# gabrielspmoreira/chameleon_recsys

Hardware: AMD Instinct MI355X
Metric: NAR training sessions/sec (higher is better)
Workload: dtype f32

## Files before the change

### chameleon_recsys_amd/_lib.py

```python
import ctypes
import os
from ctypes import c_double, c_float, c_int, c_int32, c_int64, c_long, c_size_t, c_uint32, c_void_p

_HERE = os.path.dirname(os.path.abspath(__file__))
LIB_PATH = os.path.join(_HERE, "libchameleon_nar.so")

P = c_void_p

_SIGNATURES = {
    "cham_neg_sample_workspace_bytes": (c_size_t, [c_int, c_int, c_int]),
    "cham_neg_sample": (c_int, [P, c_int, c_int, P, c_int, c_uint32, c_uint32, c_int, c_int, c_int, c_int, P, P, P, P, P,
                                P, c_size_t, P]),
    "cham_ctx_assemble": (c_int, [P, P, c_int, P, c_int, P, P, P, P, P, P]),
    "cham_set_log_bases": (c_int, [c_float, c_float]),
    "cham_step_ints": (c_int, [P, P, P, P, c_int64, c_int, c_int, P, c_int, P, P, P, P, P, P]),
    "cham_item_dynamic_raw": (c_int, [P, P, c_int, P, P, P, P, P]),
    "cham_norm_stats_from_recent": (c_int, [P, c_int, c_int64, P, P, P, P, P]),
    "cham_norm_stats_from_buffer": (c_int, [P, c_int, c_int64, P, P, P, P, P]),
    "cham_norm_stats_from_rows": (c_int, [P, P, P, c_int, P, P]),
    "cham_row_weights": (c_int, [P, c_int, P, c_size_t, c_int, P, P, P, P]),
    "cham_item_assemble": (c_int, [P, c_int, c_int, c_int, P, c_int, P, c_int, P, P, P, P, c_int, P, P, P, P, P, P]),
    "cham_item_assemble_lds": (c_int, [P, c_int, c_int, c_int, P, c_int, P, c_int, P, P, P, P, c_int, P, c_int, P, c_int, P, P, P, P, P, P]),
    "cham_feature_bwd": (c_int, [P, P, c_int, c_int, P, P, P]),
    "cham_feature_bwd_workspace_bytes": (c_size_t, [c_int]),
    "cham_feature_bwd_ws": (c_int, [P, P, c_int, c_int, P, P, P, c_size_t, P]),
    "cham_emb_grad_scan": (c_int, [P, c_int, c_int, c_int, c_int, P, P, P, c_int, P, P]),
    "cham_group_rows_workspace_bytes": (c_size_t, [c_int]),
    "cham_group_rows_segments_len": (c_size_t, [c_int]),
    "cham_group_rows": (c_int, [P, c_int, c_int, P, P, P, c_size_t, P]),
    "cham_emb_grad_grouped": (c_int, [P, c_int, c_int, c_int, c_int, P, P, P, P, P, P]),
    "cham_dropout": (c_int, [P, P, c_long, c_int, c_int, c_float, c_uint32, c_uint32, c_int, c_int, c_int, P, c_int, c_int, c_int, c_int, P]),
    "cham_dense_rows": (c_int, [P, c_int, P, c_int, c_int, c_int, c_int, P, P, P]),
    "cham_gemm_f32": (c_int, [P, c_int, c_int, P, c_int, c_int, P, c_int, c_int, c_int, c_int, P, c_int, P, c_int, c_int,
                              P, c_int, c_int, c_int, P, c_size_t, c_int, P]),
    "cham_gemm_bf16": (c_int, [P, c_int, c_int, P, c_int, c_int, P, c_int, c_int, c_int, c_int, P, c_int, P, c_int, c_int,
                               P, c_int, c_int, c_int, P, c_size_t, c_int, P]),
    "cham_gemm_f32x3": (c_int, [P, c_int, c_int, P, c_int, c_int, P, c_int, c_int, c_int, c_int, P, c_int, P, c_int, c_int,
                                P, c_int, c_int, c_int, P, c_size_t, c_int, P]),
    "cham_gemm_f32x2h": (c_int, [P, c_int, c_int, P, c_int, c_int, P, c_int, c_int, c_int, c_int, P, c_int,
                                 P, c_int, c_int, c_int, P, c_size_t, c_int, P, P, P]),
    "cham_gemm_f32x3_set_variant": (None, [c_int]),
    "cham_gemm_f32x3_launch_counts": (None, [P, c_int]),
    "cham_gemm_p3": (c_int, [P, c_int64, c_int, P, c_int64, c_int, c_int, P, c_int, c_int, c_int, c_int, P, c_int, P, c_int, c_int, c_int,
                             P, c_size_t, c_int, P]),
    "cham_gemm_b16_dma": (c_int, [P, c_int, P, c_int, c_int, P, c_int, c_int, c_int, c_int, P, c_int, P, c_int, c_int, c_int, P, c_size_t, c_int, P]),
    "cham_gemm_p3_launch_counts": (None, [P, c_int]),
    "cham_gemm_b16_dma_set_nt_wide": (c_int, [c_int]),
    "cham_split3": (c_int, [P, c_int, c_int, c_int, P, c_int64, c_int, P, c_int64, c_int, P]),
    "cham_combine_fwd_p3": (c_int, [P, P, c_int, c_int, c_int, c_int, P, P, c_int64, P]),
    "cham_mulpred_bwd_p3": (c_int, [P, P, P, c_int, c_int, c_int, P, P, c_int64, P, P]),
    "cham_dm_mulpred_p3": (c_int, [P, c_int, c_int, P, c_int64, P, P, c_int, c_int, c_int, P, c_int64, P, P, P]),
    "cham_h2_scale_absmax": (c_int, [P, c_size_t, P, c_size_t, P, P]),
    "cham_h2_scale_rownorm": (c_int, [P, c_long, c_int, c_int, P, P, P]),
    "cham_h2_scale_rownorm2": (c_int, [P, c_long, c_int, c_int, P, P, P, P]),
    "cham_split2h": (c_int, [P, c_int, c_int, c_int, P, c_int64, c_int, P, c_int64, c_int, P, c_int, P]),
    "cham_gemm_h2": (c_int, [P, c_int64, c_int, P, P, c_int64, c_int, P, c_int, P, c_int, c_int, c_int, c_int, P, c_int, P, c_int, c_int, c_int,
                             P, c_size_t, c_int, P]),
    "cham_h2b_block_elements": (c_int, []),
    "cham_gemm_h2b": (c_int, [P, c_int64, c_int, P, P, c_int64, c_int, P, c_int, P, c_int, c_int, c_int, c_int, P, c_int, P, c_int, c_int, c_int,
                              P, c_size_t, c_int, c_int, c_int, c_int, P]),
    "cham_combine_fwd_h2b": (c_int, [P, P, c_int, c_int, c_int, c_int, P, P, c_int64, P, c_int, P]),
    "cham_dm_mulpred_h2_blk": (c_int, [P, c_int, c_int, P, c_int64, P, P, P, P, c_int, c_int, c_int, P, c_int64, P, P, P, P]),
    "cham_gemm_h2_launch_counts": (None, [P, c_int]),
    "cham_gemm_h2_set_nt_wide": (c_int, [c_int]),
    "cham_combine_fwd_h2": (c_int, [P, P, c_int, c_int, c_int, c_int, P, P, c_int64, P, P]),
    "cham_mulpred_bwd_h2": (c_int, [P, P, P, c_int, c_int, c_int, P, P, c_int64, P, P, P]),
    "cham_dm_mulpred_h2": (c_int, [P, c_int, c_int, P, c_int64, P, P, c_int, c_int, c_int, P, c_int64, P, P, P, P]),
    "cham_dm_mulpred_h2h": (c_int, [P, c_int, c_int, P, c_int64, P, P, P, P, c_int, c_int, c_int, P, c_int64, P, P, P, P]),
    "cham_dm_mulpred_b16": (c_int, [P, c_int, c_int, P, P, P, c_int, c_int, c_int, P, P, P, P]),
    "cham_gemm_b16": (c_int, [P, c_int, c_int, P, c_int, c_int, P, c_int, c_int, c_int, c_int, c_int, P, c_int, P, c_int, c_int, c_int,
                              P, c_size_t, c_int, P]),
    "cham_gemm_b16_set_variant": (None, [c_int]),
    "cham_gemm_b16_launch_counts": (None, [P, c_int]),
    "cham_gemm_set_variant": (None, [c_int]),
    "cham_gemm_launch_counts": (None, [P, c_int]),
    "cham_combine_fwd": (c_int, [P, P, c_int, c_int, c_int, c_int, P, P, c_long, c_long, P]),
    "cham_combine_bwd_workspace_bytes": (c_size_t, [c_int, c_int, c_int, c_int]),
    "cham_combine_bwd": (c_int, [P, c_int, c_int, c_int, c_int, P, P, P, P, c_size_t, P]),
    "cham_combine_bwd_gs": (c_int, [P, c_int, c_int, c_int, c_int, P, P, P, P, c_size_t, P, c_size_t, P]),
    "cham_gemm_h2_groupsum_bytes": (c_size_t, [c_int, c_int, c_int]),
    "cham_gemm_h2_dgrad_gs": (c_int, [P, c_int64, c_int, P, P, c_int64, c_int, P, P, c_int, c_int, c_int, c_int, P, c_int, c_int, c_int, c_int, P,
                                      c_size_t, P]),
    "cham_combine_fwd_b16": (c_int, [P, P, c_int, c_int, c_int, c_int, P, P, P]),
    "cham_combine_bwd_b16": (c_int, [P, P, c_int, c_int, c_int, c_int, P, P, P, P, c_size_t, P]),
    "cham_mulpred_bwd_b16": (c_int, [P, P, P, c_int, c_int, c_int, P, P]),
    "cham_mul_rows_b16": (c_int, [P, P, c_int, c_int, c_int, P, P]),
    "cham_score_softmax_fwd_b16": (c_int, [P, c_int, P, P, c_int, c_int, c_float, P, P, P, P, c_float, P, P, P, P]),
    "cham_score_softmax_bwd_b16": (c_int, [P, c_int, P, P, P, c_int, c_int, c_float, c_float, P, P, c_float, P, P, P, P, P]),
    "cham_colsum_b16": (c_int, [P, c_int, c_int, c_int, P, P, c_int, P, c_size_t, P]),
    "cham_cast_b16": (c_int, [P, c_int, c_int, P, P, P]),
    "cham_upcast_b16": (c_int, [P, c_size_t, P, P]),
    "cham_rnn_fwd": (c_int, [c_int, P, P, P, c_int, c_int, c_int, P, P, P, P, P, P, P]),
    "cham_rnn_bwd": (c_int, [c_int, P, P, P, c_int, c_int, c_int, P, P, P, P, P, P]),
    "cham_rnn_coop_workspace_bytes": (c_size_t, [c_int, c_int]),
    "cham_ugrnn_fwd_coop": (c_int, [P, P, P, c_int, c_int, c_int, P, P, P, P, P, c_size_t, P]),
    "cham_ugrnn_bwd_coop": (c_int, [P, P, P, c_int, c_int, c_int, P, P, P, P, P, c_size_t, P]),
    "cham_rnn_coop_timeouts": (c_int, [P, c_int, c_int, P]),
    "cham_ugrnn_point_fwd": (c_int, [P, P, P, c_int, c_int, c_int, c_int, P, P, P, P, P, P]),
    "cham_ugrnn_point_bwd": (c_int, [P, P, P, c_int, c_int, c_int, c_int, P, P, P, P, P, P, P]),
    "cham_transpose_f32": (c_int, [P, c_int, c_int, P, P]),
    "cham_rows_gather": (c_int, [P, P, c_long, c_int, P, P]),
    "cham_rows_scatter": (c_int, [P, P, c_long, c_int, P, P]),
    "cham_mulpred_bwd": (c_int, [P, P, P, c_int, c_int, c_int, P, P]),
    "cham_score_softmax_fwd": (c_int, [P, c_int, P, P, c_int, c_int, c_float, P, P, P, P, c_float, P, P, P, P]),
    "cham_score_softmax_bwd": (c_int, [P, c_int, P, P, P, c_int, c_int, c_float, c_float, P, P, c_float, P, P, P, P, P]),
    "cham_rank_items": (c_int, [P, P, P, P, c_int, c_int, P, P, P, P]),
    "cham_state_workspace_bytes": (c_size_t, [c_int, c_int]),
    "cham_state_update": (c_int, [P, P, c_int, c_int, c_double, P, P, c_int, P, P, P, c_int, c_int, P, P, c_size_t, P]),
    "cham_sumsq_partial": (c_int, [P, c_size_t, P, P]),
    "cham_loss_finalize": (c_int, [P, c_int, c_float, P, c_float, P, P]),
    "cham_adam_tf": (c_int, [P, P, P, P, c_size_t, c_size_t, c_float, c_float, c_float, c_float, c_float, P]),
    "cham_step_scalars_bytes": (c_int, []),
    "cham_step_scalars_set": (c_int, [P, c_uint32, c_uint32, c_int64, c_float, c_float, c_int, P]),
    "cham_neg_sample_dev": (c_int, [P, c_int, c_int, P, c_int, c_uint32, P, c_int, c_int, c_int, c_int, c_int, P, P, P, P, P, P, c_size_t, P]),
    "cham_step_ints_dev": (c_int, [P, P, P, P, P, c_int, c_int, P, c_int, P, P, P, P, P, P]),
    "cham_norm_stats_from_buffer_dev": (c_int, [P, c_int, P, P, P, P, P, P]),
    "cham_score_softmax_bwd_dev": (c_int, [P, c_int, P, P, P, c_int, c_int, c_float, P, P, P, c_float, P, P, P, P, P]),
    "cham_score_softmax_bwd_b16_dev": (c_int, [P, c_int, P, P, P, c_int, c_int, c_float, P, P, P, c_float, P, P, P, P, P]),
    "cham_loss_finalize_dev": (c_int, [P, c_int, P, P, c_float, P, P]),
    "cham_adam_tf_dev": (c_int, [P, P, P, P, c_size_t, c_size_t, c_float, P, c_float, c_float, c_float, P]),
    "cham_accumulate": (c_int, [P, P, c_size_t, c_int, P]),
    "cham_loss_accumulate": (c_int, [P, P, c_int, P]),
    "cham_colsum_workspace_bytes": (c_size_t, [c_int, c_int]),
    "cham_colsum": (c_int, [P, c_int, c_int, c_int, P, P, c_int, P, c_size_t, P]),
}

EXPORTED_SYMBOLS = tuple(_SIGNATURES.keys())


class ChameleonLibError(RuntimeError):
    pass


_lib = None


def load():
    global _lib
    if _lib is not None:
        return _lib
    if not os.path.exists(LIB_PATH):
        raise ChameleonLibError(
            "HIP extension %s is missing - run `python -c 'import __graft_entry__ as g; g.build()'` "
            "(hipcc --offload-arch=gfx950).  There is no CPU fallback." % LIB_PATH)
    lib = ctypes.CDLL(LIB_PATH)
    for name, (res, args) in _SIGNATURES.items():
        fn = getattr(lib, name)
        fn.restype = res
        fn.argtypes = args
    lib.cham_gemm_h2_set_nt_wide(1 if os.environ.get("CHAM_H2_NT_WIDE", "1") == "1" else 0)
    lib.cham_gemm_b16_dma_set_nt_wide(1 if os.environ.get("CHAM_B16_NT_WIDE", "1") == "1" else 0)
    _lib = lib
    return lib


def check(rc, what):
    if rc != 0:
        raise ChameleonLibError("%s failed with code %d" % (what, rc))


def ptr(t):
    return None if t is None else t.data_ptr()
```

### chameleon_recsys_amd/build.py

```python
import hashlib
import os
import subprocess
import sys

HERE = os.path.dirname(os.path.abspath(__file__))
CSRC = os.path.join(HERE, "csrc")
LIB = os.path.join(HERE, "libchameleon_nar.so")
SOURCES = ["gemm.hip", "gemm_x3.hip", "gemm_p3.hip", "gemm_h2.hip", "dm_fused.hip", "gemm_b16.hip", "sampler.hip", "features.hip", "scorer.hip", "rnn.hip", "rnn_coop.hip", "optim.hip", "state.hip"]
FLAGS = ["--offload-arch=gfx950", "-O3", "-std=c++17", "-fPIC", "-Wall", "-Wno-unused-function"]
FLAGS += os.environ.get("CHAM_BUILD_DEFINES", "").split()


HOST_LIB = os.path.join(HERE, "libchameleon_tfrecord.so")
HOST_SOURCES = [os.path.join(CSRC, "host", "tfrecord.cpp")]
HOST_FLAGS = ["-O2", "-std=c++17", "-fPIC", "-shared", "-Wall", "-pthread"]


def _stamp(files=None, flags=FLAGS):
    h = hashlib.sha256()
    if files is None:
        files = [os.path.join(CSRC, f) for f in sorted(os.listdir(CSRC)) if os.path.isfile(os.path.join(CSRC, f))]
    for f in files:
        with open(f, "rb") as fh:
            h.update(os.path.basename(f).encode()); h.update(fh.read())
    h.update(" ".join(flags).encode())
    return h.hexdigest()


HOST_LIB_SANITIZED = os.path.join(HERE, "libchameleon_tfrecord_san.so")
SANITIZE_FLAGS = ["-O1", "-g", "-fno-omit-frame-pointer", "-fsanitize=address,undefined", "-fno-sanitize-recover=undefined"]


def build_host(force=False, verbose=True, sanitize=False):
    lib = HOST_LIB_SANITIZED if sanitize else HOST_LIB
    flags = [f for f in HOST_FLAGS if f != "-O2"] + SANITIZE_FLAGS if sanitize else HOST_FLAGS
    stamp_file = lib + ".stamp"
    stamp = _stamp(HOST_SOURCES, flags)
    if not force and os.path.exists(lib) and os.path.exists(stamp_file) and open(stamp_file).read() == stamp:
        return lib
    cmd = [os.environ.get("CXX", "g++")] + flags + HOST_SOURCES + ["-o", lib, "-lz"]
    if verbose:
        print(" ".join(cmd), flush=True)
    subprocess.check_call(cmd)
    with open(stamp_file, "w") as fh:
        fh.write(stamp)
    return lib


def sanitizer_runtime():
    try:
        out = subprocess.check_output([os.environ.get("CXX", "g++"), "-print-file-name=libasan.so"]).decode().strip()
    except (OSError, subprocess.CalledProcessError):
        return None
    return os.path.realpath(out) if os.path.sep in out and os.path.exists(out) else None


def _src_stamp(src):
    h = hashlib.sha256()
    for f in [os.path.join(CSRC, src)] + sorted(os.path.join(CSRC, x) for x in os.listdir(CSRC) if x.endswith(".h")):
        with open(f, "rb") as fh:
            h.update(os.path.basename(f).encode()); h.update(fh.read())
    h.update(" ".join(FLAGS).encode())
    return h.hexdigest()


def build(force=False, verbose=True):
    stamp_file = LIB + ".stamp"
    stamp = _stamp()
    if not force and os.path.exists(LIB) and os.path.exists(stamp_file) and open(stamp_file).read() == stamp:
        return LIB
    hipcc = os.environ.get("HIPCC", "/opt/rocm/bin/hipcc")
    objs = []
    procs = []
    os.makedirs(os.path.join(HERE, "build"), exist_ok=True)
    for s in SOURCES:
        o = os.path.join(HERE, "build", s.replace(".hip", ".o"))
        objs.append(o)
        st, sf = _src_stamp(s), o + ".stamp"
        if not force and os.path.exists(o) and os.path.exists(sf) and open(sf).read() == st:
            continue
        cmd = [hipcc] + FLAGS + ["-c", os.path.join(CSRC, s), "-o", o]
        if verbose:
            print(" ".join(cmd), flush=True)
        procs.append((s, sf, st, subprocess.Popen(cmd, stdout=subprocess.PIPE, stderr=subprocess.STDOUT)))
    for s, sf, st, p in procs:
        out, _ = p.communicate()
        if p.returncode != 0:
            sys.stderr.write(out.decode())
            raise RuntimeError("hipcc failed on %s" % s)
        if verbose and out.strip():
            print(out.decode())
        with open(sf, "w") as fh:
            fh.write(st)
    cmd = [hipcc, "--offload-arch=gfx950", "-shared", "-fPIC", "-o", LIB] + objs
    if verbose:
        print(" ".join(cmd), flush=True)
    subprocess.check_call(cmd)
    with open(stamp_file, "w") as fh:
        fh.write(stamp)
    return LIB


if __name__ == "__main__":
    build(force="--force" in sys.argv)
    build_host(force="--force" in sys.argv)
```

### chameleon_recsys_amd/csrc/gemm_h2.hip

```cpp
#include "gemm_shared.h"

typedef _Float16 half8 __attribute__((ext_vector_type(8)));
typedef short h2_s16x4 __attribute__((ext_vector_type(4)));

struct H2Params {
    const _Float16* A; const _Float16* B;
    long long a_ps, b_ps;
    int lda, ldb;
    const float* sa; const float* sb;
    float* C; int ldc;
    int M, N, K;
    const float* bias;
    const unsigned short* dref; int ldr;
    int kchunk, splits; float* partial;
    int nbm, nbn, xcd_split, accumulate;
    int a_tiles, b_tiles, r_blk;
    float* gsum; int ggrp, gsk;
};

#define H2_SLAB 8192
#define H2_STAGE (4 * H2_SLAB)
#define H2_RING 4

__device__ __forceinline__ u32x4 h2_rsrc(const void* base, unsigned bytes) {
    const unsigned long long a = (unsigned long long)base;
    u32x4 r;
    r.x = (unsigned)a; r.y = (unsigned)(a >> 32) & 0xFFFFu; r.z = bytes; r.w = 0x00020000u;
    return r;
}

__device__ __forceinline__ void h2_dma_stage(unsigned lds0, unsigned va, unsigned vb, const u32x4& ra0, const u32x4& ra1, const u32x4& rb0,
                                             const u32x4& rb1) {
    unsigned keep;
    const unsigned l1 = lds0 + H2_SLAB, l2 = lds0 + 2 * H2_SLAB, l3 = lds0 + 3 * H2_SLAB;
    asm volatile(
        "s_nop 4\n\t"
        "s_mov_b32 %0, m0\n\t"
        "s_mov_b32 m0, %1\n\ts_nop 0\n\tbuffer_load_dwordx4 %5, %7, 0 offen lds\n\t"
        "s_mov_b32 m0, %2\n\ts_nop 0\n\tbuffer_load_dwordx4 %5, %8, 0 offen lds\n\t"
        "s_mov_b32 m0, %3\n\ts_nop 0\n\tbuffer_load_dwordx4 %6, %9, 0 offen lds\n\t"
        "s_mov_b32 m0, %4\n\ts_nop 0\n\tbuffer_load_dwordx4 %6, %10, 0 offen lds\n\t"
        "s_mov_b32 m0, %0"
        : "=&s"(keep)
        : "s"(lds0), "s"(l1), "s"(l2), "s"(l3), "v"(va), "v"(vb), "s"(ra0), "s"(ra1), "s"(rb0), "s"(rb1)
        : "memory");
}

template <bool TN>
__device__ __forceinline__ half8 h2_frag(const unsigned char* __restrict__ s, unsigned hi_off = 4 * 512) {
    if constexpr (!TN) {
        return *reinterpret_cast<const half8*>(s);
    } else {
        typedef __attribute__((address_space(3))) h2_s16x4 lds_s4;
        const h2_s16x4 lo = __builtin_amdgcn_ds_read_tr16_b64_v4i16((lds_s4*)(s));
        const h2_s16x4 hi = __builtin_amdgcn_ds_read_tr16_b64_v4i16((lds_s4*)(s + hi_off));
        typedef short s16x8 __attribute__((ext_vector_type(8)));
        s16x8 v;
        v[0] = lo[0]; v[1] = lo[1]; v[2] = lo[2]; v[3] = lo[3]; v[4] = hi[0]; v[5] = hi[1]; v[6] = hi[2]; v[7] = hi[3];
        return __builtin_bit_cast(half8, v);
    }
}

__device__ __forceinline__ void h2_barrier() {
    __builtin_amdgcn_fence(__ATOMIC_RELEASE, "workgroup", "local");
    __builtin_amdgcn_s_waitcnt(0xc07f);
    __builtin_amdgcn_s_barrier();
    __builtin_amdgcn_fence(__ATOMIC_ACQUIRE, "workgroup", "local");
    __builtin_amdgcn_sched_barrier(0);
}

template <int EPI, int TM, int TNN>
__device__ __forceinline__ void h2_epilogue(const H2Params& p, floatx16 (&acc)[TM][TNN], int m0, int n0, int wm0, int wn0, int split, int lane) {
    int lane_e = lane;
    asm volatile("" : "+v"(lane_e));
    const int kl = lane_e >> 5, fl = lane_e & 31;
    const float ia = p.sa[1], ib = p.sb[1];
#pragma unroll
    for (int i = 0; i < TM; ++i)
#pragma unroll
        for (int j = 0; j < TNN; ++j)
#pragma unroll
            for (int e = 0; e < 16; ++e) acc[i][j][e] = (acc[i][j][e] * ia) * ib;
    if constexpr (EPI == 3) {
        const int limM = p.M - m0, limN = p.N - n0;
        const __amdgpu_buffer_rsrc_t cw = make_window(p.C + (size_t)m0 * p.ldc + n0);
        const bool rb = p.r_blk != 0;
        const __amdgpu_buffer_rsrc_t dw = make_window(rb ? p.dref + ((size_t)(m0 >> 8) * (size_t)(p.ldr >> 5) + (size_t)(n0 >> 5)) * H2B_BLOCK
                                                         : p.dref + (size_t)m0 * p.ldr + n0);
        const int rstride = rb ? 64 : p.ldr * 2;
        const bool gs = p.gsum != nullptr;
        const int G = gs ? p.ggrp : 1, rbase = m0 + wm0;
        float* gw = gs ? p.gsum + (size_t)(rbase >> 7) * (size_t)p.gsk * (size_t)p.N + n0 + wn0 + fl : nullptr;
        float cur[TNN], hik[TNN];
#pragma unroll
        for (int j = 0; j < TNN; ++j) { cur[j] = 0.f; hik[j] = 0.f; }
        int kk = 0;
        auto emit = [&]() {
#pragma unroll
            for (int j = 0; j < TNN; ++j) {
                const float x = cur[j] + __shfl_xor(cur[j], 32, 64);
                if (kl == 0 && wn0 + j * 32 + fl < limN) gw[(size_t)kk * p.N + j * 32] = x;
            }
            ++kk;
        };
        int bnd = 64;
        auto block_begin = [&](int i) {
            if (!gs) return;
            const int s0 = rbase + 32 * i, gf = s0 / G;
            bnd = (gf + 1) * G - s0;
            if (i > 0 && bnd == G) {
                emit();
#pragma unroll
                for (int j = 0; j < TNN; ++j) cur[j] = 0.f;
            }
        };
        auto block_add = [&](int j, const float (&v)[16]) {
            if (!gs) return;
            float lo = 0.f;
            if (bnd >= 32) {
#pragma unroll
                for (int e = 0; e < 16; ++e) lo += v[e];
            } else {
                float hi = 0.f;
#pragma unroll
                for (int e = 0; e < 16; ++e) {
                    const bool first = (e & 3) + 8 * (e >> 2) + 4 * kl < bnd;
                    lo += first ? v[e] : 0.f;
                    hi += first ? 0.f : v[e];
                }
                hik[j] = hi;
            }
            cur[j] += lo;
        };
        auto block_end = [&]() {
            if (!gs || bnd >= 32) return;
            emit();
#pragma unroll
            for (int j = 0; j < TNN; ++j) cur[j] = hik[j];
        };
        if (limM >= wm0 + TM * 32 && limN >= wn0 + TNN * 32) {
#pragma unroll
            for (int i = 0; i < TM; ++i) {
                block_begin(i);
#pragma unroll
                for (int j = 0; j < TNN; ++j) {
                    const unsigned col = (unsigned)(wn0 + j * 32 + fl), rowb = (unsigned)(wm0 + i * 32 + 4 * kl);
                    const unsigned voff = (rowb * (unsigned)p.ldc + col) * 4u;
                    const unsigned voffr = rb ? (unsigned)((wn0 >> 5) + j) * (unsigned)(H2B_BLOCK * 2) + rowb * 64u + (unsigned)fl * 2u
                                              : (rowb * (unsigned)p.ldr + col) * 2u;
                    unsigned short y[16];
#pragma unroll
                    for (int e = 0; e < 16; ++e) {
                        const int ce = (e & 3) + 8 * (e >> 2);
// ... 215 lines not shown
            for (int ii = 0; ii < TM; ++ii) AL[ii] = h2_frag<TN>(Sn + 1 * H2_SLAB + fa[ii], hia);
            mma(AH, BL);
            cur = nxt;
        }
        asm volatile("s_waitcnt vmcnt(0)" ::: "memory");
    }

    h2_epilogue<EPI, TM, TNN>(p, acc, m0, n0, wm0, wn0, split, lane);
}

#define H2W_SLAB 16384
#define H2W_BUF (4 * H2W_SLAB)

__device__ __forceinline__ void h2w_dma4(unsigned l0, unsigned l1, unsigned v0, unsigned v1, const u32x4& r0, const u32x4& r1) {
    unsigned keep;
    const unsigned l0b = l0 + 1024u, l1b = l1 + 1024u;
    asm volatile(
        "s_nop 4\n\t"
        "s_mov_b32 %0, m0\n\t"
        "s_mov_b32 m0, %1\n\ts_nop 0\n\tbuffer_load_dwordx4 %5, %7, 0 offen lds\n\t"
        "s_mov_b32 m0, %2\n\ts_nop 0\n\tbuffer_load_dwordx4 %6, %7, 0 offen lds\n\t"
        "s_mov_b32 m0, %3\n\ts_nop 0\n\tbuffer_load_dwordx4 %5, %8, 0 offen lds\n\t"
        "s_mov_b32 m0, %4\n\ts_nop 0\n\tbuffer_load_dwordx4 %6, %8, 0 offen lds\n\t"
        "s_mov_b32 m0, %0"
        : "=&s"(keep)
        : "s"(l0), "s"(l0b), "s"(l1), "s"(l1b), "v"(v0), "v"(v1), "s"(r0), "s"(r1)
        : "memory");
}

template <int EPI, bool ABLK>
__global__ __launch_bounds__(512) void gemm_h2w_kernel(H2Params p) {
    constexpr int BM = 256, BN = 256, TM = 4, TNN = 2;
    extern __shared__ __attribute__((aligned(1024))) unsigned char h2_smem[];

    const int nwg = p.nbm * p.nbn;
    const int id = blockIdx.x;
    const int q8 = nwg / 8, rr = nwg % 8, xcd = id % 8;
    const int swz = (xcd < rr ? xcd * (q8 + 1) : rr * (q8 + 1) + (xcd - rr) * q8) + id / 8;
    const int tile_m = swz / p.nbn, tile_n = swz % p.nbn;
    const int m0 = tile_m * BM, n0 = tile_n * BN;
    const int nd = p.K >> 5;
    const int lane = threadIdx.x & 63, wave = __builtin_amdgcn_readfirstlane(threadIdx.x >> 6);
    const int wm0 = (wave >> 2) * 128, wn0 = (wave & 3) * 64;

    u32x4 ra[2], rb[2];
    const size_t aall = (size_t)max(p.M - m0, 0) * p.lda * 2, ball = (size_t)max(p.N - n0, 0) * p.ldb * 2;
#pragma unroll
    for (int q = 0; q < 2; ++q) {
        if constexpr (ABLK) ra[q] = h2_rsrc(p.A + q * p.a_ps + (size_t)tile_m * (size_t)(p.lda >> 5) * H2B_BLOCK,
                                            (unsigned)min((size_t)(p.lda >> 5) * (H2B_BLOCK * 2), (size_t)0xFFFFFFF0u));
        else ra[q] = h2_rsrc(p.A + q * p.a_ps + (size_t)m0 * p.lda, (unsigned)min(aall, (size_t)0xFFFFFFF0u));
        rb[q] = h2_rsrc(p.B + q * p.b_ps + (size_t)n0 * p.ldb, (unsigned)min(ball, (size_t)0xFFFFFFF0u));
    }
    const unsigned row = 32u * (unsigned)wave + (unsigned)(lane >> 2), sp = (unsigned)((lane & 3) ^ ((lane >> 4) & 3));
    unsigned va0 = ABLK ? row * 64u + 16u * sp : (row * (unsigned)p.lda + 8u * sp) * 2u;
    unsigned va1 = va0 + (ABLK ? 16u * 64u : 16u * (unsigned)p.lda * 2u);
    constexpr unsigned stepA = ABLK ? (unsigned)(H2B_BLOCK * 2) : 64u;
    unsigned vb0 = (row * (unsigned)p.ldb + 8u * sp) * 2u, vb1 = vb0 + 16u * (unsigned)p.ldb * 2u;

    unsigned fa0[TM], fb0[TNN], fa1[TM], fb1[TNN];
    {
        const int l31 = lane & 31;
        const unsigned fo = (unsigned)l31 * 64u + (unsigned)((lane >> 5) ^ ((l31 >> 2) & 3)) * 16u;
#pragma unroll
        for (int i = 0; i < TM; ++i) { fa0[i] = (unsigned)(wm0 + 32 * i) * 64u + fo; fa1[i] = fa0[i] ^ 32u; }
#pragma unroll
        for (int j = 0; j < TNN; ++j) { fb0[j] = (unsigned)(wn0 + 32 * j) * 64u + fo; fb1[j] = fb0[j] ^ 32u; }
    }

    floatx16 acc[TM][TNN];
#pragma unroll
    for (int i = 0; i < TM; ++i)
#pragma unroll
        for (int j = 0; j < TNN; ++j)
#pragma unroll
            for (int e = 0; e < 16; ++e) acc[i][j][e] = 0.f;

    typedef __attribute__((address_space(3))) unsigned char lds_u8;
    const unsigned lds_base = (unsigned)(unsigned long long)(lds_u8*)h2_smem;
    const unsigned wave_off = (unsigned)wave * 2048u;
    half8 AH[TM], AL[TM], BH[TNN], BL[TNN];

    auto mma = [&](const half8 (&X)[TM], const half8 (&Y)[TNN]) {
#pragma unroll
        for (int ii = 0; ii < TM; ++ii)
#pragma unroll
            for (int j = 0; j < TNN; ++j) acc[ii][j] = __builtin_amdgcn_mfma_f32_32x32x16_f16(X[ii], Y[j], acc[ii][j], 0, 0, 0);
        __builtin_amdgcn_sched_barrier(0);
    };
    auto dma_a = [&](unsigned buf) {
        h2w_dma4(lds_base + buf + 0 * H2W_SLAB + wave_off, lds_base + buf + 1 * H2W_SLAB + wave_off, va0, va1, ra[0], ra[1]);
        va0 += stepA; va1 += stepA;
    };
    auto dma_b = [&](unsigned buf) {
        h2w_dma4(lds_base + buf + 2 * H2W_SLAB + wave_off, lds_base + buf + 3 * H2W_SLAB + wave_off, vb0, vb1, rb[0], rb[1]);
        vb0 += 64u; vb1 += 64u;
    };

    if (nd > 0) {
        dma_a(0u); dma_b(0u);
        if (nd > 1) {
            dma_a((unsigned)H2W_BUF);
            asm volatile("s_waitcnt vmcnt(4)" ::: "memory");
        } else {
            asm volatile("s_waitcnt vmcnt(0)" ::: "memory");
        }
        h2_barrier();
        {
#pragma unroll
            for (int j = 0; j < TNN; ++j) BH[j] = *reinterpret_cast<const half8*>(h2_smem + 2 * H2W_SLAB + fb0[j]);
#pragma unroll
            for (int i = 0; i < TM; ++i) AL[i] = *reinterpret_cast<const half8*>(h2_smem + 1 * H2W_SLAB + fa0[i]);
        }
        for (int j = 0; j < nd; ++j) {
            const unsigned b0 = (unsigned)(j & 1) * (unsigned)H2W_BUF, b1 = (unsigned)H2W_BUF - b0;
            const unsigned char* S0 = h2_smem + b0;
            const unsigned char* S1 = h2_smem + b1;
            __builtin_amdgcn_sched_barrier(0);
            if (j + 1 < nd) dma_b(b1);
            __builtin_amdgcn_sched_barrier(0);
#pragma unroll
            for (int ii = 0; ii < TM; ++ii) AH[ii] = *reinterpret_cast<const half8*>(S0 + 0 * H2W_SLAB + fa0[ii]);
#pragma unroll
            for (int jn = 0; jn < TNN; ++jn) BL[jn] = *reinterpret_cast<const half8*>(S0 + 3 * H2W_SLAB + fb0[jn]);
            mma(AL, BH);
            mma(AH, BH);
#pragma unroll
            for (int jn = 0; jn < TNN; ++jn) BH[jn] = *reinterpret_cast<const half8*>(S0 + 2 * H2W_SLAB + fb1[jn]);
#pragma unroll
            for (int ii = 0; ii < TM; ++ii) AL[ii] = *reinterpret_cast<const half8*>(S0 + 1 * H2W_SLAB + fa1[ii]);
            mma(AH, BL);
#pragma unroll
            for (int ii = 0; ii < TM; ++ii) AH[ii] = *reinterpret_cast<const half8*>(S0 + 0 * H2W_SLAB + fa1[ii]);
#pragma unroll
            for (int jn = 0; jn < TNN; ++jn) BL[jn] = *reinterpret_cast<const half8*>(S0 + 3 * H2W_SLAB + fb1[jn]);
            mma(AL, BH);
            mma(AH, BH);
            asm volatile("s_waitcnt vmcnt(0)" ::: "memory");
            h2_barrier();
            if (j + 2 < nd) dma_a(b0);
            __builtin_amdgcn_sched_barrier(0);
#pragma unroll
            for (int jn = 0; jn < TNN; ++jn) BH[jn] = *reinterpret_cast<const half8*>(S1 + 2 * H2W_SLAB + fb0[jn]);
#pragma unroll
            for (int ii = 0; ii < TM; ++ii) AL[ii] = *reinterpret_cast<const half8*>(S1 + 1 * H2W_SLAB + fa0[ii]);
            mma(AH, BL);
        }
        asm volatile("s_waitcnt vmcnt(0)" ::: "memory");
    }

    h2_epilogue<EPI, TM, TNN>(p, acc, m0, n0, wm0, wn0, 0, lane);
}

__device__ __forceinline__ void h2_finish_scale(H2Scale* rec, float bound) {
    float s = 1.f, inv = 1.f;
    if (bound > 0.f && bound < __builtin_inff()) {
        int e;
        (void)frexpf(bound, &e);
        int k = 15 - e;
        k = k < -110 ? -110 : (k > 110 ? 110 : k);
        s = ldexpf(1.f, k); inv = ldexpf(1.f, -k);
    }
    rec->scale = s; rec->inv = inv; rec->bound = bound;
}

__device__ __forceinline__ float h2_block_max(float v, float* red) {
    v = wave_max(v);
    const int lane = threadIdx.x & 63, w = threadIdx.x >> 6;
    if (lane == 0) red[w] = v;
    __syncthreads();
    float t = 0.f;
    for (int i = 0; i < (int)(blockDim.x >> 6); ++i) t = fmaxf(t, red[i]);
    __syncthreads();
    return t;
}

__global__ __launch_bounds__(256) void k_h2_scale_absmax(const float* __restrict__ x0, size_t n0, const float* __restrict__ x1, size_t n1,
                                                         H2Scale* __restrict__ rec) {
    __shared__ float red[4];
    __shared__ unsigned last;
    float m0 = 0.f, m1 = 0.f;
    const size_t stride = (size_t)gridDim.x * 256;
#pragma unroll 4
    for (size_t i = (size_t)blockIdx.x * 256 + threadIdx.x; i < n0 / 4; i += stride) {
        const float4 v = reinterpret_cast<const float4*>(x0)[i];
        m0 = fmaxf(m0, fmaxf(fmaxf(fabsf(v.x), fabsf(v.y)), fmaxf(fabsf(v.z), fabsf(v.w))));
    }
    if (x1)
#pragma unroll 4
        for (size_t i = (size_t)blockIdx.x * 256 + threadIdx.x; i < n1 / 4; i += stride) {
            const float4 v = reinterpret_cast<const float4*>(x1)[i];
            m1 = fmaxf(m1, fmaxf(fmaxf(fabsf(v.x), fabsf(v.y)), fmaxf(fabsf(v.z), fabsf(v.w))));
        }
    m0 = h2_block_max(m0, red);
    m1 = h2_block_max(m1, red);
    if (threadIdx.x == 0) {
        atomicMax(&rec->max_bits, __float_as_uint(m0));
        if (x1) atomicMax(&rec->pad1, __float_as_uint(m1));
        __threadfence();
        last = atomicAdd(&rec->ticket, 1u) == gridDim.x - 1 ? 1u : 0u;
        if (last) {
            __threadfence();
            const float a = __uint_as_float(atomicMax(&rec->max_bits, 0u)), b = __uint_as_float(atomicMax(&rec->pad1, 0u));
            h2_finish_scale(rec, a + b);
            rec->max_bits = 0u; rec->pad1 = 0u; rec->ticket = 0u;
        }
    }
}

__global__ __launch_bounds__(256) void k_h2_scale_rownorm(const float* __restrict__ X, long R, int K, int ld, const float* __restrict__ factor,
                                                          H2Scale* __restrict__ rec, H2Scale* __restrict__ rec_plain) {
    __shared__ float red[4];
    __shared__ unsigned last;
    const int lane = threadIdx.x & 63;
    const long wave_g = (long)blockIdx.x * 4 + (threadIdx.x >> 6), nwaves = (long)gridDim.x * 4;
    float mx = 0.f;
    if (K == 128) {
        const int hl = lane & 31, hw = lane >> 5;
        const long stride = 2 * nwaves;
        long r = 2 * wave_g + hw;
        for (; r + 3 * stride < R; r += 4 * stride) {
            float4 v[4];
#pragma unroll
            for (int u = 0; u < 4; ++u) v[u] = reinterpret_cast<const float4*>(X + (size_t)(r + u * stride) * ld)[hl];
#pragma unroll
            for (int u = 0; u < 4; ++u) {
                float s = v[u].x * v[u].x + v[u].y * v[u].y + v[u].z * v[u].z + v[u].w * v[u].w;
#pragma unroll
                for (int o = 16; o > 0; o >>= 1) s += __shfl_xor(s, o, 64);
                mx = fmaxf(mx, s);
            }
        }
        for (; r < R; r += stride) {
            const float4 v = reinterpret_cast<const float4*>(X + (size_t)r * ld)[hl];
            float s = v.x * v.x + v.y * v.y + v.z * v.z + v.w * v.w;
#pragma unroll
            for (int o = 16; o > 0; o >>= 1) s += __shfl_xor(s, o, 64);
            mx = fmaxf(mx, s);
        }
    } else {
        for (long r = wave_g; r < R; r += nwaves) {
            float s = 0.f;
            for (int k = lane; k < K; k += 64) { const float v = X[(size_t)r * ld + k]; s += v * v; }
            mx = fmaxf(mx, wave_sum(s));
        }
    }
    mx = h2_block_max(mx, red);
    if (threadIdx.x == 0) {
        atomicMax(&rec->max_bits, __float_as_uint(mx));
        __threadfence();
        last = atomicAdd(&rec->ticket, 1u) == gridDim.x - 1 ? 1u : 0u;
        if (last) {
            __threadfence();
            const float sq = __uint_as_float(atomicMax(&rec->max_bits, 0u));
            const float b = sqrtf(sq) * (factor ? *factor : 1.f) * 1.0009765625f;
            h2_finish_scale(rec, b);
            if (rec_plain) h2_finish_scale(rec_plain, sqrtf(sq) * 1.0009765625f);
            rec->max_bits = 0u; rec->ticket = 0u;
        }
    }
}

extern "C" int cham_h2_scale_absmax(const float* x0, size_t n0, const float* x1, size_t n1, void* rec, void* stream) {
    if (!x0 || !rec || (n0 & 3) || (x1 && (n1 & 3)) || (((uintptr_t)x0 | (uintptr_t)x1) & 15) || ((uintptr_t)rec & 15)) return -CHAM_ERR_ARG;
    size_t n = n0 > n1 ? n0 : n1;
    int blocks = (int)((n / 4 + 255) / 256);
    blocks = blocks < 1 ? 1 : (blocks > 512 ? 512 : blocks);
    hipLaunchKernelGGL(k_h2_scale_absmax, dim3(blocks), dim3(256), 0, (hipStream_t)stream, x0, n0, x1, x1 ? n1 : (size_t)0, reinterpret_cast<H2Scale*>(rec));
    CHAM_CHECK_LAUNCH();
    return CHAM_OK;
}

extern "C" int cham_h2_scale_rownorm2(const float* X, long R, int K, int ld, const float* factor, void* rec, void* rec_plain, void* stream) {
    if (!X || !rec || R < 0 || K <= 0 || ld < K || (((uintptr_t)rec | (uintptr_t)rec_plain) & 15) || rec == rec_plain) return -CHAM_ERR_ARG;
    if (K == 128 && ((ld & 3) || ((uintptr_t)X & 15))) return -CHAM_ERR_ARG;
    const long per = K == 128 ? 8 : 4;
    long blocks = (R + per - 1) / per;
    blocks = blocks < 1 ? 1 : (blocks > 1024 ? 1024 : blocks);
    hipLaunchKernelGGL(k_h2_scale_rownorm, dim3((unsigned)blocks), dim3(256), 0, (hipStream_t)stream, X, R, K, ld, factor, reinterpret_cast<H2Scale*>(rec),
                       reinterpret_cast<H2Scale*>(rec_plain));
    CHAM_CHECK_LAUNCH();
    return CHAM_OK;
}
extern "C" int cham_h2_scale_rownorm(const float* X, long R, int K, int ld, const float* factor, void* rec, void* stream) {
    return cham_h2_scale_rownorm2(X, R, K, ld, factor, rec, nullptr, stream);
}

__global__ __launch_bounds__(256) void k_split2h(const float* __restrict__ X, int R, int Cc, int ld, _Float16* __restrict__ dst, long long ps,
                                                 int ldd, _Float16* __restrict__ dstT, long long psT, int lddT, const H2Scale* __restrict__ rec) {
    const float s = rec->scale;
    const size_t n = (size_t)R * Cc;
    for (size_t i = (size_t)blockIdx.x * 256 + threadIdx.x; i < n; i += (size_t)gridDim.x * 256) {
        const int r = (int)(i / Cc), c = (int)(i % Cc);
        const float x = X[(size_t)r * ld + c];
        _Float16 h, l;
        split2h(x * s, h, l);
        const unsigned short hb = h2_keep_sign(h, x);
        if (dst) { _Float16* d = dst + (size_t)r * ldd + c; *reinterpret_cast<unsigned short*>(d) = hb; d[ps] = l; }
        if (dstT) { _Float16* d = dstT + (size_t)c * lddT + r; *reinterpret_cast<unsigned short*>(d) = hb; d[psT] = l; }
    }
}

extern "C" int cham_split2h(const float* X, int R, int Cc, int ld, void* dst, long long plane_stride, int ldd, void* dstT,
                            long long plane_strideT, int lddT, void* rec, int recompute, void* stream) {
    if (!X || R <= 0 || Cc <= 0 || (!dst && !dstT) || !rec || ((uintptr_t)rec & 15)) return -CHAM_ERR_ARG;
    const size_t n = (size_t)R * Cc;
    if (recompute) {
        if (ld != Cc || (n & 3) || ((uintptr_t)X & 15)) return -CHAM_ERR_ARG;
        const int rc = cham_h2_scale_absmax(X, n, nullptr, 0, rec, stream);
        if (rc != CHAM_OK) return rc;
    }
    int blocks = (int)((n + 255) / 256);
    if (blocks > 8192) blocks = 8192;
    hipLaunchKernelGGL(k_split2h, dim3(blocks), dim3(256), 0, (hipStream_t)stream, X, R, Cc, ld, reinterpret_cast<_Float16*>(dst), plane_stride,
                       ldd, reinterpret_cast<_Float16*>(dstT), plane_strideT, lddT, reinterpret_cast<const H2Scale*>(rec));
    CHAM_CHECK_LAUNCH();
    return CHAM_OK;
}

extern "C" int cham_h2b_block_elements(void) { return H2B_BLOCK; }

static long long g_h2_launches[8];
extern "C" void cham_gemm_h2_launch_counts(long long* out8, int reset) {
    for (int i = 0; i < 8; ++i) { if (out8) out8[i] = g_h2_launches[i]; if (reset) g_h2_launches[i] = 0; }
}

static int g_h2_nt_wide = 1;
extern "C" int cham_gemm_h2_set_nt_wide(int on) { const int was = g_h2_nt_wide; g_h2_nt_wide = on ? 1 : 0; return was; }

template <int EPI, bool ABLK>
static int h2w_launch_l(H2Params& p, hipStream_t st) {
    g_h2_launches[6] = EPI; g_h2_launches[7] = 1; ++g_h2_launches[2];
    if (ABLK) ++g_h2_launches[3];
    constexpr int smem = 2 * H2W_BUF;
    auto k = gemm_h2w_kernel<EPI, ABLK>;
    CHAM_SET_DYNAMIC_LDS(k, smem);
    hipLaunchKernelGGL(k, dim3(p.nbm * p.nbn, 1, 1), dim3(512), smem, st, p);
    CHAM_CHECK_LAUNCH();
    return CHAM_OK;
}
template <int EPI>
static int h2w_launch(H2Params& p, hipStream_t st) {
    return p.a_tiles > 0 ? h2w_launch_l<EPI, true>(p, st) : h2w_launch_l<EPI, false>(p, st);
}

template <bool TN, int EPI>
static int h2_launch(H2Params& p, hipStream_t st) {
    g_h2_launches[6] = EPI; g_h2_launches[7] = p.splits;
    constexpr int smem = H2_RING * H2_STAGE;
    auto k = gemm_h2_kernel<TN, EPI>;
    CHAM_SET_DYNAMIC_LDS(k, smem);
    hipLaunchKernelGGL(k, dim3(p.nbm * p.nbn, p.splits, 1), dim3(512), smem, st, p);
    CHAM_CHECK_LAUNCH();
    return CHAM_OK;
}
extern "C" size_t cham_gemm_h2_groupsum_bytes(int M, int N, int group_rows) {
    if (M <= 0 || N <= 0 || group_rows < 32) return 0;
    return (size_t)2 * ((M + 255) / 256) * (size_t)(127 / group_rows + 2) * (size_t)N * sizeof(float);
}
static int h2_run(const void* A, long long a_plane_stride, int lda, const float* a_scale, const void* B, long long b_plane_stride,
                  int ldb, const float* b_scale, int tn, float* C, int ldc, int M, int N, int K, const float* bias, int act,
                  const void* dref_h, int ldr, int dact, int accumulate, float* workspace, size_t workspace_bytes, int splits_hint,
                  int a_tiles, int b_tiles, int dref_blocked, int group_rows, float* groupsum, size_t groupsum_bytes, void* stream) {
    if (!A || !B || !C || !a_scale || !b_scale || M <= 0 || N <= 0 || K <= 0 || a_tiles < 0 || b_tiles < 0) return -CHAM_ERR_ARG;
    if (groupsum && (tn || !dref_h || group_rows < 32 || groupsum_bytes < cham_gemm_h2_groupsum_bytes(M, N, group_rows) || ((uintptr_t)groupsum & 15)))
        return -CHAM_ERR_ARG;
    {
        const long a_rows = tn ? K : M, b_rows = tn ? K : N;
        if (a_tiles && ((lda & 31) || (long)a_tiles * 256 < a_rows || a_plane_stride < (long long)a_tiles * (lda >> 5) * H2B_BLOCK)) return -CHAM_ERR_ARG;
        if (b_tiles && ((ldb & 31) || (long)b_tiles * 256 < b_rows || b_plane_stride < (long long)b_tiles * (ldb >> 5) * H2B_BLOCK)) return -CHAM_ERR_ARG;
        if (!tn && (b_tiles || (a_tiles && (lda != K || (K & 31) || !g_h2_nt_wide)))) return -CHAM_ERR_ARG;
        if (dref_blocked && (!dref_h || (ldr & 31) || tn)) return -CHAM_ERR_ARG;
    }
    if ((lda & 7) || (ldb & 7) || (a_plane_stride & 7) || (b_plane_stride & 7) || (N & 3) || (ldc & 3)) return -CHAM_ERR_ARG;
    if (((uintptr_t)A | (uintptr_t)B | (uintptr_t)C) & 15) return -CHAM_ERR_ARG;
    if ((size_t)ldc * 4 * 256 >= WINDOW_BYTES || (size_t)ldr * 2 * 256 >= WINDOW_BYTES) return -CHAM_ERR_ARG;
    H2Params p;
    p.A = reinterpret_cast<const _Float16*>(A); p.B = reinterpret_cast<const _Float16*>(B); p.a_ps = a_plane_stride; p.b_ps = b_plane_stride;
    p.lda = lda; p.ldb = ldb; p.sa = a_scale; p.sb = b_scale; p.C = C; p.ldc = ldc; p.M = M; p.N = N; p.K = K; p.bias = bias;
    p.dref = reinterpret_cast<const unsigned short*>(dref_h); p.ldr = ldr; p.partial = workspace; p.xcd_split = 0; p.accumulate = 0;
    p.nbm = (M + 255) / 256; p.nbn = (N + 255) / 256;
    p.a_tiles = a_tiles; p.b_tiles = b_tiles; p.r_blk = dref_blocked ? 1 : 0;
    p.gsum = groupsum; p.ggrp = group_rows; p.gsk = groupsum ? 127 / group_rows + 2 : 0;
    hipStream_t st = (hipStream_t)stream;
    if (!tn) {
        if ((K & 15) || accumulate) return -CHAM_ERR_ARG;
        if ((size_t)256 * lda * 2 >= (1ull << 31) || (size_t)256 * ldb * 2 >= (1ull << 31)) return -CHAM_ERR_ARG;
        p.kchunk = K; p.splits = 1;
        if (dref_h && (bias || act != ACT_NONE || dact != ACT_LEAKY)) return -CHAM_ERR_ARG;
        if (act != ACT_NONE && !(bias && act == ACT_TANH)) return -CHAM_ERR_ARG;
        ++g_h2_launches[0];
        if (groupsum) ++g_h2_launches[5];
        if (g_h2_nt_wide && (K & 31) == 0) {
            if (dref_h) return h2w_launch<3>(p, st);
            if (bias) return act == ACT_TANH ? h2w_launch<2>(p, st) : h2w_launch<5>(p, st);
            return h2w_launch<0>(p, st);
        }
        if (dref_h) return h2_launch<false, 3>(p, st);
        if (bias) return act == ACT_TANH ? h2_launch<false, 2>(p, st) : h2_launch<false, 5>(p, st);
        return h2_launch<false, 0>(p, st);
    }
    if ((M & 255) || (N & 255) || bias || act != ACT_NONE || dref_h) return -CHAM_ERR_ARG;
    if ((size_t)16 * lda * 2 >= (1ull << 31) || (size_t)16 * ldb * 2 >= (1ull << 31)) return -CHAM_ERR_ARG;
    const long tiles = (long)p.nbm * p.nbn;
    int splits = 1;
    if (splits_hint != 1 && workspace) {
        long want = splits_hint > 1 ? splits_hint : (tiles >= 192 ? 1 : (256 + tiles - 1) / tiles);
        const long maxk = (K + 511) / 512;
        if (want > maxk) want = maxk;
        const long maxw = (long)(workspace_bytes / ((size_t)M * N * sizeof(float)));
        if (want > maxw) want = maxw;
        if (splits_hint <= 0 && want >= 8) want = want / 8 * 8;
        if (want > 1) splits = (int)want;
// ... 48 lines not shown
```

### chameleon_recsys_amd/csrc/scorer.hip

```cpp
#include "common.h"

__device__ __forceinline__ int cand_vrow(int bt, int c, int BT, int N, int pmax, const int* __restrict__ neg_slot) {
    if (c == 0) return BT + bt;
    int s = neg_slot[(size_t)bt * N + (c - 1)];
    if (s < 0) s = pmax;
    return 2 * BT + s;
}

__global__ __launch_bounds__(256) void k_combine_fwd(const float* __restrict__ U, const float* __restrict__ V, int C,
                                                     int BT, int N, int pmax, const int* __restrict__ neg_slot,
                                                     float* __restrict__ Z1, int row_begin) {
    const int row = row_begin + blockIdx.x;
    int u, v;
    if (row < BT) { u = row; v = row; }
    else {
        const int i = row - BT, bt = i / (N + 1), c = i % (N + 1);
        u = bt; v = cand_vrow(bt, c, BT, N, pmax, neg_slot);
    }
    const float4* pu = reinterpret_cast<const float4*>(U + (size_t)u * C);
    const float4* pv = reinterpret_cast<const float4*>(V + (size_t)v * C);
    float4* po = reinterpret_cast<float4*>(Z1 + (size_t)row * C);
    for (int k = threadIdx.x; k < C / 4; k += 256) {
        const float4 a = pu[k], b = pv[k];
        float4 o;
        o.x = act_fwd(a.x + b.x, ACT_LEAKY); o.y = act_fwd(a.y + b.y, ACT_LEAKY);
        o.z = act_fwd(a.z + b.z, ACT_LEAKY); o.w = act_fwd(a.w + b.w, ACT_LEAKY);
        po[k] = o;
    }
}

template <typename T>
__global__ __launch_bounds__(256) void k_combine_fwd_cand(const float* __restrict__ U, const float* __restrict__ V, int C,
                                                          int BT, int N, int pmax, const int* __restrict__ neg_slot,
                                                          T* __restrict__ Z1c ) {
    const int bt = blockIdx.x, NC = N + 1;
    const float4* pu = reinterpret_cast<const float4*>(U + (size_t)bt * C);
    T* po = Z1c + (size_t)bt * NC * C;
    for (int k = threadIdx.x; k < C / 4; k += 256) {
        const float4 a = pu[k];
        for (int c0 = 0; c0 < NC; c0 += 4) {
            float4 b[4];
#pragma unroll
            for (int i = 0; i < 4; ++i) {
                const int c = c0 + i < NC ? c0 + i : NC - 1;
                b[i] = reinterpret_cast<const float4*>(V + (size_t)cand_vrow(bt, c, BT, N, pmax, neg_slot) * C)[k];
            }
#pragma unroll
            for (int i = 0; i < 4; ++i) {
                if (c0 + i >= NC) break;
                float4 o;
                o.x = act_fwd(a.x + b[i].x, ACT_LEAKY); o.y = act_fwd(a.y + b[i].y, ACT_LEAKY);
                o.z = act_fwd(a.z + b[i].z, ACT_LEAKY); o.w = act_fwd(a.w + b[i].w, ACT_LEAKY);
                st4(po + (size_t)(c0 + i) * C + 4 * k, o);
            }
        }
    }
}

__global__ __launch_bounds__(256) void k_combine_fwd_cand_p3(const float* __restrict__ U, const float* __restrict__ V, int C,
                                                             int BT, int N, int pmax, const int* __restrict__ neg_slot,
                                                             __bf16* __restrict__ Z1p , long long ps) {
    const int bt = blockIdx.x, NC = N + 1;
    const float4* pu = reinterpret_cast<const float4*>(U + (size_t)bt * C);
    __bf16* po = Z1p + (size_t)bt * NC * C;
    for (int k = threadIdx.x; k < C / 4; k += 256) {
        const float4 a = pu[k];
        for (int c0 = 0; c0 < NC; c0 += 4) {
            float4 b[4];
#pragma unroll
            for (int i = 0; i < 4; ++i) {
                const int c = c0 + i < NC ? c0 + i : NC - 1;
                b[i] = reinterpret_cast<const float4*>(V + (size_t)cand_vrow(bt, c, BT, N, pmax, neg_slot) * C)[k];
            }
#pragma unroll
            for (int i = 0; i < 4; ++i) {
                if (c0 + i >= NC) break;
                float4 o;
                o.x = act_fwd(a.x + b[i].x, ACT_LEAKY); o.y = act_fwd(a.y + b[i].y, ACT_LEAKY);
                o.z = act_fwd(a.z + b[i].z, ACT_LEAKY); o.w = act_fwd(a.w + b[i].w, ACT_LEAKY);
                st4_planes(po + (size_t)(c0 + i) * C + 4 * k, ps, o);
            }
        }
    }
}

__global__ __launch_bounds__(256) void k_combine_fwd_cand_h2(const float* __restrict__ U, const float* __restrict__ V, int C,
                                                             int BT, int N, int pmax, const int* __restrict__ neg_slot,
                                                             _Float16* __restrict__ Z1p , long long ps,
                                                             const H2Scale* __restrict__ rec, int blocked) {
    const int bt = blockIdx.x, NC = N + 1;
    const float sc = rec->scale;
    const float4* pu = reinterpret_cast<const float4*>(U + (size_t)bt * C);
    _Float16* po = Z1p + (size_t)bt * NC * C;
    const size_t grow0 = (size_t)bt * NC;
    const unsigned ncb = (unsigned)C >> 5;
    for (int k = threadIdx.x; k < C / 4; k += 256) {
        const float4 a = pu[k];
        for (int c0 = 0; c0 < NC; c0 += 4) {
            float4 b[4];
#pragma unroll
            for (int i = 0; i < 4; ++i) {
                const int c = c0 + i < NC ? c0 + i : NC - 1;
                b[i] = reinterpret_cast<const float4*>(V + (size_t)cand_vrow(bt, c, BT, N, pmax, neg_slot) * C)[k];
            }
#pragma unroll
            for (int i = 0; i < 4; ++i) {
                if (c0 + i >= NC) break;
                float4 o;
                o.x = act_fwd(a.x + b[i].x, ACT_LEAKY); o.y = act_fwd(a.y + b[i].y, ACT_LEAKY);
                o.z = act_fwd(a.z + b[i].z, ACT_LEAKY); o.w = act_fwd(a.w + b[i].w, ACT_LEAKY);
                st4_planes_h2(blocked ? Z1p + h2b_index(grow0 + (size_t)(c0 + i), 4u * (unsigned)k, ncb) : po + (size_t)(c0 + i) * C + 4 * k, ps, o, sc);
            }
        }
    }
}

template <typename T>
__global__ __launch_bounds__(256) void k_combine_bwd_u(const float* __restrict__ dpre_in, const T* __restrict__ dpre_cand, int C, int BT,
                                                       int N, float* __restrict__ dU, float* __restrict__ dV) {
    const int bt = blockIdx.x;
    const float4* pin = reinterpret_cast<const float4*>(dpre_in + (size_t)bt * C);
    const T* pc = dpre_cand + (size_t)bt * (N + 1) * C;
    for (int k = threadIdx.x; k < C / 4; k += 256) {
        const float4 a = pin[k];
        const float4 p0 = ld4(pc + 4 * k);
        float4 s = make_float4(a.x + p0.x, a.y + p0.y, a.z + p0.z, a.w + p0.w);
        for (int c = 1; c <= N; c += 8) {
            float4 x[8];
#pragma unroll
            for (int u = 0; u < 8; ++u) x[u] = ld4(pc + (size_t)min(c + u, N) * C + 4 * k);
#pragma unroll
            for (int u = 0; u < 8; ++u)
                if (c + u <= N) { s.x += x[u].x; s.y += x[u].y; s.z += x[u].z; s.w += x[u].w; }
        }
        reinterpret_cast<float4*>(dU + (size_t)bt * C)[k] = s;
        reinterpret_cast<float4*>(dV + (size_t)bt * C)[k] = a;
        reinterpret_cast<float4*>(dV + ((size_t)BT + bt) * C)[k] = p0;
    }
}

__global__ __launch_bounds__(256) void k_combine_bwd_u_gs(const float* __restrict__ dpre_in, const float* __restrict__ dpre_cand, int C, int BT,
                                                          int N, const float* __restrict__ gsum, float* __restrict__ dU, float* __restrict__ dV) {
    const int bt = blockIdx.x, G = N + 1, gsk = 127 / G + 2;
    const long r0 = (long)bt * G, r1 = r0 + G - 1;
    const int q0 = (int)(r0 >> 7), q1 = (int)(r1 >> 7);
    const float4* pin = reinterpret_cast<const float4*>(dpre_in + (size_t)bt * C);
    const float4* pc = reinterpret_cast<const float4*>(dpre_cand + (size_t)r0 * C);
    for (int k = threadIdx.x; k < C / 4; k += 256) {
        const float4 a = pin[k], p0 = pc[k];
        float4 s = a;
        for (int q = q0; q <= q1; ++q) {
            const int piece = bt - (int)(((long)q << 7) / G);
            const float4 x = reinterpret_cast<const float4*>(gsum + ((size_t)q * gsk + piece) * C)[k];
// ... 147 lines not shown
        list[off++] = threadIdx.x * SEG + bit;
    }
    __syncthreads();
    const int nk = C / 4;
    for (int k = threadIdx.x; k < nk; k += 256) {
        float4 acc = make_float4(0.f, 0.f, 0.f, 0.f);
        int t = 0;
        for (; t + 8 <= cnt; t += 8) {
            float4 x[8];
#pragma unroll
            for (int u = 0; u < 8; ++u) {
                const size_t i = i0 + list[t + u];
                const size_t row = (i / N) * (N + 1) + 1 + (i % N);
                x[u] = ld4(cand + row * C + 4 * k);
            }
#pragma unroll
            for (int u = 0; u < 8; ++u) { acc.x += x[u].x; acc.y += x[u].y; acc.z += x[u].z; acc.w += x[u].w; }
        }
        for (; t < cnt; ++t) {
            const size_t i = i0 + list[t];
            const size_t row = (i / N) * (N + 1) + 1 + (i % N);
            const float4 x = ld4(cand + row * C + 4 * k);
            acc.x += x.x; acc.y += x.y; acc.z += x.z; acc.w += x.w;
        }
        reinterpret_cast<float4*>(partial + (size_t)chunk * C)[k] = acc;
    }
}
__global__ __launch_bounds__(256) void k_combine_bwd_pad_final(const float* __restrict__ partial, int C, int nchunk,
                                                               float* __restrict__ dv_row) {
    for (int k = threadIdx.x; k < C / 4; k += 256) {
        float4 acc = make_float4(0.f, 0.f, 0.f, 0.f);
        for (int c = 0; c < nchunk; c += 16) {
            float4 x[16];
#pragma unroll
            for (int u = 0; u < 16; ++u) x[u] = reinterpret_cast<const float4*>(partial + (size_t)min(c + u, nchunk - 1) * C)[k];
#pragma unroll
            for (int u = 0; u < 16; ++u)
                if (c + u < nchunk) { acc.x += x[u].x; acc.y += x[u].y; acc.z += x[u].z; acc.w += x[u].w; }
        }
        reinterpret_cast<float4*>(dv_row)[k] = acc;
    }
}

template <typename T>
__global__ __launch_bounds__(256) void k_mulpred_bwd(T* __restrict__ dM, const T* __restrict__ Z2c,
                                                     const float* __restrict__ pred, int C, int N, float* __restrict__ dpred_pre) {
    const int bt = blockIdx.x;
    const float4* pp = reinterpret_cast<const float4*>(pred + (size_t)bt * C);
    for (int k = threadIdx.x; k < C / 4; k += 256) {
        const float4 p = pp[k];
        float4 acc = make_float4(0.f, 0.f, 0.f, 0.f);
        for (int c = 0; c <= N; ++c) {
            const size_t off = ((size_t)bt * (N + 1) + c) * C + 4 * k;
            const float4 g = ld4(dM + off);
            const float4 z = ld4(Z2c + off);
            acc.x += g.x * z.x; acc.y += g.y * z.y; acc.z += g.z * z.z; acc.w += g.w * z.w;
            float4 o;
            o.x = g.x * p.x * (1.f - z.x * z.x); o.y = g.y * p.y * (1.f - z.y * z.y);
            o.z = g.z * p.z * (1.f - z.z * z.z); o.w = g.w * p.w * (1.f - z.w * z.w);
            st4(dM + off, o);
        }
        float4 o;
        o.x = acc.x * (1.f - p.x * p.x); o.y = acc.y * (1.f - p.y * p.y);
        o.z = acc.z * (1.f - p.z * p.z); o.w = acc.w * (1.f - p.w * p.w);
        reinterpret_cast<float4*>(dpred_pre + (size_t)bt * C)[k] = o;
    }
}

__global__ __launch_bounds__(256) void k_mulpred_bwd_p3(const float* __restrict__ dM, const float* __restrict__ Z2c,
                                                        const float* __restrict__ pred, int C, int N, float* __restrict__ dpred_pre,
                                                        __bf16* __restrict__ dZ2p, long long ps, float* __restrict__ col_part) {
    const int bt = blockIdx.x;
    const float4* pp = reinterpret_cast<const float4*>(pred + (size_t)bt * C);
    for (int k = threadIdx.x; k < C / 4; k += 256) {
        const float4 p = pp[k];
        float4 acc = make_float4(0.f, 0.f, 0.f, 0.f), cs = make_float4(0.f, 0.f, 0.f, 0.f);
        for (int c = 0; c <= N; ++c) {
            const size_t off = ((size_t)bt * (N + 1) + c) * C + 4 * k;
            const float4 g = ld4(dM + off);
            const float4 z = ld4(Z2c + off);
            acc.x += g.x * z.x; acc.y += g.y * z.y; acc.z += g.z * z.z; acc.w += g.w * z.w;
            float4 o;
            o.x = g.x * p.x * (1.f - z.x * z.x); o.y = g.y * p.y * (1.f - z.y * z.y);
            o.z = g.z * p.z * (1.f - z.z * z.z); o.w = g.w * p.w * (1.f - z.w * z.w);
            cs.x += o.x; cs.y += o.y; cs.z += o.z; cs.w += o.w;
            st4_planes(dZ2p + off, ps, o);
        }
        float4 o;
        o.x = acc.x * (1.f - p.x * p.x); o.y = acc.y * (1.f - p.y * p.y);
        o.z = acc.z * (1.f - p.z * p.z); o.w = acc.w * (1.f - p.w * p.w);
        reinterpret_cast<float4*>(dpred_pre + (size_t)bt * C)[k] = o;
        if (col_part) reinterpret_cast<float4*>(col_part + (size_t)bt * C)[k] = cs;
    }
}

__global__ __launch_bounds__(256) void k_mulpred_bwd_h2(const float* __restrict__ dM, const float* __restrict__ Z2c,
                                                        const float* __restrict__ pred, int C, int N, float* __restrict__ dpred_pre,
                                                        _Float16* __restrict__ dZ2p, long long ps, float* __restrict__ col_part,
                                                        const H2Scale* __restrict__ rec) {
    const int bt = blockIdx.x;
    const float sc = rec->scale;
    const float4* pp = reinterpret_cast<const float4*>(pred + (size_t)bt * C);
    for (int k = threadIdx.x; k < C / 4; k += 256) {
        const float4 p = pp[k];
        float4 acc = make_float4(0.f, 0.f, 0.f, 0.f), cs = make_float4(0.f, 0.f, 0.f, 0.f);
        for (int c = 0; c <= N; ++c) {
            const size_t off = ((size_t)bt * (N + 1) + c) * C + 4 * k;
            const float4 g = ld4(dM + off);
            const float4 z = ld4(Z2c + off);
            acc.x += g.x * z.x; acc.y += g.y * z.y; acc.z += g.z * z.z; acc.w += g.w * z.w;
            float4 o;
            o.x = g.x * p.x * (1.f - z.x * z.x); o.y = g.y * p.y * (1.f - z.y * z.y);
            o.z = g.z * p.z * (1.f - z.z * z.z); o.w = g.w * p.w * (1.f - z.w * z.w);
            cs.x += o.x; cs.y += o.y; cs.z += o.z; cs.w += o.w;
            st4_planes_h2(dZ2p + off, ps, o, sc);
        }
        float4 o;
        o.x = acc.x * (1.f - p.x * p.x); o.y = acc.y * (1.f - p.y * p.y);
        o.z = acc.z * (1.f - p.z * p.z); o.w = acc.w * (1.f - p.w * p.w);
        reinterpret_cast<float4*>(dpred_pre + (size_t)bt * C)[k] = o;
        if (col_part) reinterpret_cast<float4*>(col_part + (size_t)bt * C)[k] = cs;
    }
}

__global__ __launch_bounds__(256) void k_mul_rows_b16(const __bf16* __restrict__ Z2c, const float* __restrict__ pred, int C, int NC,
                                                      __bf16* __restrict__ Mc) {
    const int bt = blockIdx.x;
    const float4* pp = reinterpret_cast<const float4*>(pred + (size_t)bt * C);
    for (int k = threadIdx.x; k < C / 4; k += 256) {
        const float4 p = pp[k];
        for (int c0 = 0; c0 < NC; c0 += 4) {
            float4 z[4];
#pragma unroll
            for (int i = 0; i < 4; ++i) z[i] = ld4(Z2c + ((size_t)bt * NC + min(c0 + i, NC - 1)) * C + 4 * k);
#pragma unroll
            for (int i = 0; i < 4; ++i) {
                if (c0 + i >= NC) break;
                st4(Mc + ((size_t)bt * NC + c0 + i) * C + 4 * k, make_float4(z[i].x * p.x, z[i].y * p.y, z[i].z * p.z, z[i].w * p.w));
            }
        }
    }
}

template <int K3, typename T>
__global__ __launch_bounds__(256) void k_score_softmax_fwd(const T* __restrict__ S3, const float* __restrict__ w4,
                                                           const float* __restrict__ b4, int BT, int N, float inv_tau,
                                                           const unsigned char* __restrict__ mask,
                                                           float* __restrict__ logits, float* __restrict__ probs,
                                                           float* __restrict__ nll, float nov_factor,
                                                           const int64_t* __restrict__ neg_ids, const float* __restrict__ pop_norm,
                                                           float* __restrict__ nov_aux , float inv_log2_base) {
    const int lane = threadIdx.x & 63, bt = blockIdx.x * 4 + (threadIdx.x >> 6);
    if (bt >= BT) return;
    const int NC = N + 1;
    float w[K3];
#pragma unroll
    for (int k = 0; k < K3; ++k) w[k] = w4[k];
    const float bias = b4[0];
    float mx = -INFINITY;
    for (int c = lane; c < NC; c += 64) {
        const T* r = S3 + ((size_t)bt * NC + c) * K3;
        float s = 0.f;
#pragma unroll
        for (int k = 0; k < K3 / 4; ++k) { const float4 x = ld4(r + 4 * k); s += x.x * w[4 * k] + x.y * w[4 * k + 1] + x.z * w[4 * k + 2] + x.w * w[4 * k + 3]; }
        s += bias;
        logits[(size_t)bt * NC + c] = s;
        mx = fmaxf(mx, s * inv_tau);
    }
    mx = wave_max(mx);
    float sum = 0.f;
    for (int c = lane; c < NC; c += 64) {
        const float e = expf(logits[(size_t)bt * NC + c] * inv_tau - mx);
        probs[(size_t)bt * NC + c] = e;
        sum += e;
    }
    sum = wave_sum(sum);
    const float inv = 1.f / sum;
    for (int c = lane; c < NC; c += 64) probs[(size_t)bt * NC + c] *= inv;
    float novterm = 0.f;
    if (nov_factor > 0.f) {
        float mxn = -INFINITY;
        for (int c = lane; c < NC; c += 64)
            if (c > 0) mxn = fmaxf(mxn, logits[(size_t)bt * NC + c] * inv_tau);
        mxn = wave_max(mxn);
        float sn = 0.f, acc = 0.f;
        for (int c = lane; c < NC; c += 64)
            if (c > 0) {
                const float e = expf(logits[(size_t)bt * NC + c] * inv_tau - mxn);
                sn += e;
                acc += e * (-log2f(pop_norm[neg_ids[(size_t)bt * N + (c - 1)]]) * inv_log2_base);
            }
        sn = wave_sum(sn); acc = wave_sum(acc);
        novterm = acc / sn;
        if (lane == 0) { nov_aux[(size_t)bt * 3] = mxn; nov_aux[(size_t)bt * 3 + 1] = sn; nov_aux[(size_t)bt * 3 + 2] = novterm; }
    }
    if (lane == 0) {
        const float z0 = logits[(size_t)bt * NC] * inv_tau;
        nll[bt] = mask[bt] ? -((z0 - mx) - logf(sum)) - nov_factor * novterm : 0.f;
    }
}

template <int K3, typename T>
__global__ __launch_bounds__(256) void k_score_softmax_bwd(const T* __restrict__ S3, const float* __restrict__ w4,
                                                           const float* __restrict__ probs, const unsigned char* __restrict__ mask,
                                                           int BT, int N, float scale ,
                                                           float* __restrict__ ds, T* __restrict__ dS3, float nov_factor,
                                                           const int64_t* __restrict__ neg_ids, const float* __restrict__ pop_norm,
                                                           const float* __restrict__ logits, float inv_tau,
                                                           const float* __restrict__ nov_aux, float inv_log2_base,
                                                           const ChamStepScalars* __restrict__ sc, float tau) {
    const size_t row = (size_t)blockIdx.x * 256 + threadIdx.x;
    const int NC = N + 1;
    if (row >= (size_t)BT * NC) return;
    if (sc) scale = 1.0f / (tau * sc->sum_mask);
    const int bt = (int)(row / NC), c = (int)(row % NC);
    float g = mask[bt] ? (probs[row] - (c == 0 ? 1.f : 0.f)) * scale : 0.f;
    if (nov_factor > 0.f && c > 0 && mask[bt]) {
        const float q = expf(logits[row] * inv_tau - nov_aux[(size_t)bt * 3]) / nov_aux[(size_t)bt * 3 + 1];
        const float nov_c = -log2f(pop_norm[neg_ids[(size_t)bt * N + (c - 1)]]) * inv_log2_base;
        g -= nov_factor * scale * q * (nov_c - nov_aux[(size_t)bt * 3 + 2]);
    }
    ds[row] = g;
    const T* r = S3 + row * K3;
    T* o = dS3 + row * K3;
#pragma unroll
    for (int k = 0; k < K3 / 4; ++k) {
        const float4 x = ld4(r + 4 * k);
        float4 y;
        y.x = g * w4[4 * k] * act_bwd_from_out(x.x, ACT_LEAKY);
        y.y = g * w4[4 * k + 1] * act_bwd_from_out(x.y, ACT_LEAKY);
        y.z = g * w4[4 * k + 2] * act_bwd_from_out(x.z, ACT_LEAKY);
        y.w = g * w4[4 * k + 3] * act_bwd_from_out(x.w, ACT_LEAKY);
        st4(o + 4 * k, y);
    }
}


__global__ __launch_bounds__(256) void k_rank_items(const float* __restrict__ probs, const int64_t* __restrict__ label_next,
                                                    const int64_t* __restrict__ neg_ids, const unsigned char* __restrict__ mask,
                                                    int BT, int N, int64_t* __restrict__ pred_ids, float* __restrict__ pred_probs,
                                                    int32_t* __restrict__ label_rank) {
    extern __shared__ float sp[];
    const int lane = threadIdx.x & 63, w = threadIdx.x >> 6, bt = blockIdx.x * 4 + w;
    const int NC = N + 1;
    float* p = sp + (size_t)w * NC;
    if (bt < BT)
        for (int c = lane; c < NC; c += 64) p[c] = probs[(size_t)bt * NC + c];
    __syncthreads();
    if (bt >= BT) return;
    for (int c = lane; c < NC; c += 64) {
        const float pc = p[c];
        int r = 0;
        for (int j = 0; j < NC; ++j) {
            const float pj = p[j];
            r += (pj > pc) || (pj == pc && j < c);
        }
        pred_ids[(size_t)bt * NC + r] = c == 0 ? label_next[bt] : neg_ids[(size_t)bt * N + (c - 1)];
        pred_probs[(size_t)bt * NC + r] = pc;
        if (c == 0) label_rank[bt] = mask[bt] ? r : -1;
    }
}

extern "C" int cham_combine_fwd(const float* U, const float* V, int C, int BT, int N, int pmax, const int32_t* neg_slot,
                                float* Z1, long row_begin, long row_count, void* stream) {
    if (!U || !V || !neg_slot || !Z1 || (C & 3) || BT <= 0 || N <= 0) return -CHAM_ERR_ARG;
    const long rows = (long)BT + (long)BT * (N + 1);
    if (row_begin < 0 || row_count <= 0 || row_begin + row_count > rows) return -CHAM_ERR_ARG;
    if (row_begin == BT && row_count == (long)BT * (N + 1))
        hipLaunchKernelGGL(k_combine_fwd_cand<float>, dim3((unsigned)BT), dim3(256), 0, (hipStream_t)stream, U, V, C, BT, N, pmax, neg_slot,
                           Z1 + (size_t)BT * C);
    else
        hipLaunchKernelGGL(k_combine_fwd, dim3((unsigned)row_count), dim3(256), 0, (hipStream_t)stream, U, V, C, BT, N, pmax,
                           neg_slot, Z1, (int)row_begin);
    CHAM_CHECK_LAUNCH();
    return CHAM_OK;
}
extern "C" int cham_combine_fwd_b16(const float* U, const float* V, int C, int BT, int N, int pmax, const int32_t* neg_slot,
                                    void* Z1c, void* stream) {
    if (!U || !V || !neg_slot || !Z1c || (C & 3) || BT <= 0 || N <= 0) return -CHAM_ERR_ARG;
    hipLaunchKernelGGL(k_combine_fwd_cand<__bf16>, dim3((unsigned)BT), dim3(256), 0, (hipStream_t)stream, U, V, C, BT, N, pmax, neg_slot,
                       reinterpret_cast<__bf16*>(Z1c));
    CHAM_CHECK_LAUNCH();
    return CHAM_OK;
}

static inline size_t al256(size_t x) { return (x + 255) & ~(size_t)255; }
struct SlotWs { size_t bitmap_bytes, partial_bytes, pad_bytes; int W, nchunk, nchunk_pad; };
static SlotWs slot_ws(int C, int BT, int N, int pmax) {
    SlotWs w;
    w.W = (BT + 31) / 32;
    w.nchunk = (w.W + SLOT_HOT / 32 - 1) / (SLOT_HOT / 32);
    w.nchunk_pad = (int)(((size_t)BT * N + SLOT_LIST - 1) / SLOT_LIST);
    w.bitmap_bytes = al256((size_t)pmax * w.W * sizeof(unsigned));
    w.partial_bytes = al256((size_t)w.nchunk * pmax * C * sizeof(float));
    w.pad_bytes = al256((size_t)w.nchunk_pad * C * sizeof(float));
    return w;
}
extern "C" size_t cham_combine_bwd_workspace_bytes(int C, int BT, int N, int pmax) {
    if (C <= 0 || BT <= 0 || N <= 0 || pmax <= 0) return 0;
    const SlotWs w = slot_ws(C, BT, N, pmax);
    return w.bitmap_bytes + w.partial_bytes + w.pad_bytes;
}

template <typename T>
static int combine_bwd_impl(const float* dpre_in, const T* dpre_cand, int C, int BT, int N, int pmax, const int32_t* neg_slot,
                            float* dU, float* dV, float* workspace, size_t workspace_bytes, void* stream, const float* gsum = nullptr) {
    if (!dpre_in || !dpre_cand || !neg_slot || !dU || !dV || !workspace || (C & 3) || BT <= 0 || N <= 0 || pmax <= 0) return -CHAM_ERR_ARG;
    if (workspace_bytes < cham_combine_bwd_workspace_bytes(C, BT, N, pmax) || ((uintptr_t)workspace & 15)) return -CHAM_ERR_ARG;
    hipStream_t st = (hipStream_t)stream;
    const SlotWs w = slot_ws(C, BT, N, pmax);
    unsigned* bitmap = reinterpret_cast<unsigned*>(workspace);
    float* partial = reinterpret_cast<float*>(reinterpret_cast<char*>(workspace) + w.bitmap_bytes);
    float* pad_partial = reinterpret_cast<float*>(reinterpret_cast<char*>(workspace) + w.bitmap_bytes + w.partial_bytes);
    const size_t n = (size_t)BT * N;
    if constexpr (sizeof(T) == 4) {
        if (gsum) hipLaunchKernelGGL(k_combine_bwd_u_gs, dim3(BT), dim3(256), 0, st, dpre_in, reinterpret_cast<const float*>(dpre_cand), C, BT, N, gsum, dU, dV);
        else hipLaunchKernelGGL(k_combine_bwd_u<T>, dim3(BT), dim3(256), 0, st, dpre_in, dpre_cand, C, BT, N, dU, dV);
    } else {
        hipLaunchKernelGGL(k_combine_bwd_u<T>, dim3(BT), dim3(256), 0, st, dpre_in, dpre_cand, C, BT, N, dU, dV);
    }
    if (hipMemsetAsync(bitmap, 0, (size_t)pmax * w.W * sizeof(unsigned), st) != hipSuccess) return -CHAM_ERR_LAUNCH;
    hipLaunchKernelGGL(k_slot_bitmap, dim3((unsigned)((n + 255) / 256)), dim3(256), 0, st, neg_slot, n, N, pmax, w.W, bitmap);
    hipLaunchKernelGGL(k_slot_reduce<T>, dim3(pmax, w.nchunk), dim3(256), 0, st, dpre_cand, C, BT, N, neg_slot, bitmap, w.W, pmax, partial, dV);
    hipLaunchKernelGGL(k_slot_final, dim3(pmax), dim3(256), 0, st, partial, C, pmax, w.nchunk, BT, bitmap, w.W, dV);
    hipLaunchKernelGGL(k_combine_bwd_slots_partial<T>, dim3(w.nchunk_pad), dim3(256), 0, st, dpre_cand, C, BT, N, neg_slot, pmax,
                       pad_partial, SLOT_LIST);
    hipLaunchKernelGGL(k_combine_bwd_pad_final, dim3(1), dim3(256), 0, st, pad_partial, C, w.nchunk_pad,
                       dV + ((size_t)2 * BT + pmax) * C);
    CHAM_CHECK_LAUNCH();
    return CHAM_OK;
}
extern "C" int cham_combine_bwd(const float* dpre, int C, int BT, int N, int pmax, const int32_t* neg_slot,
                                float* dU, float* dV, float* workspace, size_t workspace_bytes, void* stream) {
    if (!dpre || BT <= 0 || C <= 0) return -CHAM_ERR_ARG;
    return combine_bwd_impl<float>(dpre, dpre + (size_t)BT * C, C, BT, N, pmax, neg_slot, dU, dV, workspace, workspace_bytes, stream);
}
extern "C" int cham_combine_bwd_gs(const float* dpre, int C, int BT, int N, int pmax, const int32_t* neg_slot, float* dU, float* dV,
                                   float* workspace, size_t workspace_bytes, const float* groupsum, size_t groupsum_bytes, void* stream) {
    if (!dpre || BT <= 0 || C <= 0 || !groupsum || N + 1 < 32 || ((uintptr_t)groupsum & 15)) return -CHAM_ERR_ARG;
    const size_t rows = (size_t)BT * (N + 1);
    if (groupsum_bytes < (size_t)2 * ((rows + 255) / 256) * (size_t)(127 / (N + 1) + 2) * (size_t)C * sizeof(float)) return -CHAM_ERR_ARG;
    return combine_bwd_impl<float>(dpre, dpre + (size_t)BT * C, C, BT, N, pmax, neg_slot, dU, dV, workspace, workspace_bytes, stream, groupsum);
}
extern "C" int cham_combine_bwd_b16(const float* dpre_in, const void* dpre_cand, int C, int BT, int N, int pmax, const int32_t* neg_slot,
                                    float* dU, float* dV, float* workspace, size_t workspace_bytes, void* stream) {
    return combine_bwd_impl<__bf16>(dpre_in, reinterpret_cast<const __bf16*>(dpre_cand), C, BT, N, pmax, neg_slot, dU, dV, workspace,
                                    workspace_bytes, stream);
}

extern "C" int cham_mulpred_bwd(float* dM, const float* Z2c, const float* pred, int C, int BT, int N, float* dpred_pre,
                                void* stream) {
    if (!dM || !Z2c || !pred || !dpred_pre || (C & 3) || BT <= 0) return -CHAM_ERR_ARG;
    hipLaunchKernelGGL(k_mulpred_bwd<float>, dim3(BT), dim3(256), 0, (hipStream_t)stream, dM, Z2c, pred, C, N, dpred_pre);
    CHAM_CHECK_LAUNCH();
    return CHAM_OK;
}
extern "C" int cham_mulpred_bwd_b16(void* dM, const void* Z2c, const float* pred, int C, int BT, int N, float* dpred_pre, void* stream) {
    if (!dM || !Z2c || !pred || !dpred_pre || (C & 3) || BT <= 0) return -CHAM_ERR_ARG;
    hipLaunchKernelGGL(k_mulpred_bwd<__bf16>, dim3(BT), dim3(256), 0, (hipStream_t)stream, reinterpret_cast<__bf16*>(dM),
                       reinterpret_cast<const __bf16*>(Z2c), pred, C, N, dpred_pre);
    CHAM_CHECK_LAUNCH();
    return CHAM_OK;
}
extern "C" int cham_combine_fwd_p3(const float* U, const float* V, int C, int BT, int N, int pmax, const int32_t* neg_slot, void* Z1p,
                                   long long plane_stride, void* stream) {
    if (!U || !V || !neg_slot || !Z1p || C <= 0 || (C & 3) || BT < 0 || N < 0 || (plane_stride & 3)) return -CHAM_ERR_ARG;
    if (BT == 0) return CHAM_OK;
    hipLaunchKernelGGL(k_combine_fwd_cand_p3, dim3(BT), dim3(256), 0, (hipStream_t)stream, U, V, C, BT, N, pmax, neg_slot,
                       reinterpret_cast<__bf16*>(Z1p), plane_stride);
    CHAM_CHECK_LAUNCH();
    return CHAM_OK;
}

extern "C" int cham_mulpred_bwd_p3(const float* dM, const float* Z2c, const float* pred, int C, int BT, int N, float* dpred_pre, void* dZ2p,
                                   long long plane_stride, float* col_part, void* stream) {
    if (!dM || !Z2c || !pred || !dpred_pre || !dZ2p || C <= 0 || (C & 3) || BT < 0 || N < 0 || (plane_stride & 3)) return -CHAM_ERR_ARG;
    if (BT == 0) return CHAM_OK;
    hipLaunchKernelGGL(k_mulpred_bwd_p3, dim3(BT), dim3(256), 0, (hipStream_t)stream, dM, Z2c, pred, C, N, dpred_pre,
                       reinterpret_cast<__bf16*>(dZ2p), plane_stride, col_part);
    CHAM_CHECK_LAUNCH();
    return CHAM_OK;
}

extern "C" int cham_combine_fwd_h2b(const float* U, const float* V, int C, int BT, int N, int pmax, const int32_t* neg_slot, void* Z1p,
                                    long long plane_stride, const void* scale_rec, int blocked, void* stream) {
    if (!U || !V || !neg_slot || !Z1p || !scale_rec || C <= 0 || (C & 3) || BT < 0 || N < 0 || (plane_stride & 3)) return -CHAM_ERR_ARG;
    if (blocked && ((C & 31) || plane_stride < (long long)(((size_t)BT * (N + 1) + 255) / 256) * (C >> 5) * H2B_BLOCK)) return -CHAM_ERR_ARG;
// ... 109 lines not shown
```

### chameleon_recsys_amd/nar/nar_model.py

```python
import math
import os

import numpy as np
import torch

from .. import _lib
from .. import _roctx
from .._lib import check, ptr
from .clicked_items_state import lane_stream
from .layout import COL_ITEMEMB, ParamLayout

ACT_NONE, ACT_LEAKY, ACT_TANH = 0, 1, 2


class ModeKeys:
    TRAIN = 'train'
    EVAL = 'eval'
    PREDICT = 'infer'


_raw_stream = getattr(torch._C, '_cuda_getCurrentRawStream', None)
_raw_device = getattr(torch._C, '_cuda_getDevice', None)


_raw_checked = False


def _stream():
    global _raw_stream, _raw_checked
    if _raw_stream is not None and _raw_device is not None:
        if not _raw_checked:
            _raw_checked = True
            try:
                if int(_raw_stream(_raw_device())) != int(torch.cuda.current_stream().cuda_stream):
                    _raw_stream = None
            except Exception:
                _raw_stream = None
            if _raw_stream is None:
                return torch.cuda.current_stream().cuda_stream
        return _raw_stream(_raw_device())
    return torch.cuda.current_stream().cuda_stream


class Tensor:

    def __init__(self, name, fn):
        self.name, self._fn = name, fn

    def eval(self):
        v = self._fn()
        if torch.is_tensor(v):
            v = v.cpu().numpy()
        return v


class Placeholder:

    def __init__(self, name):
        self.name = name

    def __hash__(self):
        return hash(self.name)

    def __eq__(self, o):
        return isinstance(o, Placeholder) and o.name == self.name


_VARIABLE_STORE = None


class variable_store:
    def __init__(self, store):
        self.store = store

    def __enter__(self):
        global _VARIABLE_STORE
        self._prev, _VARIABLE_STORE = _VARIABLE_STORE, self.store
        return self.store

    def __exit__(self, *a):
        global _VARIABLE_STORE
        _VARIABLE_STORE = self._prev


_TORCH_DTYPE = {np.dtype(n).str: t for n, t in (('int64', torch.int64), ('int32', torch.int32), ('float32', torch.float32),
                                                   ('uint8', torch.uint8))}


def pack_offsets(arrays, align=256):
    offs, total = {}, 0
    for k, a in arrays.items():
        offs[k] = total
        total += (a.nbytes + align - 1) & ~(align - 1)
    return offs, total


class _PinnedRing:

    def __init__(self, n=4, nbytes=4 << 20):
        self.n, self.nbytes = n, nbytes
        self.bufs, self.events, self.k, self.off = [None] * n, [None] * n, -1, 0

    def begin(self, need):
        self.k = (self.k + 1) % self.n
        if self.events[self.k] is not None:
            self.events[self.k].synchronize()
        if self.bufs[self.k] is None or self.bufs[self.k].numel() < need:
            self.bufs[self.k] = torch.empty(max(need, self.nbytes), dtype=torch.uint8, pin_memory=True)
        self.off = 0

    def stage(self, a):
        n = a.nbytes
        if n == 0 or self.off + n > self.bufs[self.k].numel():
            return torch.from_numpy(a)
        view = self.bufs[self.k][self.off:self.off + n]
        self.off += (n + 255) & ~255
        t = view.view(torch.from_numpy(a).dtype).view(a.shape)
        t.copy_(torch.from_numpy(a))
        return t

    def end(self, stream):
        ev = torch.cuda.Event()
        ev.record(stream)
        self.events[self.k] = ev


class NARRuntime:

    def __init__(self, params, device='cuda:0', seed=42, weights=None):
        self.lib = _lib.load()
        self._views = {}
        if not torch.cuda.is_available():
            raise _lib.ChameleonLibError("no ROCm device visible: the NAR step has no CPU path")
        self.device = torch.device(device)
        self.params = params
        acfg = params['articles_features_config']
        ace = np.ascontiguousarray(params['content_article_embeddings_matrix'], dtype=np.float32)
        self.n_items = acfg['article_id'].get('cardinality', ace.shape[0]) if 'article_id' in acfg else ace.shape[0]
        if self.n_items != ace.shape[0]:
            raise ValueError("article_id cardinality (%d) != ACE rows (%d)" % (self.n_items, ace.shape[0]))
        self.item_id_bits = max(1, int(self.n_items - 1).bit_length())
        self.layout = ParamLayout(params['session_features_config'], acfg, self.n_items, ace.shape[1],
                                  params['CAR_embedding_size'], params['rnn_units'],
                                  params.get('rnn_num_layers', 1), params.get('rnn_cell', 'ugrnn'),
                                  params.get('internal_features_config'), params.get('max_cardinality_for_ohe', 10))
        L = self.layout
        logical = weights if weights is not None else L.init_logical(seed)
        dev = self.device
        self.flat = torch.from_numpy(L.pack(logical)).to(dev)
        self.m = torch.zeros_like(self.flat)
        self.v = torch.zeros_like(self.flat)
        self.grads = torch.zeros_like(self.flat)
        self.global_step = 0
        self.dev_scalars = os.environ.get("CHAM_DEV_SCALARS", "1") == "1"
        self.loss_side = os.environ.get("CHAM_LOSS_SIDE", "1") == "1"
        self.dgrad_groupsum = os.environ.get("CHAM_DGRAD_GROUPSUM", "1") == "1"
        self.feature_bwd_ws = os.environ.get("CHAM_FEATURE_BWD_WS", "1") == "1"
        self.tail_split = os.environ.get("CHAM_TAIL_SPLIT", "1") == "1"
        self.capturing = False
        self.scalars = None
        self.gemm_dtype = params.get('gemm_dtype', 'f32')
        if self.gemm_dtype not in ('f32', 'f32_native', 'bf16'):
            raise ValueError("gemm_dtype must be 'f32', 'f32_native' or 'bf16'")
        self.x3 = self.gemm_dtype == 'f32' and os.environ.get("CHAM_GEMM_X3", "1") == "1"
        self.p3 = self.x3 and os.environ.get("CHAM_GEMM_P3", "1") == "1" and self.layout.C % 256 == 0
        self.h2 = self.p3 and os.environ.get("CHAM_GEMM_H2", "1") == "1"
        blk = os.environ.get("CHAM_H2_BLOCKED", "0")
        self.h2_blocked = (self.h2 and blk in ("1", "dz2", "z1") and os.environ.get("CHAM_H2_NT_WIDE", "1") == "1" and self.layout.C % 32 == 0)
        self.h2_blocked_which = blk if self.h2_blocked else "0"
        mode = os.environ.get("CHAM_S1_H2", "1") if self.h2 else "0"
        self.s1_h2 = mode in ("1", "a")
        self.dm_f16 = self.s1_h2
        self.s1_h2_fwd = mode == "a"
        self.tf_random_seed = int(params.get('tf_random_seed', 42))
        meta = params['articles_metadata']
        self.ace = torch.from_numpy(ace).to(dev)
        self.created = torch.from_numpy(np.ascontiguousarray(meta['created_at_ts'], dtype=np.int64)).to(dev)
        def meta_column(n):
            a = np.asarray(meta[n])
            if n in L.meta_is_float:
                return np.ascontiguousarray(a, dtype=np.float32).view(np.int32).astype(np.int64)
            if acfg[n]['type'] == 'numerical' and not np.issubdtype(a.dtype, np.integer) and not np.array_equal(a, np.round(a)):
                raise ValueError("article feature %r holds non-integer values but its config says dtype %r: declare it "
                                 "{'type': 'numerical', 'dtype': 'float'}" % (n, acfg[n].get('dtype')))
            return a.astype(np.int64)
        if L.meta_names:
            mc = np.stack([meta_column(n) for n in L.meta_names])
        else:
            mc = np.zeros((1, self.n_items), np.int64)
        self.meta_cat = torch.from_numpy(np.ascontiguousarray(mc)).to(dev)
        self.ctx_desc = torch.from_numpy(L.ctx_descriptors()).to(dev)
        self.ctx_emb_groups, self.item_emb_groups = L.ctx_emb_groups(), L.item_emb_groups()
        segs, singles = L.item_segments()
        self.item_segs, self.n_item_segs = torch.from_numpy(np.ascontiguousarray(segs)).to(dev), int(segs.shape[0])
        self.item_singles, self.n_item_singles = torch.from_numpy(np.ascontiguousarray(singles)).to(dev), int(singles.shape[0])
        self.item_lds = L.Fi * 4 * 8 <= 64 * 1024
        self.item_desc = torch.from_numpy(L.item_descriptors()).to(dev)
        self.gemm_ws = torch.empty(64 << 20, dtype=torch.float32, device=dev)
        self.colsum_ws = torch.empty(4 << 20, dtype=torch.float32, device=dev)
        self.side_stream = lane_stream(dev, "side", 0)
        self._side_raw = self.side_stream.cuda_stream
        self.gemm_ws_side = torch.empty(32 << 20, dtype=torch.float32, device=dev)
        self.colsum_ws_side = torch.empty(2 << 20, dtype=torch.float32, device=dev)
        self.wgrad_aux = os.environ.get("CHAM_WGRAD_AUX", "1") == "1"
        self.aux_stream = lane_stream(dev, "aux", 0)
        self._aux_raw = self.aux_stream.cuda_stream
        self.gemm_ws_aux = torch.empty(16 << 20, dtype=torch.float32, device=dev)
        self.colsum_ws_aux = torch.empty(2 << 20, dtype=torch.float32, device=dev)
        self.head_split = os.environ.get("CHAM_HEAD_SPLIT", "1") == "1"
        self.overlap = os.environ.get("CHAM_OVERLAP", "1") == "1"
        self.compact = os.environ.get("CHAM_COMPACT", "1") == "1"
        self.p3_w2_splits = 32
        self.w2_main_rows = 131072
        self.rnn_coop_rows = 131072 if (L.cell == 'ugrnn' and L.Hp == 256 and not L.rnn_stepwise) else -1
        self._rnn_coop_ws = {}
        self.presample = os.environ.get("CHAM_PRESAMPLE", "1") == "1"
        self.upload_stream = lane_stream(dev, "upload")
        self.pinned = _PinnedRing()
        self.sumsq = torch.zeros(1024, dtype=torch.float32, device=dev)
        self.b16 = self.gemm_dtype == 'bf16'
        self.shadow, self._shadow_key, self.weights_version = {}, None, 0
        if self.b16:
            if L.C % 128:
                raise ValueError("gemm_dtype='bf16' needs CAR_embedding_size % 128 == 0")
            for name in ('W2', 'Ws1', 'Ws2', 'Ws3'):
                r, c = L.entries[name].shape
                self.shadow[name] = torch.zeros(r, c, dtype=torch.bfloat16, device=dev)
                self.shadow[name + 'T'] = torch.zeros(c, r, dtype=torch.bfloat16, device=dev)
        self.b16_dma = self.gemm_dtype == 'bf16' and L.C % 256 == 0
        self.dm_fused_b16 = self.gemm_dtype == 'bf16' and L.entries['Ws1'].shape == (L.C, 128) and L.C % 64 == 0
        if self.p3:
            C_ = L.C
            npl, pdt = (2, torch.float16) if self.h2 else (3, torch.bfloat16)
            self.w2p = torch.zeros(npl, C_, C_, dtype=pdt, device=dev)
            self.w2tp = torch.zeros(npl, C_, C_, dtype=pdt, device=dev)
            if self.h2:
                self.sc_w2 = torch.zeros(8, dtype=torch.float32, device=dev)
                self.sc_ws1n = torch.zeros(8, dtype=torch.float32, device=dev)
                self.sc_unit = torch.tensor([16384.0, 1.0 / 16384.0, 1.0, 0, 0, 0, 0, 0], dtype=torch.float32, device=dev)
            self.dm_fused = L.entries['Ws1'].shape == (C_, 128) and C_ % 64 == 0
            self.ws1p = torch.zeros(3, C_, 128, dtype=torch.bfloat16, device=dev)
            if self.h2:
                self.ws1h = torch.zeros(2, C_, 128, dtype=torch.float16, device=dev)
        self._plans = {}
        self.max_plans = 24
        self.plan_bytes_budget = 128 << 30
        self.profile = None
        self.dp_rank, self.dp_world, self.dp_allreduce, self.dp_sharded = 0, 1, None, None
        self.dp_early_bucket, self.dp_gather_slots, self.dp_mode, self.dp_active = None, None, 'allreduce', False

    def view(self, flat, name):
        cache = self._views.get(id(flat))
        if cache is None or cache[0] is not flat:
            cache = self._views[id(flat)] = (flat, {})
        v = cache[1].get(name)
        if v is None:
            e = self.layout.entries[name]
            v = cache[1][name] = flat[e.offset:e.offset + int(np.prod(e.shape))].view(*e.shape)
        return v

    def p(self, name):
        return self.view(self.flat, name)

    def g(self, name):
        return self.view(self.grads, name)

    def logical_weights(self):
        return self.layout.unpack(self.flat.cpu().numpy())

    def logical_grads(self):
        return self.layout.unpack(self.grads.cpu().numpy())

    def load_logical_weights(self, logical):
        self.flat.copy_(torch.from_numpy(self.layout.pack(logical)))
        self.weights_version += 1

    def shadows_stale(self):
        return (self.b16 or self.p3) and (self.global_step, self.weights_version) != self._shadow_key

    def refresh_shadows(self):
        if not self.shadows_stale():
            return
        key = (self.global_step, self.weights_version)
        if self.h2:
            C = self.layout.C
            check(self.lib.cham_split2h(ptr(self.p('W2')), C, C, C, ptr(self.w2p), C * C, C, ptr(self.w2tp), C * C, C, ptr(self.sc_w2), 1, _stream()),
                  "cham_split2h")
            k1 = self.layout.entries['Ws1'].shape[1]
            check(self.lib.cham_h2_scale_rownorm(ptr(self.p('Ws1')), C, k1, k1, None, ptr(self.sc_ws1n), _stream()), "cham_h2_scale_rownorm")
        elif self.p3:
            C = self.layout.C
            check(self.lib.cham_split3(ptr(self.p('W2')), C, C, C, ptr(self.w2p), C * C, C, ptr(self.w2tp), C * C, C, _stream()), "cham_split3")
        if self.p3:
            C = self.layout.C
            if self.dm_fused:
                check(self.lib.cham_split3(ptr(self.p('Ws1')), C, 128, 128, ptr(self.ws1p), C * 128, 128, None, 0, 0, _stream()), "cham_split3")
                if self.dm_f16:
                    check(self.lib.cham_split2h(ptr(self.p('Ws1')), C, 128, 128, ptr(self.ws1h), C * 128, 128, None, 0, 0, ptr(self.sc_ws1n), 0,
                                                _stream()), "cham_split2h")
        if self.b16:
            for name in ('W2', 'Ws1', 'Ws2', 'Ws3'):
                r, c = self.layout.entries[name].shape
                check(self.lib.cham_cast_b16(ptr(self.p(name)), r, c, ptr(self.shadow[name]), ptr(self.shadow[name + 'T']), _stream()),
                      "cham_cast_b16")
        self._shadow_key = key

    def state_dict(self):
        m, v = self.m, self.v
        if getattr(self, 'dp_gather_slots', None) is not None:
            m, v = self.dp_gather_slots(m, v)
        return {'flat': self.flat.cpu(), 'm': m.cpu(), 'v': v.cpu(), 'global_step': self.global_step,
                'dp_mode': getattr(self, 'dp_mode', 'allreduce'), 'dp_world': self.dp_world, 'layout': self.layout.fingerprint()}

    def load_state_dict(self, sd):
        if sd.get('layout') is not None and sd['layout'] != self.layout.fingerprint():
            raise ValueError("checkpoint was written for a different parameter layout (feature config / rnn_cell / sizes changed)")
        if tuple(sd['flat'].shape) != tuple(self.flat.shape):
# ... 501 lines not shown
    def _batch_counts(self):
        ic = np.asarray(self.inputs['item_clicked'])
        nz = ic[ic != 0]
        return int(nz.shape[0]), int(np.unique(nz).shape[0])

    def feed(self, feed_dict):
        by_name = {(k.name if isinstance(k, Placeholder) else k): v for k, v in feed_dict.items()}
        self.feed_state(by_name['articles_recent_pop_norm'], by_name['pop_recent_items_buffer'])

    def feed_device_state(self, state):
        state.sync_to_current()
        self.articles_recent_pop_norm = state
        self.pop_recent_items_buffer = state
        self._dev_state = dict(buffer=state.buf_ids, pop_norm=state.pop_norm, last=state.buf_ids,
                               n_last=min(self.recent_clicks_for_normalization, state.buf_ids.numel()) if state.n_updates > 0 else 0,
                               device=True)

    def feed_state(self, pop_norm, buffer_ids):
        if getattr(pop_norm, 'is_device', False):
            return self.feed_device_state(pop_norm)
        self.articles_recent_pop_norm = pop_norm
        self.pop_recent_items_buffer = buffer_ids
        dev = self.rt.device
        buf = np.ascontiguousarray(buffer_ids, dtype=np.int64)
        nz = buf[buf != 0][: self.recent_clicks_for_normalization]
        self._dev_state = dict(
            buffer=torch.from_numpy(buf).to(dev, non_blocking=True),
            pop_norm=torch.from_numpy(np.ascontiguousarray(pop_norm, dtype=np.float32)).to(dev, non_blocking=True),
            last=torch.from_numpy(np.ascontiguousarray(nz)).to(dev, non_blocking=True), n_last=int(nz.shape[0]))

    def upload_batch(self, features, labels, global_features=None, global_labels=None, row_begin=0):
        L, dev = self.rt.layout, self.rt.device
        item_clicked = np.ascontiguousarray(features['item_clicked'], dtype=np.int64)
        B, T = item_clicked.shape
        gf = features if global_features is None else global_features
        gl = labels if global_labels is None else global_labels
        aci = np.concatenate([np.asarray(gf['item_clicked'], np.int64), np.asarray(gl['label_last_item'], np.int64).reshape(-1, 1)], 1)
        ssz = np.asarray(features['session_size'], dtype=np.int64).reshape(-1)
        seq_len = (ssz - 1).astype(np.int32)
        mask = (np.arange(T)[None, :] < seq_len[:, None])
        g_ssz = np.asarray(gf['session_size'], dtype=np.int64).reshape(-1)
        g_T = np.asarray(gf['item_clicked']).shape[1]
        sum_mask = float(np.minimum(np.maximum(g_ssz - 1, 0), g_T).sum())
        ets = np.ascontiguousarray(features['event_timestamp'], dtype=np.int64)
        max_ts = int(np.asarray(gf['event_timestamp']).max())
        cat = np.stack([np.asarray(features[n], np.int64).reshape(-1) for n in L.ctx_cat_names]) if L.ctx_cat_names \
            else np.zeros((1, B * T), np.int64)
        num = np.stack([np.asarray(features[n], np.float32).reshape(-1) for n in L.ctx_num_names]) if L.ctx_num_names \
            else np.zeros((1, B * T), np.float32)
        g_ets = ets if global_features is None else np.ascontiguousarray(gf['event_timestamp'], dtype=np.int64)
        label_next = np.ascontiguousarray(labels['label_next_item'], dtype=np.int64)
        mrows = mask.reshape(-1)
        pos = np.flatnonzero(mrows).astype(np.int32)
        P = int(pos.shape[0])
        host = dict(g_event_ts=g_ets, aci=aci, item_clicked=item_clicked, label_next=label_next, event_ts=ets, seq_len=seq_len)
        compacted = self.rt.compact and 0 < P < B * T
        if compacted:
            host.update(pos=pos, ic_rows=item_clicked.reshape(-1)[pos], ln_rows=label_next.reshape(-1)[pos], ets_rows=ets.reshape(-1)[pos],
                        mask=np.ones(P, np.uint8), cat=cat[:, pos], num=num[:, pos])
        else:
            host.update(mask=mrows.astype(np.uint8), cat=cat, num=num)
        d = dict(B=B, T=T, Bg=aci.shape[0], row_begin=row_begin, sum_mask=sum_mask, max_ts=max_ts, P=P if compacted else B * T, pos=None)
        d.update(self._h2d(host))
        if not compacted:
            d.update(ic_rows=d['item_clicked'].view(-1), ln_rows=d['label_next'].view(-1), ets_rows=d['event_ts'].view(-1))
        return d

    def _h2d(self, host):
        dev = self.rt.device
        main, up, ring = torch.cuda.current_stream(), self.rt.upload_stream, self.rt.pinned
        arrs = {k: np.ascontiguousarray(a) for k, a in host.items()}
        out = {}
        if ring is not None:
            offs, total = pack_offsets(arrs)
            ring.begin(total)
            arena = ring.bufs[ring.k]
            bytes_view = arena.numpy()
            for k, a in arrs.items():
                if a.nbytes:
                    bytes_view[offs[k]:offs[k] + a.nbytes] = a.reshape(-1).view(np.uint8)
            with torch.cuda.stream(up if up is not None else main):
                block = torch.empty(max(total, 256), dtype=torch.uint8, device=dev)
                block[:total].copy_(arena[:total], non_blocking=True)
            if up is not None:
                block.record_stream(main)
            for k, a in arrs.items():
                out[k] = block[offs[k]:offs[k] + a.nbytes].view(_TORCH_DTYPE[a.dtype.str]).view(a.shape)
            out['_block'], out['_total'] = block, total
            out['_layout'] = tuple((k, offs[k], a.dtype.str, a.shape) for k, a in arrs.items())
        else:
            for k, a in arrs.items():
                x = torch.from_numpy(a)
                if up is None:
                    out[k] = x.to(dev, non_blocking=True)
                    continue
                with torch.cuda.stream(up):
                    x = x.to(dev, non_blocking=True)
                x.record_stream(main)
                out[k] = x
        out['uploaded'] = torch.cuda.Event()
        out['uploaded'].record(up if up is not None else main)
        if ring is not None:
            ring.end(up if up is not None else main)
        return out

    def _neg_sample(self, pl, d, step, k, stream, which=None):
        rt, st, o = self.rt, self._dev_state, pl._samp[k]
        if which is not None:
            check(rt.lib.cham_neg_sample_dev(ptr(d['aci']), d['Bg'], d['T'] + 1, ptr(st['buffer']), st['buffer'].numel(),
                                             rt.tf_random_seed, ptr(rt.scalars), which, d['row_begin'], d['B'], self.negative_samples,
                                             self.negative_sample_from_buffer, ptr(o['neg_ids']), ptr(o['neg_slot']), ptr(o['pool']),
                                             ptr(o['canon']), ptr(o['meta']), ptr(pl.sampler_ws), pl.ws_bytes, stream), "cham_neg_sample_dev")
            return
        check(rt.lib.cham_neg_sample(ptr(d['aci']), d['Bg'], d['T'] + 1, ptr(st['buffer']), st['buffer'].numel(),
                                     rt.tf_random_seed, step, d['row_begin'], d['B'], self.negative_samples,
                                     self.negative_sample_from_buffer, ptr(o['neg_ids']), ptr(o['neg_slot']), ptr(o['pool']),
                                     ptr(o['canon']), ptr(o['meta']), ptr(pl.sampler_ws), pl.ws_bytes, stream), "cham_neg_sample")

    def presample(self, d):
        rt, state = self.rt, self.articles_recent_pop_norm
        if not (rt.presample and self.is_training and getattr(state, 'is_device', False) and state.stream is not None
                and self._dev_state is not None and self._dev_state.get('device')):
            return False
        pl = rt.plan(d['B'], d['T'], self.negative_samples, self.negative_sample_from_buffer, d['Bg'])
        k, step = 1 - pl._samp_cur, rt.global_step
        if not rt.capturing:
            state.stream.wait_event(pl.created)
            if d.get('uploaded') is not None:
                state.stream.wait_event(d['uploaded'])
            d['aci'].record_stream(state.stream)
        with torch.cuda.stream(state.stream):
            self._neg_sample(pl, d, step, k, state.stream.cuda_stream, which=1 if rt.capturing else None)
            ev = torch.cuda.Event()
            ev.record()
        d['_presampled'] = (pl, k, step, ev)
        return True

    def forward(self, d, step=None):
        depth = _roctx.depth()
        try:
            return self._forward(d, step)
        finally:
            _roctx.unwind(depth)

    def _forward(self, d, step):
        rt, lib, L = self.rt, self.rt.lib, self.rt.layout
        st = self._dev_state
        if st is None:
            raise RuntimeError("feed_state() must be called before every step (ItemsStateUpdaterHook.before_run)")
        B, T, N = d['B'], d['T'], self.negative_samples
        pl = rt.plan(B, T, N, self.negative_sample_from_buffer, d['Bg'])
        self._plan, self._d = pl, d
        pl.used_p3 = False
        check(lib.cham_set_log_bases(self.elapsed_days_smooth_log_base, self.popularity_smooth_log_base), "cham_set_log_bases")
        if d.get('uploaded') is not None:
            torch.cuda.current_stream().wait_event(d['uploaded'])
        s = _stream()
        shadows_ev = None
        if rt.overlap and rt.shadows_stale():
            rt.side_stream.wait_stream(torch.cuda.current_stream())
            with torch.cuda.stream(rt.side_stream):
                rt.refresh_shadows()
                shadows_ev = torch.cuda.Event()
                shadows_ev.record()
        pos, BT, BTf, NC, pmax = d['pos'], d['P'], pl.BT, pl.NC, pl.pmax
        pl.pos, pl.P = pos, BT
        Rc = BT * NC; Rall = BT + Rc; RV = 2 * BT + pmax + 1
        C, Hp, Fc, Fi = L.C, L.Hp, L.Fc, L.Fi
        cell, NGH = (1 if L.cell == 'gru' else 0), L.NG * L.Hp
        if step is None:
            step = rt.global_step if self.is_training else self.eval_step_key(rt.global_step, self._eval_iter)
        p = rt.p
        _roctx.push("K0 negative sampling")
        ps = d.pop('_presampled', None)
        dsc = rt.dev_scalars
        if dsc:
            rt.set_step_scalars(step, d['max_ts'], d['sum_mask'], fields=3, stream=s)
        if ps is not None and ps[0] is pl and ps[2] == step and st.get('device'):
            pl.use_sampler_set(ps[1])
            if ps[3] is not None:
                torch.cuda.current_stream().wait_event(ps[3])
        else:
            self._neg_sample(pl, d, step, pl._samp_cur, s, which=0 if dsc else None)
        if rt.dp_mode in ('sparse', 'sparse_rs') and getattr(rt, 'dp_active', rt.dp_world > 1):
            n1 = d['aci'].numel()
            if getattr(pl, 'touched', None) is None or pl.touched.numel() < n1 + pmax + 1:
                pl.touched = torch.zeros(n1 + pmax + 1, dtype=torch.int32, device=rt.device)
            pl.touched[:n1].copy_(d['aci'].reshape(-1))
            pl.touched[n1:n1 + pmax].copy_(pl.pool)
            pl.touched[n1 + pmax:n1 + pmax + 1].zero_()
            rt.dp_touched = pl.touched[:n1 + pmax + 1]
        neg_ids, neg_slot = pl.neg_ids, pl.neg_slot
        if pos is not None:
            neg_ids, neg_slot = pl.neg_ids_c, pl.neg_slot_c
            check(lib.cham_rows_gather(ptr(pl.neg_ids), ptr(pos), BT, 2 * N, ptr(neg_ids), s), "cham_rows_gather")
            check(lib.cham_rows_gather(ptr(pl.neg_slot), ptr(pos), BT, N, ptr(neg_slot), s), "cham_rows_gather")
        pl.cur_neg_ids, pl.cur_neg_slot = neg_ids, neg_slot
        if getattr(pl, 'grouped_ev', None) is not None:
            torch.cuda.current_stream().wait_event(pl.grouped_ev)
        _roctx.pop(); _roctx.push("K1 features (gather, normalise, scale / center)")
        if dsc:
            check(lib.cham_step_ints_dev(ptr(d['ic_rows']), ptr(d['ln_rows']), ptr(pl.pool), ptr(d['ets_rows']), ptr(rt.scalars), BT, pmax, ptr(d['seq_len']),
                                         B, ptr(d['mask']), ptr(pl.ids_all), ptr(pl.ref_ts), ptr(pl.seq_len), ptr(pl.mask), s), "cham_step_ints_dev")
        else:
            check(lib.cham_step_ints(ptr(d['ic_rows']), ptr(d['ln_rows']), ptr(pl.pool), ptr(d['ets_rows']), int(d['max_ts']), BT, pmax, ptr(d['seq_len']),
                                     B, ptr(d['mask']), ptr(pl.ids_all), ptr(pl.ref_ts), ptr(pl.seq_len), ptr(pl.mask), s), "cham_step_ints")
        pl.grouped_ev = None
        if self.is_training:
            if rt.overlap:
                e_ids = torch.cuda.Event()
                e_ids.record()
                rt.side_stream.wait_event(e_ids)
                with torch.cuda.stream(rt.side_stream):
                    check(lib.cham_group_rows(ptr(pl.ids_all), RV, rt.item_id_bits, ptr(pl.perm), ptr(pl.seg), ptr(pl.group_ws),
                                              pl.group_ws.numel() * 4, _stream()), "cham_group_rows")
                    pl.grouped_ev = torch.cuda.Event()
                    pl.grouped_ev.record()
            else:
                check(lib.cham_group_rows(ptr(pl.ids_all), RV, rt.item_id_bits, ptr(pl.perm), ptr(pl.seg), ptr(pl.group_ws),
                                          pl.group_ws.numel() * 4, s), "cham_group_rows")
        check(lib.cham_item_dynamic_raw(ptr(pl.ids_all), ptr(pl.ref_ts), RV, ptr(rt.created), ptr(st['pop_norm']),
                                        ptr(pl.rec_raw), ptr(pl.nov_raw), s), "cham_item_dynamic_raw")
        if st['n_last'] > 0 and st.get('device') and dsc:
            check(lib.cham_norm_stats_from_buffer_dev(ptr(st['last']), st['n_last'], ptr(rt.scalars), ptr(rt.created),
                                                      ptr(st['pop_norm']), ptr(pl.stat_scratch), ptr(pl.stats), s),
                  "cham_norm_stats_from_buffer_dev")
        elif st['n_last'] > 0 and st.get('device'):
            check(lib.cham_norm_stats_from_buffer(ptr(st['last']), st['n_last'], d['max_ts'], ptr(rt.created),
                                                  ptr(st['pop_norm']), ptr(pl.stat_scratch), ptr(pl.stats), s),
                  "cham_norm_stats_from_buffer")
        elif st['n_last'] > 0:
            check(lib.cham_norm_stats_from_recent(ptr(st['last']), st['n_last'], d['max_ts'], ptr(rt.created),
                                                  ptr(st['pop_norm']), ptr(pl.stat_scratch), ptr(pl.stats), s),
                  "cham_norm_stats_from_recent")
        else:
            check(lib.cham_row_weights(ptr(pl.ids_all), 2 * BT, ptr(neg_slot), BT * N, pmax, ptr(pl.pool),
                                       ptr(pl.w_rows), pl.w_rows[2 * BT:].data_ptr(), s), "cham_row_weights")
            for g, (a, b) in enumerate([(0, BT), (BT, 2 * BT), (2 * BT, RV)]):
                check(lib.cham_norm_stats_from_rows(pl.rec_raw[a:].data_ptr(), pl.nov_raw[a:].data_ptr(),
                                                    pl.w_rows[a:].data_ptr(), b - a, pl.stats[g].data_ptr(), s),
                      "cham_norm_stats_from_rows")
        check(lib.cham_ctx_assemble(ptr(d['cat']), ptr(d['num']), BT, ptr(rt.ctx_desc), Fc, ptr(rt.flat), ptr(p('gamma_ctx')),
                                    ptr(p('beta_ctx')), ptr(pl.Xc_raw), ptr(pl.Xc_s), s), "cham_ctx_assemble")
        if rt.item_lds:
            check(lib.cham_item_assemble_lds(ptr(pl.ids_all), RV, BT, 2 * BT, ptr(rt.meta_cat), rt.n_items, ptr(rt.ace), L.D,
                                             ptr(pl.rec_raw), ptr(pl.nov_raw), ptr(pl.stats), ptr(rt.item_desc), Fi, ptr(rt.item_segs),
                                             rt.n_item_segs, ptr(rt.item_singles) if rt.n_item_singles else None, rt.n_item_singles,
                                             ptr(rt.flat), ptr(p('gamma_item')), ptr(p('beta_item')), ptr(pl.Xi_raw), ptr(pl.Xi_s), s),
                  "cham_item_assemble_lds")
        else:
            check(lib.cham_item_assemble(ptr(pl.ids_all), RV, BT, 2 * BT, ptr(rt.meta_cat), rt.n_items, ptr(rt.ace), L.D,
                                         ptr(pl.rec_raw), ptr(pl.nov_raw), ptr(pl.stats), ptr(rt.item_desc), Fi, ptr(rt.flat),
                                         ptr(p('gamma_item')), ptr(p('beta_item')), ptr(pl.Xi_raw), ptr(pl.Xi_s), s),
                  "cham_item_assemble")
        if shadows_ev is not None:
            torch.cuda.current_stream().wait_event(shadows_ev)
        else:
            rt.refresh_shadows()
        _roctx.pop(); _roctx.push("K2 PreCAR + CAR, K3 recurrent branch (side lane)")
        drop = self.is_training and self.keep_prob < 1.0
        head_split = rt.head_split and rt.overlap and BT * NC > rt.w2_main_rows
        if drop:
            pl.dropout_buffers(rt)
            keep, Fw, e1, e2 = float(self.keep_prob), Fc + Fi, L.entries['W1c'], L.entries['W1i']
            assert e2.offset == e1.offset + e1.size
            W1 = rt.flat[e1.offset:e2.offset + e2.size].view(Fw, C)
            gW1 = rt.grads[e1.offset:e2.offset + e2.size].view(Fw, C)

            def dropout(x, y, rows, cols, ld, site_first, site_rest, group, posmap, col_split=None, col_shift=0):
                check(lib.cham_dropout(ptr(x), ptr(y), rows, cols, ld, keep, rt.tf_random_seed, step & 0xFFFFFFFF, site_first, site_rest,
                                       group, ptr(posmap), T, d['row_begin'], cols if col_split is None else col_split, col_shift,
                                       _stream()), "cham_dropout")
            self._drop = dict(fn=dropout, W1=W1, gW1=gW1, Fw=Fw)
            check(lib.cham_dense_rows(ptr(pl.Xc_s), Fc, ptr(pl.Xi_s), Fi, BT, N, pmax, ptr(neg_slot), ptr(pl.Xd), s), "cham_dense_rows")
            dropout(pl.Xd, pl.Xd, BT, Fw, Fw, 16, 16, 1, pos, Fc, Fc - L.f_ctx)
            dropout(pl.Xd[BT:], pl.Xd[BT:], Rc, Fw, Fw, 17, 18, NC, pos, Fc, Fc - L.f_ctx)
            rt.gemm(pl.Xd, W1, pl.Z1, BT, C, Fw, Fw, C, C, bias=p('b1'), act=ACT_LEAKY)
        else:
            self._drop = None
            rt.gemm(pl.Xc_s, p('W1c'), pl.U, BT, C, Fc, Fc, C, C, bias=p('b1'))
            rt.gemm(pl.Xi_s, p('W1i'), pl.V, RV, C, Fi, Fi, C, C)
            if not head_split:
                check(lib.cham_combine_fwd(ptr(pl.U), ptr(pl.V), C, BT, N, pmax, ptr(neg_slot), ptr(pl.Z1), 0, BT, s), "cham_combine_fwd")
        if not head_split:
            rt.gemm(pl.Z1, p('W2'), pl.Z2, BT, C, C, C, C, C, bias=p('b2'), act=ACT_TANH)
        rt.fork()
        with rt.side():
            if head_split:
                if not drop:
                    check(lib.cham_combine_fwd(ptr(pl.U), ptr(pl.V), C, BT, N, pmax, ptr(neg_slot), ptr(pl.Z1), 0, BT, _stream()), "cham_combine_fwd")
                rt.gemm(pl.Z1, p('W2'), pl.Z2, BT, C, C, C, C, C, bias=p('b2'), act=ACT_TANH)
            x, ldx, K = pl.Z2, C, C
            if pos is not None:
                pl.Z2f.zero_()
                check(lib.cham_rows_scatter(ptr(pl.Z2), ptr(pos), BT, C, ptr(pl.Z2f), _stream()), "cham_rows_scatter")
                x = pl.Z2f
            for l in range(L.L):
                rt.gemm(x, p('rnn%d/Wx' % l), pl.xproj[l], BTf, NGH, K, ldx, NGH, NGH, bias=p('rnn%d/b' % l))
                if L.rnn_stepwise:
                    pl.h_state.zero_()
                    for t in range(T):
                        rt.gemm(pl.h_state, p('rnn%d/Wh' % l), pl.zh, B, 2 * Hp, Hp, Hp, 2 * Hp, 2 * Hp, force_f32=True)
                        check(lib.cham_ugrnn_point_fwd(ptr(pl.xproj[l]), ptr(pl.zh), ptr(pl.seq_len), B, T, t, Hp, ptr(pl.h_state),
                                                       ptr(pl.rnn_out[l]), ptr(pl.hprev[l]), ptr(pl.G[l]), ptr(pl.Cc[l]), _stream()),
                              "cham_ugrnn_point_fwd")
                elif 0 < Rc <= rt.rnn_coop_rows and B <= 1024:
                    ws = rt.rnn_coop_ws(B)
                    check(lib.cham_ugrnn_fwd_coop(ptr(pl.xproj[l]), ptr(p('rnn%d/Wh' % l)), ptr(pl.seq_len), B, T, Hp, ptr(pl.rnn_out[l]),
                                                  ptr(pl.hprev[l]), ptr(pl.G[l]), ptr(pl.Cc[l]), ptr(ws), ws.numel(), _stream()), "cham_ugrnn_fwd_coop")
                else:
                    check(lib.cham_rnn_fwd(cell, ptr(pl.xproj[l]), ptr(p('rnn%d/Wh' % l)), ptr(pl.seq_len), B, T, Hp,
                                           ptr(pl.rnn_out[l]), ptr(pl.hprev[l]), ptr(pl.G[l]), ptr(pl.Cc[l]), ptr(pl.R[l]),
                                           ptr(pl.RH[l]), _stream()), "cham_rnn_fwd")
                x, ldx, K = pl.rnn_out[l], Hp, Hp
                if drop:
                    dropout(pl.rnn_out[l], pl.rnn_drop[l], BTf, Hp, Hp, 20 + l, 20 + l, 1, None)
                    x = pl.rnn_drop[l]
            if pos is not None:
                check(lib.cham_rows_gather(ptr(x), ptr(pos), BT, Hp, ptr(pl.rnn_c), _stream()), "cham_rows_gather")
                x = pl.rnn_c
            rt.gemm(x, p('Wf1'), pl.FC1, BT, 512, Hp, Hp, 512, 512, bias=p('bf1'), act=ACT_LEAKY)
            fc1 = pl.FC1
            if drop:
                dropout(pl.FC1, pl.FC1d, BT, 512, 512, 19, 19, 1, pos)
                fc1 = pl.FC1d
            rt.gemm(fc1, p('Wf2'), pl.pred, BT, C, 512, 512, C, C, bias=p('bf2'), act=ACT_TANH)
        if rt.b16:
            sh = rt.shadow
            if drop:
                rt.gemm(pl.Xd[BT:], self._drop['W1'], pl.Z1f[BT:], Rc, C, Fc + Fi, Fc + Fi, C, C, bias=p('b1'), act=ACT_LEAKY)
                check(lib.cham_cast_b16(pl.Z1f[BT:].data_ptr(), Rc, C, ptr(pl.Z1c), None, s), "cham_cast_b16")
            else:
                check(lib.cham_combine_fwd_b16(ptr(pl.U), ptr(pl.V), C, BT, N, pmax, ptr(neg_slot), ptr(pl.Z1c), s), "cham_combine_fwd_b16")
            rt.gemm_b16(pl.Z1c, C, 0, sh['W2T'], C, 1, pl.Z2c, C, 0, Rc, C, C, bias=p('b2'), act=ACT_TANH, dma=rt.b16_dma)
            rt.join()
            check(lib.cham_mul_rows_b16(ptr(pl.Z2c), ptr(pl.pred), C, BT, NC, ptr(pl.Mc), s), "cham_mul_rows_b16")
            rt.gemm_b16(pl.Mc, C, 0, sh['Ws1T'], C, 1, pl.S1, 128, 0, Rc, 128, C, bias=p('bs1'), act=ACT_LEAKY)
            rt.gemm_b16(pl.S1, 128, 0, sh['Ws2T'], 128, 1, pl.S2, 64, 0, Rc, 64, 128, bias=p('bs2'), act=ACT_LEAKY)
            rt.gemm_b16(pl.S2, 64, 0, sh['Ws3T'], 64, 1, pl.S3, 32, 0, Rc, 32, 64, bias=p('bs3'), act=ACT_LEAKY)
            softmax_fwd = lib.cham_score_softmax_fwd_b16
        else:
            use_p3 = pl.used_p3 = rt.p3 and not drop and Rc > 0
            if drop:
                rt.gemm(pl.Xd[BT:], self._drop['W1'], pl.Z1[BT:], Rc, C, Fc + Fi, Fc + Fi, C, C, bias=p('b1'), act=ACT_LEAKY)
            elif use_p3 and rt.h2:
                check(lib.cham_h2_scale_absmax(ptr(pl.U), BT * C, ptr(pl.V), RV * C, ptr(pl.sc_z1), s), "cham_h2_scale_absmax")
                check(lib.cham_combine_fwd_h2b(ptr(pl.U), ptr(pl.V), C, BT, N, pmax, ptr(neg_slot), ptr(pl.Z1p), pl.z1_ps, ptr(pl.sc_z1), 1 if pl.z1_tiles else 0, s),
                      "cham_combine_fwd_h2")
            elif use_p3:
                check(lib.cham_combine_fwd_p3(ptr(pl.U), ptr(pl.V), C, BT, N, pmax, ptr(neg_slot), ptr(pl.Z1p), pl.p3_ps, s), "cham_combine_fwd_p3")
            else:
                check(lib.cham_combine_fwd(ptr(pl.U), ptr(pl.V), C, BT, N, pmax, ptr(neg_slot), ptr(pl.Z1), BT, Rc, s), "cham_combine_fwd")
            if use_p3 and rt.h2:
                rt.gemm_h2(pl.Z1p, pl.z1_ps, C, pl.sc_z1, rt.w2tp, C * C, C, rt.sc_w2, 0, pl.Z2[BT:], C, Rc, C, C, bias=p('b2'), act=ACT_TANH, a_tiles=pl.z1_tiles)
            elif use_p3:
                rt.gemm_p3(pl.Z1p, pl.p3_ps, C, rt.w2tp, C * C, C, 0, pl.Z2[BT:], C, Rc, C, C, bias=p('b2'), act=ACT_TANH)
            else:
                rt.gemm(pl.Z1[BT:], p('W2'), pl.Z2[BT:], Rc, C, C, C, C, C, bias=p('b2'), act=ACT_TANH)
            rt.join()
            _roctx.pop(); _roctx.push("K5 scorer, softmax, loss")
            Z2c = pl.Z2[BT:Rall]
            rt.gemm(Z2c, p('Ws1'), pl.S1, Rc, 128, C, C, 128, 128, bias=p('bs1'), act=ACT_LEAKY, rowscale=pl.pred, ldrs=C, rs_div=NC,
                    h2scales=(rt.sc_unit, rt.sc_ws1n) if rt.s1_h2_fwd else None)
            rt.gemm(pl.S1, p('Ws2'), pl.S2, Rc, 64, 128, 128, 64, 64, bias=p('bs2'), act=ACT_LEAKY)
            rt.gemm(pl.S2, p('Ws3'), pl.S3, Rc, 32, 64, 64, 32, 32, bias=p('bs3'), act=ACT_LEAKY)
            softmax_fwd = lib.cham_score_softmax_fwd
        check(softmax_fwd(ptr(pl.S3), 32, ptr(p('Ws4')), ptr(p('bs4')), BT, N, float(self.softmax_temperature),
                          ptr(pl.mask), ptr(pl.logits), ptr(pl.probs), ptr(pl.nll), self.novelty_reg_factor,
                          ptr(neg_ids), ptr(st['pop_norm']), ptr(pl.nov_aux), s), "cham_score_softmax_fwd")
        def loss_kernels(s):
            check(lib.cham_sumsq_partial(ptr(rt.flat), L.n_reg, ptr(rt.sumsq), s), "cham_sumsq_partial")
            if dsc:
                check(lib.cham_loss_finalize_dev(ptr(pl.nll), BT, ptr(rt.scalars), ptr(rt.sumsq), float(self.reg_weight_decay), ptr(pl.loss), s),
                      "cham_loss_finalize_dev")
            else:
                check(lib.cham_loss_finalize(ptr(pl.nll), BT, d['sum_mask'], ptr(rt.sumsq), float(self.reg_weight_decay), ptr(pl.loss), s),
                      "cham_loss_finalize")
        if getattr(self, '_defer_loss', False) and rt.overlap and rt.loss_side:
            e_nll = torch.cuda.Event(); e_nll.record()
            rt.side_stream.wait_event(e_nll)
            with torch.cuda.stream(rt.side_stream):
                loss_kernels(_stream())
        else:
            loss_kernels(s)
        _roctx.pop()
        self.total_loss = pl.loss
        if not self.is_training and st.get('device'):
            self.articles_recent_pop_norm.note_consumed(d['aci'])
        return pl

    def backward(self):
        rt, lib, L = self.rt, self.rt.lib, self.rt.layout
        pl, d = self._plan, self._d
        check(lib.cham_set_log_bases(self.elapsed_days_smooth_log_base, self.popularity_smooth_log_base), "cham_set_log_bases")
        s = _stream()
        B, T, N = pl.B, pl.T, pl.N
        pos, BT, BTf, NC, pmax = pl.pos, pl.P, pl.BT, pl.NC, pl.pmax
        Rc = BT * NC; Rall = BT + Rc; RV = 2 * BT + pmax + 1
        neg_ids, neg_slot = pl.cur_neg_ids, pl.cur_neg_slot
        C, Hp, Fc, Fi = L.C, L.Hp, L.Fc, L.Fi
        cell, NGH = (1 if L.cell == 'gru' else 0), L.NG * L.Hp
        p, g = rt.p, rt.g
        main_stream, on = torch.cuda.current_stream(), rt.overlap
        b16 = rt.b16
        sh = rt.shadow
        drop = self._drop
        dropout = drop['fn'] if drop else None
        use_p3 = getattr(pl, 'used_p3', False)

        def mark():
            if not on:
                return None
            ev = torch.cuda.Event(); ev.record()
            return ev

        import contextlib

        @contextlib.contextmanager
        def side(*events):
            if not on:
                yield
                return
            for ev in events:
                rt.side_stream.wait_event(ev)
            with torch.cuda.stream(rt.side_stream):
                yield

        def main_wait(ev):
            if on:
                main_stream.wait_event(ev)

        @contextlib.contextmanager
        def aux(*events):
            for ev in events:
                rt.aux_stream.wait_event(ev)
            with torch.cuda.stream(rt.aux_stream):
                yield
        e_auxdone = None

        e_start = mark()
        if on and rt.loss_side:
            with side(e_start):
                rt.grads[:L.emb_end].zero_()
        else:
            rt.grads[:L.emb_end].zero_()
            e_start = mark()
        if rt.dev_scalars:
            check((lib.cham_score_softmax_bwd_b16_dev if b16 else lib.cham_score_softmax_bwd_dev)(
                ptr(pl.S3), 32, ptr(p('Ws4')), ptr(pl.probs), ptr(pl.mask), BT, N, float(self.softmax_temperature), ptr(rt.scalars),
                ptr(pl.ds), ptr(pl.dS3), self.novelty_reg_factor, ptr(neg_ids), ptr(self._dev_state['pop_norm']), ptr(pl.logits),
                ptr(pl.nov_aux), s), "cham_score_softmax_bwd_dev")
        else:
            check((lib.cham_score_softmax_bwd_b16 if b16 else lib.cham_score_softmax_bwd)(
                ptr(pl.S3), 32, ptr(p('Ws4')), ptr(pl.probs), ptr(pl.mask), BT, N, float(self.softmax_temperature), d['sum_mask'],
                ptr(pl.ds), ptr(pl.dS3), self.novelty_reg_factor, ptr(neg_ids), ptr(self._dev_state['pop_norm']), ptr(pl.logits),
                ptr(pl.nov_aux), s), "cham_score_softmax_bwd")
        if self._dev_state.get('device'):
            self.articles_recent_pop_norm.note_consumed(d['aci'])
        if b16:
            rt.gemm_b16(pl.dS3, 32, 0, sh['Ws3'], 32, 1, pl.dS2, 64, 0, Rc, 64, 32, dref=pl.S2, ldr=64, dact=ACT_LEAKY)
            rt.gemm_b16(pl.dS2, 64, 0, sh['Ws2'], 64, 1, pl.dS1, 128, 0, Rc, 128, 64, dref=pl.S1, ldr=128, dact=ACT_LEAKY)
            Z2c, dZ2c = pl.Z2c[:Rc], pl.dZ2c[:Rc]
        else:
            rt.gemm(pl.dS3, p('Ws3'), pl.dS2, Rc, 64, 32, 32, 32, 64, transB=1, dref=pl.S2, ldr=64, dact=ACT_LEAKY)
            rt.gemm(pl.dS2, p('Ws2'), pl.dS1, Rc, 128, 64, 64, 64, 128, transB=1, dref=pl.S1, ldr=128, dact=ACT_LEAKY)
            if not (use_p3 and rt.dm_fused and 32 <= NC <= 256):
                pl.ensure_rows('dZ2')
            Z2c, dZ2c = pl.Z2[BT:Rall], pl.dZ2[BT:Rall]
        h2 = use_p3 and rt.h2
        if h2:
            check(lib.cham_h2_scale_rownorm2(ptr(pl.dS1), Rc, pl.dS1.shape[1], pl.dS1.shape[1], rt.sc_ws1n.data_ptr() + 8, ptr(pl.sc_dz2),
                                             ptr(pl.sc_ds1), s), "cham_h2_scale_rownorm2")
        e_dS1 = mark()
        dm_fused = use_p3 and rt.dm_fused and 32 <= NC <= 256
        dm_fused_b16 = b16 and rt.dm_fused_b16 and 32 <= NC <= 256
        if dm_fused_b16:
            pass
        elif b16:
            rt.gemm_b16(pl.dS1, 128, 0, sh['Ws1'], 128, 1, dZ2c, C, 0, Rc, C, 128)
        elif not dm_fused:
            rt.gemm(pl.dS1, p('Ws1'), dZ2c, Rc, C, 128, 128, 128, C, transB=1)
        def scorer_small_wgrads():
            if b16:
                rt.gemm_b16(pl.S1, 128, 1, pl.dS2, 64, 0, g('Ws2'), 64, 1, 128, 64, Rc, splits=0)
                rt.colsum(pl.dS2, 64, Rc, 64, g('bs2'), b16=True)
                rt.gemm_b16(pl.S2, 64, 1, pl.dS3, 32, 0, g('Ws3'), 32, 1, 64, 32, Rc, splits=0)
                rt.colsum(pl.dS3, 32, Rc, 32, g('bs3'), b16=True)
                rt.colsum(pl.S3, 32, Rc, 32, g('Ws4'), w=pl.ds, b16=True)
            else:
                rt.gemm(pl.S1, pl.dS2, g('Ws2'), 128, 64, Rc, 128, 64, 64, transA=1, splits=0)
                rt.colsum(pl.dS2, 64, Rc, 64, g('bs2'))
                rt.gemm(pl.S2, pl.dS3, g('Ws3'), 64, 32, Rc, 64, 32, 32, transA=1, splits=0)
                rt.colsum(pl.dS3, 32, Rc, 32, g('bs3'))
                rt.colsum(pl.S3, 32, Rc, 32, g('Ws4'), w=pl.ds)
            rt.colsum(pl.ds, 1, Rc, 1, g('bs4'))
        crit_first = on and (not b16 or pos is not None)
        w2_main = bool(on and use_p3 and 0 < Rc <= rt.w2_main_rows)
        use_aux = bool(on and rt.wgrad_aux and use_p3 and not w2_main and not b16 and L.L == 1 and cell == 0 and not L.rnn_stepwise and not drop)
        def ws1_wgrad():
            if b16:
                rt.gemm_b16(pl.Mc, C, 1, pl.dS1, 128, 0, g('Ws1'), 128, 1, C, 128, Rc, splits=0)
                rt.colsum(pl.dS1, 128, Rc, 128, g('bs1'), b16=True)
            else:
                rt.gemm(Z2c, pl.dS1, g('Ws1'), C, 128, Rc, C, 128, 128, transA=1, rowscale=pl.pred, ldrs=C, rs_div=NC, splits=0,
                        h2scales=(rt.sc_unit, pl.sc_ds1) if (rt.s1_h2 and use_p3) else None)
                rt.colsum(pl.dS1, 128, Rc, 128, g('bs1'))
        with side(e_start, e_dS1):
            ws1_wgrad()
            if not crit_first:
                scorer_small_wgrads()
        if dm_fused:
            prof = rt.profile
            if prof is not None:
                e0, e1 = torch.cuda.Event(enable_timing=True), torch.cuda.Event(enable_timing=True)
                e0.record()
            if h2 and pl.dz2_tiles:
                f16 = rt.dm_f16
                check(lib.cham_dm_mulpred_h2_blk(ptr(pl.dS1), 128, 128, ptr(rt.ws1h if f16 else rt.ws1p), C * 128, ptr(pl.sc_ds1) if f16 else None,
                                                 ptr(rt.sc_ws1n) if f16 else None, ptr(Z2c), ptr(pl.pred), C, BT, N, ptr(pl.dZ2p), pl.dz2_ps, ptr(pl.sc_dz2),
                                                 ptr(pl.dpred), ptr(pl.b2part), s), "cham_dm_mulpred_h2_blk")
            elif h2:
                if rt.dm_f16:
                    check(lib.cham_dm_mulpred_h2h(ptr(pl.dS1), 128, 128, ptr(rt.ws1h), C * 128, ptr(pl.sc_ds1), ptr(rt.sc_ws1n), ptr(Z2c), ptr(pl.pred),
                                                  C, BT, N, ptr(pl.dZ2p), pl.dz2_ps, ptr(pl.sc_dz2), ptr(pl.dpred), ptr(pl.b2part), s), "cham_dm_mulpred_h2h")
                else:
                    check(lib.cham_dm_mulpred_h2(ptr(pl.dS1), 128, 128, ptr(rt.ws1p), C * 128, ptr(Z2c), ptr(pl.pred), C, BT, N, ptr(pl.dZ2p), pl.dz2_ps,
                                                 ptr(pl.sc_dz2), ptr(pl.dpred), ptr(pl.b2part), s), "cham_dm_mulpred_h2")
            else:
                check(lib.cham_dm_mulpred_p3(ptr(pl.dS1), 128, 128, ptr(rt.ws1p), C * 128, ptr(Z2c), ptr(pl.pred), C, BT, N, ptr(pl.dZ2p), pl.p3_ps,
                                             ptr(pl.dpred), ptr(pl.b2part), s), "cham_dm_mulpred_p3")
            if prof is not None:
                e1.record()
                prof.append(dict(M=Rc, N=C, K=128, transA=0, transB=1, splits=1, act=0, dref=False, dact=0, bias=False, rowscale=False, bf16=False,
                                 dmf=True, h2out=bool(h2), f16p=bool(h2 and rt.dm_f16), tile=0, epi=0, ev=(e0, e1)))
        elif dm_fused_b16:
            prof = rt.profile
            if prof is not None:
                e0, e1 = torch.cuda.Event(enable_timing=True), torch.cuda.Event(enable_timing=True)
                e0.record()
            check(lib.cham_dm_mulpred_b16(ptr(pl.dS1), 128, 128, ptr(sh['Ws1']), ptr(Z2c), ptr(pl.pred), C, BT, N, ptr(dZ2c), ptr(pl.dpred),
                                          ptr(pl.b2part), s), "cham_dm_mulpred_b16")
            if prof is not None:
                e1.record()
                prof.append(dict(M=Rc, N=C, K=128, transA=0, transB=1, splits=1, act=0, dref=False, dact=0, bias=False, rowscale=False, bf16=True,
                                 dmf=True, tile=0, epi=0, ev=(e0, e1)))
        elif h2:
            check(lib.cham_mulpred_bwd_h2(ptr(dZ2c), ptr(Z2c), ptr(pl.pred), C, BT, N, ptr(pl.dpred), ptr(pl.dZ2p), pl.dz2_ps, ptr(pl.b2part),
                                          ptr(pl.sc_dz2), s), "cham_mulpred_bwd_h2")
        elif use_p3:
            check(lib.cham_mulpred_bwd_p3(ptr(dZ2c), ptr(Z2c), ptr(pl.pred), C, BT, N, ptr(pl.dpred), ptr(pl.dZ2p), pl.p3_ps, ptr(pl.b2part), s),
                  "cham_mulpred_bwd_p3")
        else:
            check((lib.cham_mulpred_bwd_b16 if b16 else lib.cham_mulpred_bwd)(ptr(dZ2c), ptr(Z2c), ptr(pl.pred), C, BT, N, ptr(pl.dpred), s),
                  "cham_mulpred_bwd")
        e_dZ2c = mark()
        if b16:
            rt.gemm_b16(dZ2c, C, 0, sh['W2'], C, 1, pl.dZ1c, C, 0, Rc, C, C, dref=pl.Z1c, ldr=C, dact=ACT_LEAKY, dma=rt.b16_dma)
        def w2_wgrad_planes(splits):
            if h2:
                rt.gemm_h2(pl.Z1p, pl.z1_ps, C, pl.sc_z1, pl.dZ2p, pl.dz2_ps, C, pl.sc_dz2, 1, g('W2'), C, C, C, Rc, splits=splits,
                           a_tiles=pl.z1_tiles, b_tiles=pl.dz2_tiles)
            else:
                rt.gemm_p3(pl.Z1p, pl.p3_ps, C, pl.dZ2p, pl.p3_ps, C, 1, g('W2'), C, C, C, Rc, splits=splits)
        if h2:
            gsum = getattr(pl, 'gsum', None) if not drop else None
            rt.gemm_h2(pl.dZ2p, pl.dz2_ps, C, pl.sc_dz2, rt.w2p, C * C, C, rt.sc_w2, 0, pl.dZ1[BT:], C, Rc, C, C, dref_h=pl.Z1p, ldr=C, dact=ACT_LEAKY,
                       a_tiles=pl.dz2_tiles, dref_blocked=1 if pl.z1_tiles else 0, group_rows=NC, groupsum=gsum)
        elif use_p3:
            rt.gemm_p3(pl.dZ2p, pl.p3_ps, C, rt.w2p, C * C, C, 0, pl.dZ1[BT:], C, Rc, C, C, dref_h=pl.Z1p, ldr=C, dact=ACT_LEAKY)
        elif not b16 and Rc > 0:
            rt.gemm(pl.dZ2[BT:Rall], p('W2'), pl.dZ1[BT:Rall], Rc, C, C, C, C, C, transB=1, dref=pl.Z1[BT:Rall], ldr=C, dact=ACT_LEAKY)
        e_cdgrad = mark()
        e_w2main = None
        if w2_main:
            w2_wgrad_planes(0)
            e_w2main = mark()
        last = L.L - 1
        deferred_w2 = None
        with side(e_dZ2c):
            ss = _stream()
            rnn_y = (lambda l: pl.rnn_drop[l]) if drop else (lambda l: pl.rnn_out[l])

            def fc_wgrads():
                rt.gemm(pl.FC1d if drop else pl.FC1, pl.dpred, g('Wf2'), 512, C, BT, 512, C, C, transA=1, splits=0)
                rt.colsum(pl.dpred, C, BT, C, g('bf2'))
                rt.gemm(pl.rnn_c if pos is not None else rnn_y(last), pl.dFC1, g('Wf1'), Hp, 512, BT, Hp, 512, 512, transA=1, splits=0)
                rt.colsum(pl.dFC1, 512, BT, 512, g('bf1'))
                if crit_first:
                    scorer_small_wgrads()
                if rt.dp_early_bucket is not None and not self._accumulating:
                    rt.dp_early_bucket(rt.grads)
            rt.gemm(pl.dpred, p('Wf2'), pl.dFC1, BT, 512, C, C, C, 512, transB=1, dref=pl.FC1, ldr=512, dact=ACT_LEAKY)
            if drop:
                dropout(pl.dFC1, pl.dFC1, BT, 512, 512, 19, 19, 1, pos)
            if not crit_first:
                fc_wgrads()
            if pos is not None:
                rt.gemm(pl.dFC1, p('Wf1'), pl.drnn_c, BT, Hp, 512, 512, 512, Hp, transB=1)
                pl.drnn.zero_()
                check(lib.cham_rows_scatter(ptr(pl.drnn_c), ptr(pos), BT, Hp, ptr(pl.drnn), ss), "cham_rows_scatter")
            else:
                rt.gemm(pl.dFC1, p('Wf1'), pl.drnn, BT, Hp, 512, 512, 512, Hp, transB=1)
            if drop:
                dropout(pl.drnn, pl.drnn, BTf, Hp, Hp, 20 + last, 20 + last, 1, None)
            for l in range(last, -1, -1):
                if L.rnn_stepwise:
                    pl.carry.zero_()
                    for t in range(T - 1, -1, -1):
                        check(lib.cham_ugrnn_point_bwd(ptr(pl.drnn), ptr(pl.carry), ptr(pl.seq_len), B, T, t, Hp, ptr(pl.hprev[l]),
                                                       ptr(pl.G[l]), ptr(pl.Cc[l]), ptr(pl.dxproj), ptr(pl.dzs), ptr(pl.direct), ss),
                              "cham_ugrnn_point_bwd")
                        pl.carry.copy_(pl.direct)
                        rt.gemm(pl.dzs, p('rnn%d/Wh' % l), pl.carry, B, Hp, 2 * Hp, 2 * Hp, 2 * Hp, Hp, transB=1, accumulate=1, force_f32=True)
                elif 0 < Rc <= rt.rnn_coop_rows and B <= 1024:
                    ws = rt.rnn_coop_ws(B)
                    check(lib.cham_ugrnn_bwd_coop(ptr(pl.drnn), ptr(p('rnn%d/Wh' % l)), ptr(pl.seq_len), B, T, Hp, ptr(pl.hprev[l]), ptr(pl.G[l]),
                                                  ptr(pl.Cc[l]), ptr(pl.dxproj), ptr(ws), ws.numel(), ss), "cham_ugrnn_bwd_coop")
                else:
                    check(lib.cham_transpose_f32(ptr(p('rnn%d/Wh' % l)), Hp, 2 * Hp, ptr(pl.WhT), ss), "cham_transpose_f32")
                    if cell == 1:
                        check(lib.cham_transpose_f32(ptr(p('rnn%d/Wch' % l)), Hp, Hp, pl.WhT[2 * Hp:].data_ptr(), ss), "cham_transpose_f32")
                    check(lib.cham_rnn_bwd(cell, ptr(pl.drnn), ptr(pl.WhT), ptr(pl.seq_len), B, T, Hp, ptr(pl.hprev[l]), ptr(pl.G[l]),
                                           ptr(pl.Cc[l]), ptr(pl.R[l]), ptr(pl.dxproj), ss), "cham_rnn_bwd")
# ... 518 lines not shown
```

### include/chameleon_nar.h

```cpp
#ifndef CHAMELEON_NAR_H
#define CHAMELEON_NAR_H
#include <stddef.h>
#include <stdint.h>
#ifdef __cplusplus
extern "C" {
#endif

#define CHAM_ACT_NONE 0
#define CHAM_ACT_LEAKY 1
#define CHAM_ACT_TANH 2

size_t cham_neg_sample_workspace_bytes(int n_aci, int buf_size, int n_from_buffer);
int cham_neg_sample(const int64_t* aci, int Bg, int T1, const int64_t* buffer, int buf_size, uint32_t seed, uint32_t step,
                    int row_begin, int row_count, int N, int n_from_buffer, int64_t* neg_ids, int32_t* neg_slot,
                    int64_t* pool, int32_t* canon, int32_t* meta, void* workspace, size_t workspace_bytes, void* stream);

int cham_ctx_assemble(const int64_t* cat, const float* num, int R, const int64_t* desc, int F, const float* params,
                      const float* gamma, const float* beta, float* xraw, float* xs, void* stream);
int cham_set_log_bases(float elapsed_days_smooth_log_base, float popularity_smooth_log_base);

int cham_step_ints(const int64_t* ic_rows, const int64_t* ln_rows, const int64_t* pool, const int64_t* ets_rows, int64_t max_ts, int BT, int pmax,
                   const int32_t* seq_len_in, int B, const uint8_t* mask_in, int64_t* ids_all, int64_t* ref_ts, int32_t* seq_len, uint8_t* mask,
                   void* stream);

// ... 21 lines not shown
                        size_t workspace_bytes, void* stream);

int cham_emb_grad_scan(const float* dxs, int R, int F, int c0, int dim, const float* gamma, const int64_t* keysrc,
                       const int64_t* ids, int cardinality, float* table_grad, void* stream);
size_t cham_group_rows_workspace_bytes(int R);
size_t cham_group_rows_segments_len(int R);
int cham_group_rows(const int64_t* ids, int R, int key_bits, int32_t* perm, int32_t* seg, void* workspace, size_t workspace_bytes,
                    void* stream);
int cham_emb_grad_grouped(const float* dxs, int R, int F, int c0, int dim, const float* gamma, const int64_t* ids,
                          const int32_t* perm, const int32_t* seg, float* table_grad, void* stream);

int cham_dropout(const float* x, float* y, long rows, int cols, int ld, float keep_prob, uint32_t seed, uint32_t step,
                 int site_first, int site_rest, int group, const int32_t* pos, int T, int row_begin, int col_split, int col_shift,
                 void* stream);
int cham_dense_rows(const float* Xc_s, int Fc, const float* Xi_s, int Fi, int BT, int N, int pmax, const int32_t* neg_slot, float* X,
                    void* stream);

int cham_gemm_f32(const float* A, int lda, int transA, const float* B, int ldb, int transB, float* C, int ldc, int M, int N,
                  int K, const float* bias, int act, const float* dref, int ldr, int dact, const float* rowscale, int ldrs,
                  int rs_div, int accumulate, float* workspace, size_t workspace_bytes, int splits_hint, void* stream);

int cham_gemm_bf16(const float* A, int lda, int transA, const float* B, int ldb, int transB, float* C, int ldc, int M, int N,
                   int K, const float* bias, int act, const float* dref, int ldr, int dact, const float* rowscale, int ldrs,
                   int rs_div, int accumulate, float* workspace, size_t workspace_bytes, int splits_hint, void* stream);

int cham_gemm_f32x3(const float* A, int lda, int transA, const float* B, int ldb, int transB, float* C, int ldc, int M, int N,
                    int K, const float* bias, int act, const float* dref, int ldr, int dact, const float* rowscale, int ldrs,
                    int rs_div, int accumulate, float* workspace, size_t workspace_bytes, int splits_hint, void* stream);
void cham_gemm_f32x3_set_variant(int variant);
void cham_gemm_f32x3_launch_counts(long long* out8, int reset);

int cham_gemm_f32x2h(const float* A, int lda, int transA, const float* B, int ldb, int transB, float* C, int ldc, int M, int N, int K,
                     const float* bias, int act, const float* rowscale, int ldrs, int rs_div, int accumulate, float* workspace,
                     size_t workspace_bytes, int splits_hint, const float* sa_rec, const float* sb_rec, void* stream);

int cham_gemm_p3(const void* A, long long a_plane_stride, int lda, const void* B, long long b_plane_stride, int ldb, int tn, float* C,
                 int ldc, int M, int N, int K, const float* bias, int act, const void* dref_h, int ldr, int dact, int accumulate,
                 float* workspace, size_t workspace_bytes, int splits_hint, void* stream);

int cham_gemm_b16_dma(const void* A, int lda, const void* B, int ldb, int tn, void* C, int ldc, int M, int N, int K, const float* bias,
                      int act, const void* dref, int ldr, int dact, int accumulate, float* workspace, size_t workspace_bytes,
                      int splits_hint, void* stream);
void cham_gemm_p3_launch_counts(long long* out8, int reset);
int cham_gemm_b16_dma_set_nt_wide(int on);
int cham_split3(const float* X, int R, int Cc, int ld, void* dst, long long plane_stride, int ldd, void* dstT, long long plane_strideT,
                int lddT, void* stream);

int cham_h2_scale_absmax(const float* x0, size_t n0, const float* x1, size_t n1, void* rec, void* stream);
int cham_h2_scale_rownorm(const float* X, long R, int K, int ld, const float* factor, void* rec, void* stream);
int cham_h2_scale_rownorm2(const float* X, long R, int K, int ld, const float* factor, void* rec, void* rec_plain, void* stream);
int cham_split2h(const float* X, int R, int Cc, int ld, void* dst, long long plane_stride, int ldd, void* dstT, long long plane_strideT,
                 int lddT, void* rec, int recompute, void* stream);
int cham_gemm_h2(const void* A, long long a_plane_stride, int lda, const float* a_scale, const void* B, long long b_plane_stride, int ldb,
                 const float* b_scale, int tn, float* C, int ldc, int M, int N, int K, const float* bias, int act, const void* dref_h, int ldr,
                 int dact, int accumulate, float* workspace, size_t workspace_bytes, int splits_hint, void* stream);
void cham_gemm_h2_launch_counts(long long* out8, int reset);
int cham_gemm_h2_set_nt_wide(int on);
int cham_h2b_block_elements(void);
int cham_gemm_h2b(const void* A, long long a_plane_stride, int lda, const float* a_scale, const void* B, long long b_plane_stride, int ldb,
                  const float* b_scale, int tn, float* C, int ldc, int M, int N, int K, const float* bias, int act, const void* dref_h, int ldr,
                  int dact, int accumulate, float* workspace, size_t workspace_bytes, int splits_hint, int a_tiles, int b_tiles,
                  int dref_blocked, void* stream);
int cham_combine_fwd_h2b(const float* U, const float* V, int C, int BT, int N, int pmax, const int32_t* neg_slot, void* Z1p,
                         long long plane_stride, const void* scale_rec, int blocked, void* stream);
int cham_dm_mulpred_h2_blk(const float* dS1, int lds1, int K, const void* Wp, long long w_plane_stride, const void* ds1_scale_rec,
                           const void* w_scale_rec, const float* Z2c, const float* pred, int C, int BT, int N, void* dZ2p,
                           long long out_plane_stride, const void* out_scale_rec, float* dpred_pre, float* col_part, void* stream);
int cham_combine_fwd_h2(const float* U, const float* V, int C, int BT, int N, int pmax, const int32_t* neg_slot, void* Z1p,
                        long long plane_stride, const void* scale_rec, void* stream);
int cham_mulpred_bwd_h2(const float* dM, const float* Z2c, const float* pred, int C, int BT, int N, float* dpred_pre, void* dZ2p,
                        long long plane_stride, float* col_part, const void* scale_rec, void* stream);
int cham_dm_mulpred_h2(const float* dS1, int lds1, int K, const void* Wp, long long w_plane_stride, const float* Z2c, const float* pred,
                       int C, int BT, int N, void* dZ2p, long long out_plane_stride, const void* out_scale_rec, float* dpred_pre,
                       float* col_part, void* stream);
int cham_dm_mulpred_h2h(const float* dS1, int lds1, int K, const void* Wh, long long w_plane_stride, const void* ds1_scale_rec,
                        const void* w_scale_rec, const float* Z2c, const float* pred, int C, int BT, int N, void* dZ2p,
                        long long out_plane_stride, const void* out_scale_rec, float* dpred_pre, float* col_part, void* stream);
int cham_dm_mulpred_b16(const void* dS1, int lds1, int K, const void* Ws1b, const void* Z2c, const float* pred, int C, int BT, int N, void* dZ2c,
                        float* dpred_pre, float* col_part, void* stream);

int cham_combine_fwd_p3(const float* U, const float* V, int C, int BT, int N, int pmax, const int32_t* neg_slot, void* Z1p,
                        long long plane_stride, void* stream);
int cham_mulpred_bwd_p3(const float* dM, const float* Z2c, const float* pred, int C, int BT, int N, float* dpred_pre, void* dZ2p,
                        long long plane_stride, float* col_part, void* stream);

int cham_dm_mulpred_p3(const float* dS1, int lds1, int K, const void* Wp, long long w_plane_stride, const float* Z2c, const float* pred,
                       int C, int BT, int N, void* dZ2p, long long out_plane_stride, float* dpred_pre, float* col_part, void* stream);

int cham_gemm_b16(const void* A, int lda, int transA, const void* B, int ldb, int transB, void* C, int ldc, int out_f32, int M,
                  int N, int K, const float* bias, int act, const void* dref, int ldr, int dact, int accumulate, float* workspace,
                  size_t workspace_bytes, int splits_hint, void* stream);
void cham_gemm_b16_set_variant(int variant);
void cham_gemm_b16_launch_counts(long long* out8, int reset);

void cham_gemm_set_variant(int variant);
void cham_gemm_launch_counts(long long* out16, int reset);

int cham_combine_fwd(const float* U, const float* V, int C, int BT, int N, int pmax, const int32_t* neg_slot, float* Z1,
                     long row_begin, long row_count, void* stream);
size_t cham_combine_bwd_workspace_bytes(int C, int BT, int N, int pmax);
int cham_combine_bwd(const float* dpre, int C, int BT, int N, int pmax, const int32_t* neg_slot, float* dU, float* dV,
                     float* workspace, size_t workspace_bytes, void* stream);
size_t cham_gemm_h2_groupsum_bytes(int M, int N, int group_rows);
int cham_gemm_h2_dgrad_gs(const void* A, long long a_plane_stride, int lda, const float* a_scale, const void* B, long long b_plane_stride, int ldb,
                          const float* b_scale, float* C, int ldc, int M, int N, int K, const void* dref_h, int ldr, int a_tiles, int dref_blocked,
                          int group_rows, float* groupsum, size_t groupsum_bytes, void* stream);
int cham_combine_bwd_gs(const float* dpre, int C, int BT, int N, int pmax, const int32_t* neg_slot, float* dU, float* dV, float* workspace,
                        size_t workspace_bytes, const float* groupsum, size_t groupsum_bytes, void* stream);

int cham_combine_fwd_b16(const float* U, const float* V, int C, int BT, int N, int pmax, const int32_t* neg_slot, void* Z1c,
                         void* stream);
int cham_combine_bwd_b16(const float* dpre_in, const void* dpre_cand, int C, int BT, int N, int pmax, const int32_t* neg_slot,
                         float* dU, float* dV, float* workspace, size_t workspace_bytes, void* stream);
int cham_mulpred_bwd_b16(void* dM, const void* Z2c, const float* pred, int C, int BT, int N, float* dpred_pre, void* stream);
int cham_mul_rows_b16(const void* Z2c, const float* pred, int C, int BT, int NC, void* Mc, void* stream);
int cham_score_softmax_fwd_b16(const void* S3, int K3, const float* w4, const float* b4, int BT, int N, float tau,
                               const uint8_t* mask, float* logits, float* probs, float* nll, float novelty_reg_factor,
                               const int64_t* neg_ids, const float* pop_norm, float* nov_aux, void* stream);
int cham_score_softmax_bwd_b16(const void* S3, int K3, const float* w4, const float* probs, const uint8_t* mask, int BT, int N,
                               float tau, float sum_mask, float* ds, void* dS3, float novelty_reg_factor, const int64_t* neg_ids,
                               const float* pop_norm, const float* logits, const float* nov_aux, void* stream);
int cham_colsum_b16(const void* X, int ld, int R, int F, const float* w, float* out, int accumulate, float* workspace,
                    size_t workspace_bytes, void* stream);
int cham_cast_b16(const float* W, int R, int Cc, void* dst, void* dstT, void* stream);
int cham_upcast_b16(const void* src, size_t n, float* dst, void* stream);

int cham_rnn_fwd(int cell_kind, const float* xproj, const float* Wh, const int32_t* seq_len, int B, int T, int Hp, float* out,
                 float* hprev, float* G, float* Cc, float* R, float* RH, void* stream);
int cham_rnn_bwd(int cell_kind, const float* dout, const float* WhT, const int32_t* seq_len, int B, int T, int Hp,
                 const float* hprev, const float* G, const float* Cc, const float* R, float* dxproj, void* stream);
size_t cham_rnn_coop_workspace_bytes(int B, int Hp);
int cham_ugrnn_fwd_coop(const float* xproj, const float* Wh, const int32_t* seq_len, int B, int T, int Hp, float* out, float* hprev, float* G,
                        float* Cc, void* workspace, size_t workspace_bytes, void* stream);
int cham_ugrnn_bwd_coop(const float* dout, const float* Wh, const int32_t* seq_len, int B, int T, int Hp, const float* hprev, const float* G,
                        const float* Cc, float* dxproj, void* workspace, size_t workspace_bytes, void* stream);
int cham_rnn_coop_timeouts(const void* workspace, int B, int Hp, void* stream);
int cham_ugrnn_point_fwd(const float* xproj, const float* zh, const int32_t* seq_len, int B, int T, int t, int Hp, float* h,
                         float* out, float* hprev, float* G, float* Cc, void* stream);
int cham_ugrnn_point_bwd(const float* dout, const float* carry, const int32_t* seq_len, int B, int T, int t, int Hp,
                         const float* hprev, const float* G, const float* Cc, float* dxproj, float* dzs, float* direct,
                         void* stream);
int cham_transpose_f32(const float* in, int rows, int cols, float* out, void* stream);
int cham_rows_gather(const void* src, const int32_t* pos, long n_rows, int words, void* dst, void* stream);
int cham_rows_scatter(const void* src, const int32_t* pos, long n_rows, int words, void* dst, void* stream);

int cham_mulpred_bwd(float* dM, const float* Z2c, const float* pred, int C, int BT, int N, float* dpred_pre, void* stream);
int cham_score_softmax_fwd(const float* S3, int K3, const float* w4, const float* b4, int BT, int N, float tau,
                           const uint8_t* mask, float* logits, float* probs, float* nll, float novelty_reg_factor,
                           const int64_t* neg_ids, const float* pop_norm, float* nov_aux, void* stream);
int cham_score_softmax_bwd(const float* S3, int K3, const float* w4, const float* probs, const uint8_t* mask, int BT, int N,
                           float tau, float sum_mask, float* ds, float* dS3, float novelty_reg_factor, const int64_t* neg_ids,
                           const float* pop_norm, const float* logits, const float* nov_aux, void* stream);

int cham_rank_items(const float* probs, const int64_t* label_next, const int64_t* neg_ids, const uint8_t* mask, int BT, int N,
                    int64_t* pred_ids, float* pred_probs, int32_t* label_rank, void* stream);

size_t cham_state_workspace_bytes(int B, int buffer_size);
int cham_state_update(const int64_t* aci, const int64_t* event_ts, int B, int T, double buffer_hours, int64_t* buf_ids,
                      int64_t* buf_ts, int buffer_size, int32_t* recent_pop, float* pop_norm, int64_t* articles_pop, int n_items,
                      int for_norm, int32_t* n_valid, void* workspace, size_t workspace_bytes, void* stream);

int cham_sumsq_partial(const float* params, size_t n_reg, float* partial, void* stream);
int cham_loss_finalize(const float* nll, int BT, float sum_mask, const float* sumsq_partial, float lambda, float* loss,
                       void* stream);
int cham_adam_tf(float* params, const float* grads, float* m, float* v, size_t n, size_t n_reg, float lambda, float lr_t,
                 float beta1, float beta2, float eps, void* stream);
int cham_accumulate(float* acc, const float* x, size_t n, int first, void* stream);
int cham_loss_accumulate(float* acc, const float* loss, int first, void* stream);
size_t cham_colsum_workspace_bytes(int R, int F);
int cham_colsum(const float* X, int ld, int R, int F, const float* w, float* out, int accumulate, float* workspace,
                size_t workspace_bytes, void* stream);


int cham_step_scalars_bytes(void);
int cham_step_scalars_set(void* rec, uint32_t step, uint32_t step_next, int64_t max_ts, float sum_mask, float lr_t, int fields, void* stream);
int cham_neg_sample_dev(const int64_t* aci, int Bg, int T1, const int64_t* buffer, int buf_size, uint32_t seed, const void* scalars, int which,
                        int row_begin, int row_count, int N, int n_from_buffer, int64_t* neg_ids, int32_t* neg_slot, int64_t* pool, int32_t* canon,
                        int32_t* meta, void* workspace, size_t workspace_bytes, void* stream);
int cham_step_ints_dev(const int64_t* ic_rows, const int64_t* ln_rows, const int64_t* pool, const int64_t* ets_rows, const void* scalars, int BT,
                       int pmax, const int32_t* seq_len_in, int B, const uint8_t* mask_in, int64_t* ids_all, int64_t* ref_ts, int32_t* seq_len,
                       uint8_t* mask, void* stream);
int cham_norm_stats_from_buffer_dev(const int64_t* buffer_ids, int n_prefix, const void* scalars, const int64_t* created, const float* pop_norm,
                                    float* scratch, float* stats, void* stream);
int cham_score_softmax_bwd_dev(const float* S3, int K3, const float* w4, const float* probs, const uint8_t* mask, int BT, int N, float tau,
                               const void* scalars, float* ds, float* dS3, float novelty_reg_factor, const int64_t* neg_ids, const float* pop_norm,
                               const float* logits, const float* nov_aux, void* stream);
int cham_score_softmax_bwd_b16_dev(const void* S3, int K3, const float* w4, const float* probs, const uint8_t* mask, int BT, int N, float tau,
                                   const void* scalars, float* ds, void* dS3, float novelty_reg_factor, const int64_t* neg_ids,
                                   const float* pop_norm, const float* logits, const float* nov_aux, void* stream);
int cham_loss_finalize_dev(const float* nll, int BT, const void* scalars, const float* sumsq_partial, float lambda, float* loss, void* stream);
int cham_adam_tf_dev(float* params, const float* grads, float* m, float* v, size_t n, size_t n_reg, float lambda, const void* scalars,
                     float beta1, float beta2, float eps, void* stream);

#ifdef __cplusplus
}
#endif
#endif
```

Baseline: 34950.

## Fuse scorer MLP tail, softmax and its backward into one kernel

Adds a scorer_tail kernel that runs the S2/S3 GEMMs, the final scoring layer, softmax and NLL in a single launch per 256-row tile with weights staged in LDS. In training it also computes ds, dS3 and dS2 in the same pass, and in mode "2" additionally dS1 and the h2 row-norm scale fold. This removes several separate GEMM and softmax launches along with the global round trips of their intermediates. Shared softmax and scale helpers are moved into a common header, and the path is on by default when NC fits the tile.

```diff
diff --git a/chameleon_recsys_amd/_lib.py b/chameleon_recsys_amd/_lib.py
--- a/chameleon_recsys_amd/_lib.py
+++ b/chameleon_recsys_amd/_lib.py
@@ -102,6 +102,11 @@
     "cham_rows_gather": (c_int, [P, P, c_long, c_int, P, P]),
     "cham_rows_scatter": (c_int, [P, P, c_long, c_int, P, P]),
     "cham_mulpred_bwd": (c_int, [P, P, P, c_int, c_int, c_int, P, P]),
+    "cham_scorer_tail": (c_int, [P, P, P, P, P, P, P, c_int, c_int, c_float, P, P, P, P, P, P, c_float, P, P, P, c_int, c_float, P, P, P, P, P, P,
+                                 P, P]),
+    "cham_scorer_tail_dev": (c_int, [P, P, P, P, P, P, P, c_int, c_int, c_float, P, P, P, P, P, P, c_float, P, P, P, c_int, P, P, P, P, P, P, P,
+                                     P, P]),
+    "cham_scorer_tail_rows": (c_int, []),
     "cham_score_softmax_fwd": (c_int, [P, c_int, P, P, c_int, c_int, c_float, P, P, P, P, c_float, P, P, P, P]),
     "cham_score_softmax_bwd": (c_int, [P, c_int, P, P, P, c_int, c_int, c_float, c_float, P, P, c_float, P, P, P, P, P]),
     "cham_rank_items": (c_int, [P, P, P, P, c_int, c_int, P, P, P, P]),
diff --git a/chameleon_recsys_amd/build.py b/chameleon_recsys_amd/build.py
--- a/chameleon_recsys_amd/build.py
+++ b/chameleon_recsys_amd/build.py
@@ -6,7 +6,7 @@
 HERE = os.path.dirname(os.path.abspath(__file__))
 CSRC = os.path.join(HERE, "csrc")
 LIB = os.path.join(HERE, "libchameleon_nar.so")
-SOURCES = ["gemm.hip", "gemm_x3.hip", "gemm_p3.hip", "gemm_h2.hip", "dm_fused.hip", "gemm_b16.hip", "sampler.hip", "features.hip", "scorer.hip", "rnn.hip", "rnn_coop.hip", "optim.hip", "state.hip"]
+SOURCES = ["gemm.hip", "gemm_x3.hip", "gemm_p3.hip", "gemm_h2.hip", "dm_fused.hip", "gemm_b16.hip", "sampler.hip", "features.hip", "scorer.hip", "scorer_tail.hip", "rnn.hip", "rnn_coop.hip", "optim.hip", "state.hip"]
 FLAGS = ["--offload-arch=gfx950", "-O3", "-std=c++17", "-fPIC", "-Wall", "-Wno-unused-function"]
 FLAGS += os.environ.get("CHAM_BUILD_DEFINES", "").split()
 
diff --git a/chameleon_recsys_amd/csrc/gemm_h2.hip b/chameleon_recsys_amd/csrc/gemm_h2.hip
--- a/chameleon_recsys_amd/csrc/gemm_h2.hip
+++ b/chameleon_recsys_amd/csrc/gemm_h2.hip
@@ -1,4 +1,5 @@
 #include "gemm_shared.h"
+#include "scorer_shared.h"
 
 typedef _Float16 half8 __attribute__((ext_vector_type(8)));
 typedef short h2_s16x4 __attribute__((ext_vector_type(4)));
@@ -520,28 +521,6 @@
     h2_epilogue<EPI, TM, TNN>(p, acc, m0, n0, wm0, wn0, 0, lane);
 }
 
-__device__ __forceinline__ void h2_finish_scale(H2Scale* rec, float bound) {
-    float s = 1.f, inv = 1.f;
-    if (bound > 0.f && bound < __builtin_inff()) {
-        int e;
-        (void)frexpf(bound, &e);
-        int k = 15 - e;
-        k = k < -110 ? -110 : (k > 110 ? 110 : k);
-        s = ldexpf(1.f, k); inv = ldexpf(1.f, -k);
-    }
-    rec->scale = s; rec->inv = inv; rec->bound = bound;
-}
-
-__device__ __forceinline__ float h2_block_max(float v, float* red) {
-    v = wave_max(v);
-    const int lane = threadIdx.x & 63, w = threadIdx.x >> 6;
-    if (lane == 0) red[w] = v;
-    __syncthreads();
-    float t = 0.f;
-    for (int i = 0; i < (int)(blockDim.x >> 6); ++i) t = fmaxf(t, red[i]);
-    __syncthreads();
-    return t;
-}
 
 __global__ __launch_bounds__(256) void k_h2_scale_absmax(const float* __restrict__ x0, size_t n0, const float* __restrict__ x1, size_t n1,
                                                          H2Scale* __restrict__ rec) {
@@ -592,20 +571,9 @@
 #pragma unroll
             for (int u = 0; u < 4; ++u) v[u] = reinterpret_cast<const float4*>(X + (size_t)(r + u * stride) * ld)[hl];
 #pragma unroll
-            for (int u = 0; u < 4; ++u) {
-                float s = v[u].x * v[u].x + v[u].y * v[u].y + v[u].z * v[u].z + v[u].w * v[u].w;
-#pragma unroll
-                for (int o = 16; o > 0; o >>= 1) s += __shfl_xor(s, o, 64);
-                mx = fmaxf(mx, s);
-            }
-        }
-        for (; r < R; r += stride) {
-            const float4 v = reinterpret_cast<const float4*>(X + (size_t)r * ld)[hl];
-            float s = v.x * v.x + v.y * v.y + v.z * v.z + v.w * v.w;
-#pragma unroll
-            for (int o = 16; o > 0; o >>= 1) s += __shfl_xor(s, o, 64);
-            mx = fmaxf(mx, s);
-        }
+            for (int u = 0; u < 4; ++u) mx = fmaxf(mx, h2_rownorm_sq128(v[u]));
+        }
+        for (; r < R; r += stride) mx = fmaxf(mx, h2_rownorm_sq128(reinterpret_cast<const float4*>(X + (size_t)r * ld)[hl]));
     } else {
         for (long r = wave_g; r < R; r += nwaves) {
             float s = 0.f;
@@ -614,19 +582,7 @@
         }
     }
     mx = h2_block_max(mx, red);
-    if (threadIdx.x == 0) {
-        atomicMax(&rec->max_bits, __float_as_uint(mx));
-        __threadfence();
-        last = atomicAdd(&rec->ticket, 1u) == gridDim.x - 1 ? 1u : 0u;
-        if (last) {
-            __threadfence();
-            const float sq = __uint_as_float(atomicMax(&rec->max_bits, 0u));
-            const float b = sqrtf(sq) * (factor ? *factor : 1.f) * 1.0009765625f;
-            h2_finish_scale(rec, b);
-            if (rec_plain) h2_finish_scale(rec_plain, sqrtf(sq) * 1.0009765625f);
-            rec->max_bits = 0u; rec->ticket = 0u;
-        }
-    }
+    if (threadIdx.x == 0) h2_rownorm_fold(mx, rec, rec_plain, factor, gridDim.x, &last);
 }
 
 extern "C" int cham_h2_scale_absmax(const float* x0, size_t n0, const float* x1, size_t n1, void* rec, void* stream) {
diff --git a/chameleon_recsys_amd/csrc/scorer.hip b/chameleon_recsys_amd/csrc/scorer.hip
--- a/chameleon_recsys_amd/csrc/scorer.hip
+++ b/chameleon_recsys_amd/csrc/scorer.hip
@@ -1,4 +1,5 @@
 #include "common.h"
+#include "scorer_shared.h"
 
 __device__ __forceinline__ int cand_vrow(int bt, int c, int BT, int N, int pmax, const int* __restrict__ neg_slot) {
     if (c == 0) return BT + bt;
@@ -452,52 +453,8 @@
                                                            float* __restrict__ nov_aux , float inv_log2_base) {
     const int lane = threadIdx.x & 63, bt = blockIdx.x * 4 + (threadIdx.x >> 6);
     if (bt >= BT) return;
-    const int NC = N + 1;
-    float w[K3];
-#pragma unroll
-    for (int k = 0; k < K3; ++k) w[k] = w4[k];
-    const float bias = b4[0];
-    float mx = -INFINITY;
-    for (int c = lane; c < NC; c += 64) {
-        const T* r = S3 + ((size_t)bt * NC + c) * K3;
-        float s = 0.f;
-#pragma unroll
-        for (int k = 0; k < K3 / 4; ++k) { const float4 x = ld4(r + 4 * k); s += x.x * w[4 * k] + x.y * w[4 * k + 1] + x.z * w[4 * k + 2] + x.w * w[4 * k + 3]; }
-        s += bias;
-        logits[(size_t)bt * NC + c] = s;
-        mx = fmaxf(mx, s * inv_tau);
-    }
-    mx = wave_max(mx);
-    float sum = 0.f;
-    for (int c = lane; c < NC; c += 64) {
-        const float e = expf(logits[(size_t)bt * NC + c] * inv_tau - mx);
-        probs[(size_t)bt * NC + c] = e;
-        sum += e;
-    }
-    sum = wave_sum(sum);
-    const float inv = 1.f / sum;
-    for (int c = lane; c < NC; c += 64) probs[(size_t)bt * NC + c] *= inv;
-    float novterm = 0.f;
-    if (nov_factor > 0.f) {
-        float mxn = -INFINITY;
-        for (int c = lane; c < NC; c += 64)
-            if (c > 0) mxn = fmaxf(mxn, logits[(size_t)bt * NC + c] * inv_tau);
-        mxn = wave_max(mxn);
-        float sn = 0.f, acc = 0.f;
-        for (int c = lane; c < NC; c += 64)
-            if (c > 0) {
-                const float e = expf(logits[(size_t)bt * NC + c] * inv_tau - mxn);
-                sn += e;
-                acc += e * (-log2f(pop_norm[neg_ids[(size_t)bt * N + (c - 1)]]) * inv_log2_base);
-            }
-        sn = wave_sum(sn); acc = wave_sum(acc);
-        novterm = acc / sn;
-        if (lane == 0) { nov_aux[(size_t)bt * 3] = mxn; nov_aux[(size_t)bt * 3 + 1] = sn; nov_aux[(size_t)bt * 3 + 2] = novterm; }
-    }
-    if (lane == 0) {
-        const float z0 = logits[(size_t)bt * NC] * inv_tau;
-        nll[bt] = mask[bt] ? -((z0 - mx) - logf(sum)) - nov_factor * novterm : 0.f;
-    }
+    score_softmax_fwd_click<K3, K3, T>(S3 + (size_t)bt * (N + 1) * K3, w4, b4, bt, N, inv_tau, mask, logits, probs, nll, nov_factor, neg_ids,
+                                       pop_norm, nov_aux, inv_log2_base, lane);
 }
 
 template <int K3, typename T>
@@ -514,25 +471,8 @@
     if (row >= (size_t)BT * NC) return;
     if (sc) scale = 1.0f / (tau * sc->sum_mask);
     const int bt = (int)(row / NC), c = (int)(row % NC);
-    float g = mask[bt] ? (probs[row] - (c == 0 ? 1.f : 0.f)) * scale : 0.f;
-    if (nov_factor > 0.f && c > 0 && mask[bt]) {
-        const float q = expf(logits[row] * inv_tau - nov_aux[(size_t)bt * 3]) / nov_aux[(size_t)bt * 3 + 1];
-        const float nov_c = -log2f(pop_norm[neg_ids[(size_t)bt * N + (c - 1)]]) * inv_log2_base;
-        g -= nov_factor * scale * q * (nov_c - nov_aux[(size_t)bt * 3 + 2]);
-    }
-    ds[row] = g;
-    const T* r = S3 + row * K3;
-    T* o = dS3 + row * K3;
-#pragma unroll
-    for (int k = 0; k < K3 / 4; ++k) {
-        const float4 x = ld4(r + 4 * k);
-        float4 y;
-        y.x = g * w4[4 * k] * act_bwd_from_out(x.x, ACT_LEAKY);
-        y.y = g * w4[4 * k + 1] * act_bwd_from_out(x.y, ACT_LEAKY);
-        y.z = g * w4[4 * k + 2] * act_bwd_from_out(x.z, ACT_LEAKY);
-        y.w = g * w4[4 * k + 3] * act_bwd_from_out(x.w, ACT_LEAKY);
-        st4(o + 4 * k, y);
-    }
+    score_softmax_bwd_row<K3, T>(row, bt, c, S3 + row * K3, dS3 + row * K3, w4, probs, mask, N, scale, ds, nov_factor, neg_ids, pop_norm,
+                                 logits, inv_tau, nov_aux, inv_log2_base);
 }
 
 
diff --git a/chameleon_recsys_amd/csrc/scorer_shared.h b/chameleon_recsys_amd/csrc/scorer_shared.h
--- /dev/null
+++ b/chameleon_recsys_amd/csrc/scorer_shared.h
@@ -0,0 +1,125 @@
+#pragma once
+#include "common.h"
+
+template <int K3, int LD3, typename T>
+__device__ __forceinline__ void score_softmax_fwd_click(const T* S3p, const float* __restrict__ w4, const float* __restrict__ b4, int bt, int N,
+                                                        float inv_tau, const unsigned char* __restrict__ mask, float* __restrict__ logits,
+                                                        float* __restrict__ probs, float* __restrict__ nll, float nov_factor,
+                                                        const int64_t* __restrict__ neg_ids, const float* __restrict__ pop_norm,
+                                                        float* __restrict__ nov_aux , float inv_log2_base, int lane) {
+    const int NC = N + 1;
+    float w[K3];
+#pragma unroll
+    for (int k = 0; k < K3; ++k) w[k] = w4[k];
+    const float bias = b4[0];
+    float mx = -INFINITY;
+    for (int c = lane; c < NC; c += 64) {
+        const T* r = S3p + (size_t)c * LD3;
+        float s = 0.f;
+#pragma unroll
+        for (int k = 0; k < K3 / 4; ++k) { const float4 x = ld4(r + 4 * k); s += x.x * w[4 * k] + x.y * w[4 * k + 1] + x.z * w[4 * k + 2] + x.w * w[4 * k + 3]; }
+        s += bias;
+        logits[(size_t)bt * NC + c] = s;
+        mx = fmaxf(mx, s * inv_tau);
+    }
+    mx = wave_max(mx);
+    float sum = 0.f;
+    for (int c = lane; c < NC; c += 64) {
+        const float e = expf(logits[(size_t)bt * NC + c] * inv_tau - mx);
+        probs[(size_t)bt * NC + c] = e;
+        sum += e;
+    }
+    sum = wave_sum(sum);
+    const float inv = 1.f / sum;
+    for (int c = lane; c < NC; c += 64) probs[(size_t)bt * NC + c] *= inv;
+    float novterm = 0.f;
+    if (nov_factor > 0.f) {
+        float mxn = -INFINITY;
+        for (int c = lane; c < NC; c += 64)
+            if (c > 0) mxn = fmaxf(mxn, logits[(size_t)bt * NC + c] * inv_tau);
+        mxn = wave_max(mxn);
+        float sn = 0.f, acc = 0.f;
+        for (int c = lane; c < NC; c += 64)
+            if (c > 0) {
+                const float e = expf(logits[(size_t)bt * NC + c] * inv_tau - mxn);
+                sn += e;
+                acc += e * (-log2f(pop_norm[neg_ids[(size_t)bt * N + (c - 1)]]) * inv_log2_base);
+            }
+        sn = wave_sum(sn); acc = wave_sum(acc);
+        novterm = acc / sn;
+        if (lane == 0) { nov_aux[(size_t)bt * 3] = mxn; nov_aux[(size_t)bt * 3 + 1] = sn; nov_aux[(size_t)bt * 3 + 2] = novterm; }
+    }
+    if (lane == 0) {
+        const float z0 = logits[(size_t)bt * NC] * inv_tau;
+        nll[bt] = mask[bt] ? -((z0 - mx) - logf(sum)) - nov_factor * novterm : 0.f;
+    }
+}
+
+template <int K3, typename T>
+__device__ __forceinline__ void score_softmax_bwd_row(size_t row, int bt, int c, const T* r, T* o, const float* __restrict__ w4,
+                                                      const float* __restrict__ probs, const unsigned char* __restrict__ mask, int N, float scale,
+                                                      float* __restrict__ ds, float nov_factor, const int64_t* __restrict__ neg_ids,
+                                                      const float* __restrict__ pop_norm, const float* __restrict__ logits, float inv_tau,
+                                                      const float* __restrict__ nov_aux, float inv_log2_base) {
+    float g = mask[bt] ? (probs[row] - (c == 0 ? 1.f : 0.f)) * scale : 0.f;
+    if (nov_factor > 0.f && c > 0 && mask[bt]) {
+        const float q = expf(logits[row] * inv_tau - nov_aux[(size_t)bt * 3]) / nov_aux[(size_t)bt * 3 + 1];
+        const float nov_c = -log2f(pop_norm[neg_ids[(size_t)bt * N + (c - 1)]]) * inv_log2_base;
+        g -= nov_factor * scale * q * (nov_c - nov_aux[(size_t)bt * 3 + 2]);
+    }
+    ds[row] = g;
+#pragma unroll
+    for (int k = 0; k < K3 / 4; ++k) {
+        const float4 x = ld4(r + 4 * k);
+        float4 y;
+        y.x = g * w4[4 * k] * act_bwd_from_out(x.x, ACT_LEAKY);
+        y.y = g * w4[4 * k + 1] * act_bwd_from_out(x.y, ACT_LEAKY);
+        y.z = g * w4[4 * k + 2] * act_bwd_from_out(x.z, ACT_LEAKY);
+        y.w = g * w4[4 * k + 3] * act_bwd_from_out(x.w, ACT_LEAKY);
+        st4(o + 4 * k, y);
+    }
+}
+
+__device__ __forceinline__ void h2_finish_scale(H2Scale* rec, float bound) {
+    float s = 1.f, inv = 1.f;
+    if (bound > 0.f && bound < __builtin_inff()) {
+        int e;
+        (void)frexpf(bound, &e);
+        int k = 15 - e;
+        k = k < -110 ? -110 : (k > 110 ? 110 : k);
+        s = ldexpf(1.f, k); inv = ldexpf(1.f, -k);
+    }
+    rec->scale = s; rec->inv = inv; rec->bound = bound;
+}
+
+__device__ __forceinline__ float h2_block_max(float v, float* red) {
+    v = wave_max(v);
+    const int lane = threadIdx.x & 63, w = threadIdx.x >> 6;
+    if (lane == 0) red[w] = v;
+    __syncthreads();
+    float t = 0.f;
+    for (int i = 0; i < (int)(blockDim.x >> 6); ++i) t = fmaxf(t, red[i]);
+    __syncthreads();
+    return t;
+}
+
+__device__ __forceinline__ float h2_rownorm_sq128(const float4 v) {
+    float s = v.x * v.x + v.y * v.y + v.z * v.z + v.w * v.w;
+#pragma unroll
+    for (int o = 16; o > 0; o >>= 1) s += __shfl_xor(s, o, 64);
+    return s;
+}
+
+__device__ __forceinline__ void h2_rownorm_fold(float mx, H2Scale* rec, H2Scale* rec_plain, const float* factor, unsigned nblocks, unsigned* last) {
+    atomicMax(&rec->max_bits, __float_as_uint(mx));
+    __threadfence();
+    *last = atomicAdd(&rec->ticket, 1u) == nblocks - 1 ? 1u : 0u;
+    if (*last) {
+        __threadfence();
+        const float sq = __uint_as_float(atomicMax(&rec->max_bits, 0u));
+        const float b = sqrtf(sq) * (factor ? *factor : 1.f) * 1.0009765625f;
+        h2_finish_scale(rec, b);
+        if (rec_plain) h2_finish_scale(rec_plain, sqrtf(sq) * 1.0009765625f);
+        rec->max_bits = 0u; rec->ticket = 0u;
+    }
+}
diff --git a/chameleon_recsys_amd/csrc/scorer_tail.hip b/chameleon_recsys_amd/csrc/scorer_tail.hip
--- /dev/null
+++ b/chameleon_recsys_amd/csrc/scorer_tail.hip
@@ -0,0 +1,306 @@
+#include "gemm_shared.h"
+#include "scorer_shared.h"
+
+namespace {
+
+constexpr int TAIL_ROWS = 256, TAIL_THREADS = 512;
+constexpr int LW2 = 68, LW3 = 33, LS3 = 36, LSC = 66, LSTG = 132;
+constexpr int OFF_W2 = 0, OFF_W3 = OFF_W2 + 128 * LW2, OFF_S3 = OFF_W3 + 64 * LW3, OFF_SC = OFF_S3 + TAIL_ROWS * LS3,
+              OFF_M1 = OFF_SC + 8 * 32 * LSC, OFF_RED = OFF_M1 + 8 * 64 * 2, TAIL_LDS_FLOATS = OFF_RED + 16;
+static_assert(16 * LSTG <= 32 * LSC, "the dS1 staging half-tile must fit the wave's scratch");
+static_assert((OFF_M1 & 1) == 0 && (OFF_S3 & 3) == 0, "alignment of the mask words / the float4 rows of S3");
+
+typedef __bf16 tail_bf16x8 __attribute__((ext_vector_type(8)));
+
+struct TailParams {
+    const float* S1; const float* Ws2; const float* bs2; const float* Ws3; const float* bs3; const float* w4; const float* b4;
+    int BT, N, PW;
+    float inv_tau, tau, scale, nov_factor, inv_log2_base;
+    const unsigned char* mask; const int64_t* neg_ids; const float* pop_norm;
+    float* S2; float* S3; float* logits; float* probs; float* nll; float* nov_aux;
+    const ChamStepScalars* sc;
+    float* ds; float* dS3; float* dS2; float* dS1;
+    const float* factor; H2Scale* rec; H2Scale* rec_plain;
+};
+
+__device__ __forceinline__ void split8(const float (&x)[8], tail_bf16x8& h, tail_bf16x8& m, tail_bf16x8& l) {
+#pragma unroll
+    for (int e = 0; e < 8; ++e) { __bf16 a, b, c; split3(x[e], a, b, c); h[e] = a; m[e] = b; l[e] = c; }
+}
+
+template <bool TRAIN>
+__global__ __launch_bounds__(TAIL_THREADS) void k_scorer_tail(TailParams p) {
+    extern __shared__ __attribute__((aligned(16))) float sm[];
+    float* W2s = sm + OFF_W2;
+    float* W3s = sm + OFF_W3;
+    float* S3b = sm + OFF_S3;
+    unsigned long long* M1 = reinterpret_cast<unsigned long long*>(sm + OFF_M1);
+    float* red = sm + OFF_RED;
+    __shared__ unsigned last;
+
+    const int NC = p.N + 1;
+    const int pos0 = blockIdx.x * p.PW;
+    const int PWv = min(p.PW, p.BT - pos0);
+    const int RW = PWv * NC;
+    const size_t r0 = (size_t)pos0 * NC;
+    const int tid = threadIdx.x, lane = tid & 63, fl = lane & 31, h = lane >> 5;
+    const int w = __builtin_amdgcn_readfirstlane(tid >> 6);
+    const bool active = w * 32 < RW;
+    float* scr = sm + OFF_SC + w * 32 * LSC;
+
+    for (int i = tid; i < 128 * 16; i += TAIL_THREADS) {
+        const int r = i >> 4, q = i & 15;
+        st4(W2s + r * LW2 + 4 * q, ld4(p.Ws2 + r * 64 + 4 * q));
+    }
+    for (int i = tid; i < 64 * 32; i += TAIL_THREADS) W3s[(i >> 5) * LW3 + (i & 31)] = p.Ws3[i];
+
+    const int lr = w * 32 + fl;
+    const bool rok = lr < RW;
+    float a1[64];
+    {
+        const float* s1 = p.S1 + (r0 + (rok ? lr : 0)) * 128;
+#pragma unroll
+        for (int q = 0; q < 32; ++q) {
+            const float4 v = rok ? ld4(s1 + 4 * q) : make_float4(0.f, 0.f, 0.f, 0.f);
+            a1[2 * q] = h ? v.y : v.x;
+            a1[2 * q + 1] = h ? v.w : v.z;
+        }
+        unsigned long long m1 = 0ull;
+#pragma unroll
+        for (int j = 0; j < 64; ++j) m1 |= (unsigned long long)(a1[j] > 0.f) << j;
+        M1[w * 64 + lane] = m1;
+    }
+    __syncthreads();
+
+    unsigned m2 = 0u;
+    if (active) {
+        floatx16 acc[2];
+#pragma unroll
+        for (int c = 0; c < 2; ++c)
+#pragma unroll
+            for (int e = 0; e < 16; ++e) acc[c][e] = 0.f;
+#pragma unroll
+        for (int j = 0; j < 64; ++j) {
+            const float* b = W2s + (2 * j + h) * LW2 + fl;
+#pragma unroll
+            for (int c = 0; c < 2; ++c) acc[c] = __builtin_amdgcn_mfma_f32_32x32x2f32(a1[j], b[32 * c], acc[c], 0, 0, 0);
+        }
+#pragma unroll
+        for (int c = 0; c < 2; ++c) {
+            const int col = 32 * c + fl;
+            const float bv = p.bs2[col];
+#pragma unroll
+            for (int e = 0; e < 16; ++e) {
+                const int row = (e & 3) + 8 * (e >> 2) + 4 * h;
+                const float v = act_fwd_c<ACT_LEAKY>(acc[c][e] + bv);
+                m2 |= (unsigned)(v > 0.f) << (c * 16 + e);
+                scr[row * LSC + col] = v;
+                if (w * 32 + row < RW) p.S2[(r0 + w * 32 + row) * 64 + col] = v;
+            }
+        }
+    }
+    __syncthreads();
+
+    if (active) {
+        floatx16 acc;
+#pragma unroll
+        for (int e = 0; e < 16; ++e) acc[e] = 0.f;
+#pragma unroll
+        for (int j = 0; j < 32; ++j)
+            acc = __builtin_amdgcn_mfma_f32_32x32x2f32(scr[fl * LSC + 2 * j + h], W3s[(2 * j + h) * LW3 + fl], acc, 0, 0, 0);
+        const float bv = p.bs3[fl];
+#pragma unroll
+        for (int e = 0; e < 16; ++e) {
+            const int row = (e & 3) + 8 * (e >> 2) + 4 * h;
+            const float v = act_fwd_c<ACT_LEAKY>(acc[e] + bv);
+            S3b[(w * 32 + row) * LS3 + fl] = v;
+            if (w * 32 + row < RW) p.S3[(r0 + w * 32 + row) * 32 + fl] = v;
+        }
+    }
+    __syncthreads();
+
+    for (int c = w; c < PWv; c += TAIL_THREADS / 64)
+        score_softmax_fwd_click<32, LS3, float>(S3b + c * NC * LS3, p.w4, p.b4, pos0 + c, p.N, p.inv_tau, p.mask, p.logits, p.probs, p.nll,
+                                                p.nov_factor, p.neg_ids, p.pop_norm, p.nov_aux, p.inv_log2_base, lane);
+    if constexpr (!TRAIN) return;
+    __syncthreads();
+
+    if (tid < RW) {
+        const float scale = p.sc ? 1.0f / (p.tau * p.sc->sum_mask) : p.scale;
+        const size_t row = r0 + tid;
+        float* r = S3b + tid * LS3;
+        score_softmax_bwd_row<32, float>(row, pos0 + tid / NC, tid % NC, r, r, p.w4, p.probs, p.mask, p.N, scale, p.ds, p.nov_factor,
+                                         p.neg_ids, p.pop_norm, p.logits, p.inv_tau, p.nov_aux, p.inv_log2_base);
+    }
+    __syncthreads();
+    for (int i = tid; i < RW * 8; i += TAIL_THREADS) st4(p.dS3 + (r0 + (i >> 3)) * 32 + 4 * (i & 7), ld4(S3b + (i >> 3) * LS3 + 4 * (i & 7)));
+
+    if (active) {
+        floatx16 acc[2];
+#pragma unroll
+        for (int c = 0; c < 2; ++c)
+#pragma unroll
+            for (int e = 0; e < 16; ++e) acc[c][e] = 0.f;
+#pragma unroll
+        for (int j = 0; j < 16; ++j) {
+            const float a = S3b[(w * 32 + fl) * LS3 + 2 * j + h];
+#pragma unroll
+            for (int c = 0; c < 2; ++c)
+                acc[c] = __builtin_amdgcn_mfma_f32_32x32x2f32(a, W3s[(32 * c + fl) * LW3 + 2 * j + h], acc[c], 0, 0, 0);
+        }
+#pragma unroll
+        for (int c = 0; c < 2; ++c) {
+            const int col = 32 * c + fl;
+#pragma unroll
+            for (int e = 0; e < 16; ++e) {
+                const int row = (e & 3) + 8 * (e >> 2) + 4 * h;
+                const float d = ((m2 >> (c * 16 + e)) & 1u) ? 1.f : 0.2f;
+                const float v = acc[c][e] * d + 0.f;
+                scr[row * LSC + col] = v;
+                if (w * 32 + row < RW) p.dS2[(r0 + w * 32 + row) * 64 + col] = v;
+            }
+        }
+    }
+    if (!p.dS1) return;
+    __syncthreads();
+
+    floatx16 acc[4];
+#pragma unroll
+    for (int c = 0; c < 4; ++c)
+#pragma unroll
+        for (int e = 0; e < 16; ++e) acc[c][e] = 0.f;
+    if (active) {
+        tail_bf16x8 ah[4], am[4], al[4];
+#pragma unroll
+        for (int t = 0; t < 4; ++t) {
+            float x[8];
+#pragma unroll
+            for (int e = 0; e < 8; ++e) x[e] = scr[fl * LSC + 16 * t + 8 * h + e];
+            split8(x, ah[t], am[t], al[t]);
+        }
+#pragma unroll
+        for (int c = 0; c < 4; ++c) {
+            const float* wr = W2s + (32 * c + fl) * LW2 + 8 * h;
+#pragma unroll
+            for (int t = 0; t < 4; ++t) {
+                float x[8];
+                const float4 u0 = ld4(wr + 16 * t), u1 = ld4(wr + 16 * t + 4);
+                x[0] = u0.x; x[1] = u0.y; x[2] = u0.z; x[3] = u0.w; x[4] = u1.x; x[5] = u1.y; x[6] = u1.z; x[7] = u1.w;
+                tail_bf16x8 bh, bm, bl;
+                split8(x, bh, bm, bl);
+                acc[c] = __builtin_amdgcn_mfma_f32_32x32x16_bf16(al[t], bh, acc[c], 0, 0, 0);
+                acc[c] = __builtin_amdgcn_mfma_f32_32x32x16_bf16(ah[t], bl, acc[c], 0, 0, 0);
+                acc[c] = __builtin_amdgcn_mfma_f32_32x32x16_bf16(am[t], bm, acc[c], 0, 0, 0);
+                acc[c] = __builtin_amdgcn_mfma_f32_32x32x16_bf16(am[t], bh, acc[c], 0, 0, 0);
+                acc[c] = __builtin_amdgcn_mfma_f32_32x32x16_bf16(ah[t], bm, acc[c], 0, 0, 0);
+                acc[c] = __builtin_amdgcn_mfma_f32_32x32x16_bf16(ah[t], bh, acc[c], 0, 0, 0);
+            }
+        }
+#pragma unroll
+        for (int e = 0; e < 16; ++e) {
+            const int row = (e & 3) + 8 * (e >> 2) + 4 * h;
+            const unsigned long long m = M1[w * 64 + row + 32 * (fl & 1)];
+#pragma unroll
+            for (int c = 0; c < 4; ++c) {
+                const float d = ((m >> (16 * c + (fl >> 1))) & 1ull) ? 1.f : 0.2f;
+                acc[c][e] = acc[c][e] * d + 0.f;
+            }
+        }
+    }
+    float mx = 0.f;
+#pragma unroll
+    for (int hf = 0; hf < 2; ++hf) {
+        __syncthreads();
+        if (active) {
+#pragma unroll
+            for (int e = 8 * hf; e < 8 * hf + 8; ++e) {
+                const int row = (e & 3) + 8 * ((e >> 2) - 2 * hf) + 4 * h;
+#pragma unroll
+                for (int c = 0; c < 4; ++c) scr[row * LSTG + 32 * c + fl] = acc[c][e];
+            }
+        }
+        __syncthreads();
+        if (active) {
+#pragma unroll
+            for (int rr = h; rr < 16; rr += 2) {
+                const float4 v = ld4(scr + rr * LSTG + 4 * fl);
+                const float s = h2_rownorm_sq128(v);
+                const int lrow = w * 32 + 16 * hf + rr;
+                if (lrow < RW) {
+                    st4(p.dS1 + (r0 + lrow) * 128 + 4 * fl, v);
+                    mx = fmaxf(mx, s);
+                }
+            }
+        }
+    }
+    if (p.rec) {
+        mx = h2_block_max(mx, red);
+        if (tid == 0) h2_rownorm_fold(mx, p.rec, p.rec_plain, p.factor, gridDim.x, &last);
+    }
+}
+
+int scorer_tail_launch(TailParams& p, int train, void* stream) {
+    const int NC = p.N + 1;
+    if (!p.S1 || !p.Ws2 || !p.bs2 || !p.Ws3 || !p.bs3 || !p.w4 || !p.b4 || !p.mask || !p.S2 || !p.S3 || !p.logits || !p.probs || !p.nll)
+        return -CHAM_ERR_ARG;
+    if (p.BT <= 0 || p.N < 1 || NC > TAIL_ROWS) return -CHAM_ERR_ARG;
+    if (p.nov_factor > 0.f && (!p.neg_ids || !p.pop_norm || !p.nov_aux)) return -CHAM_ERR_ARG;
+    if (((uintptr_t)p.S1 | (uintptr_t)p.Ws2 | (uintptr_t)p.dS3 | (uintptr_t)p.dS1) & 15) return -CHAM_ERR_ARG;
+    if (train) {
+        if (!p.ds || !p.dS3 || !p.dS2 || (p.rec && !p.dS1)) return -CHAM_ERR_ARG;
+        if (!p.sc && !(p.scale > 0.f)) return -CHAM_ERR_ARG;
+        if (p.rec && (((uintptr_t)p.rec | (uintptr_t)p.rec_plain) & 15 || p.rec == p.rec_plain)) return -CHAM_ERR_ARG;
+    } else {
+        p.rec = nullptr;
+    }
+    p.PW = TAIL_ROWS / NC;
+    const unsigned blocks = (unsigned)((p.BT + p.PW - 1) / p.PW);
+    const int smem = TAIL_LDS_FLOATS * 4;
+    auto k = train ? k_scorer_tail<true> : k_scorer_tail<false>;
+    CHAM_SET_DYNAMIC_LDS(k, smem);
+    hipLaunchKernelGGL(k, dim3(blocks), dim3(TAIL_THREADS), smem, (hipStream_t)stream, p);
+    CHAM_CHECK_LAUNCH();
+    return CHAM_OK;
+}
+
+int scorer_tail_entry(const float* S1, const float* Ws2, const float* bs2, const float* Ws3, const float* bs3, const float* w4, const float* b4,
+                      int BT, int N, float tau, const uint8_t* mask, float* S2, float* S3, float* logits, float* probs, float* nll,
+                      float novelty_reg_factor, const int64_t* neg_ids, const float* pop_norm, float* nov_aux, int train, float sum_mask,
+                      const void* scalars, float* ds, float* dS3, float* dS2, float* dS1, const float* factor, void* rec, void* rec_plain,
+                      void* stream) {
+    TailParams p;
+    p.S1 = S1; p.Ws2 = Ws2; p.bs2 = bs2; p.Ws3 = Ws3; p.bs3 = bs3; p.w4 = w4; p.b4 = b4;
+    p.BT = BT; p.N = N; p.PW = 1;
+    p.inv_tau = 1.0f / tau; p.tau = tau; p.scale = scalars ? 0.f : (train ? 1.0f / (tau * sum_mask) : 0.f);
+    p.nov_factor = novelty_reg_factor; p.inv_log2_base = g_cham_inv_log2_pop_base;
+    p.mask = mask; p.neg_ids = neg_ids; p.pop_norm = pop_norm;
+    p.S2 = S2; p.S3 = S3; p.logits = logits; p.probs = probs; p.nll = nll; p.nov_aux = nov_aux;
+    p.sc = reinterpret_cast<const ChamStepScalars*>(scalars);
+    p.ds = ds; p.dS3 = dS3; p.dS2 = dS2; p.dS1 = dS1;
+    p.factor = factor; p.rec = reinterpret_cast<H2Scale*>(rec); p.rec_plain = reinterpret_cast<H2Scale*>(rec_plain);
+    if (train && !scalars && !(sum_mask > 0.f)) return -CHAM_ERR_ARG;
+    return scorer_tail_launch(p, train, stream);
+}
+
+}
+
+extern "C" int cham_scorer_tail_rows() { return TAIL_ROWS; }
+
+extern "C" int cham_scorer_tail(const float* S1, const float* Ws2, const float* bs2, const float* Ws3, const float* bs3, const float* w4,
+                                const float* b4, int BT, int N, float tau, const uint8_t* mask, float* S2, float* S3, float* logits,
+                                float* probs, float* nll, float novelty_reg_factor, const int64_t* neg_ids, const float* pop_norm,
+                                float* nov_aux, int train, float sum_mask, float* ds, float* dS3, float* dS2, float* dS1,
+                                const float* factor, void* rec, void* rec_plain, void* stream) {
+    return scorer_tail_entry(S1, Ws2, bs2, Ws3, bs3, w4, b4, BT, N, tau, mask, S2, S3, logits, probs, nll, novelty_reg_factor, neg_ids,
+                             pop_norm, nov_aux, train, sum_mask, nullptr, ds, dS3, dS2, dS1, factor, rec, rec_plain, stream);
+}
+
+extern "C" int cham_scorer_tail_dev(const float* S1, const float* Ws2, const float* bs2, const float* Ws3, const float* bs3, const float* w4,
+                                    const float* b4, int BT, int N, float tau, const uint8_t* mask, float* S2, float* S3, float* logits,
+                                    float* probs, float* nll, float novelty_reg_factor, const int64_t* neg_ids, const float* pop_norm,
+                                    float* nov_aux, int train, const void* scalars, float* ds, float* dS3, float* dS2, float* dS1,
+                                    const float* factor, void* rec, void* rec_plain, void* stream) {
+    if (!scalars) return -CHAM_ERR_ARG;
+    return scorer_tail_entry(S1, Ws2, bs2, Ws3, bs3, w4, b4, BT, N, tau, mask, S2, S3, logits, probs, nll, novelty_reg_factor, neg_ids,
+                             pop_norm, nov_aux, train, 0.f, scalars, ds, dS3, dS2, dS1, factor, rec, rec_plain, stream);
+}
diff --git a/chameleon_recsys_amd/nar/nar_model.py b/chameleon_recsys_amd/nar/nar_model.py
--- a/chameleon_recsys_amd/nar/nar_model.py
+++ b/chameleon_recsys_amd/nar/nar_model.py
@@ -163,6 +163,7 @@
         if self.gemm_dtype not in ('f32', 'f32_native', 'bf16'):
             raise ValueError("gemm_dtype must be 'f32', 'f32_native' or 'bf16'")
         self.x3 = self.gemm_dtype == 'f32' and os.environ.get("CHAM_GEMM_X3", "1") == "1"
+        self.scorer_tail = os.environ.get("CHAM_SCORER_TAIL", "1") if self.x3 else "0"
         self.p3 = self.x3 and os.environ.get("CHAM_GEMM_P3", "1") == "1" and self.layout.C % 256 == 0
         self.h2 = self.p3 and os.environ.get("CHAM_GEMM_H2", "1") == "1"
         blk = os.environ.get("CHAM_H2_BLOCKED", "0")
@@ -970,6 +971,7 @@
         pl = rt.plan(B, T, N, self.negative_sample_from_buffer, d['Bg'])
         self._plan, self._d = pl, d
         pl.used_p3 = False
+        pl.tail, pl.tail_train = None, False
         check(lib.cham_set_log_bases(self.elapsed_days_smooth_log_base, self.popularity_smooth_log_base), "cham_set_log_bases")
         if d.get('uploaded') is not None:
             torch.cuda.current_stream().wait_event(d['uploaded'])
@@ -1180,12 +1182,18 @@
             Z2c = pl.Z2[BT:Rall]
             rt.gemm(Z2c, p('Ws1'), pl.S1, Rc, 128, C, C, 128, 128, bias=p('bs1'), act=ACT_LEAKY, rowscale=pl.pred, ldrs=C, rs_div=NC,
                     h2scales=(rt.sc_unit, rt.sc_ws1n) if rt.s1_h2_fwd else None)
-            rt.gemm(pl.S1, p('Ws2'), pl.S2, Rc, 64, 128, 128, 64, 64, bias=p('bs2'), act=ACT_LEAKY)
-            rt.gemm(pl.S2, p('Ws3'), pl.S3, Rc, 32, 64, 64, 32, 32, bias=p('bs3'), act=ACT_LEAKY)
+            if rt.scorer_tail != "0" and 2 <= NC <= 256 and (256 // NC) * NC >= 192:
+                pl.tail, pl.tail_train = rt.scorer_tail, self.is_training
+            else:
+                rt.gemm(pl.S1, p('Ws2'), pl.S2, Rc, 64, 128, 128, 64, 64, bias=p('bs2'), act=ACT_LEAKY)
+                rt.gemm(pl.S2, p('Ws3'), pl.S3, Rc, 32, 64, 64, 32, 32, bias=p('bs3'), act=ACT_LEAKY)
             softmax_fwd = lib.cham_score_softmax_fwd
-        check(softmax_fwd(ptr(pl.S3), 32, ptr(p('Ws4')), ptr(p('bs4')), BT, N, float(self.softmax_temperature),
-                          ptr(pl.mask), ptr(pl.logits), ptr(pl.probs), ptr(pl.nll), self.novelty_reg_factor,
-                          ptr(neg_ids), ptr(st['pop_norm']), ptr(pl.nov_aux), s), "cham_score_softmax_fwd")
+        if pl.tail:
+            self._scorer_tail(pl, d, neg_ids, st, s)
+        else:
+            check(softmax_fwd(ptr(pl.S3), 32, ptr(p('Ws4')), ptr(p('bs4')), BT, N, float(self.softmax_temperature),
+                              ptr(pl.mask), ptr(pl.logits), ptr(pl.probs), ptr(pl.nll), self.novelty_reg_factor,
+                              ptr(neg_ids), ptr(st['pop_norm']), ptr(pl.nov_aux), s), "cham_score_softmax_fwd")
         def loss_kernels(s):
             check(lib.cham_sumsq_partial(ptr(rt.flat), L.n_reg, ptr(rt.sumsq), s), "cham_sumsq_partial")
             if dsc:
@@ -1206,6 +1214,21 @@
         if not self.is_training and st.get('device'):
             self.articles_recent_pop_norm.note_consumed(d['aci'])
         return pl
+
+    def _scorer_tail(self, pl, d, neg_ids, st, s):
+        rt, lib, p = self.rt, self.rt.lib, self.rt.p
+        train = 1 if pl.tail_train else 0
+        full = train and pl.tail == "2"
+        h2 = full and pl.used_p3 and rt.h2
+        args = [ptr(pl.S1), ptr(p('Ws2')), ptr(p('bs2')), ptr(p('Ws3')), ptr(p('bs3')), ptr(p('Ws4')), ptr(p('bs4')), pl.P, pl.N,
+                float(self.softmax_temperature), ptr(pl.mask), ptr(pl.S2), ptr(pl.S3), ptr(pl.logits), ptr(pl.probs), ptr(pl.nll),
+                self.novelty_reg_factor, ptr(neg_ids), ptr(st['pop_norm']), ptr(pl.nov_aux), train]
+        tail = [ptr(pl.ds) if train else None, ptr(pl.dS3) if train else None, ptr(pl.dS2) if train else None, ptr(pl.dS1) if full else None,
+                rt.sc_ws1n.data_ptr() + 8 if h2 else None, ptr(pl.sc_dz2) if h2 else None, ptr(pl.sc_ds1) if h2 else None, s]
+        if rt.dev_scalars:
+            check(lib.cham_scorer_tail_dev(*args, ptr(rt.scalars), *tail), "cham_scorer_tail_dev")
+        else:
+            check(lib.cham_scorer_tail(*args, float(d['sum_mask']) if train else 1.0, *tail), "cham_scorer_tail")
 
     def backward(self):
         rt, lib, L = self.rt, self.rt.lib, self.rt.layout
@@ -1263,7 +1286,10 @@
         else:
             rt.grads[:L.emb_end].zero_()
             e_start = mark()
-        if rt.dev_scalars:
+        tail = pl.tail if pl.tail_train else None
+        if tail:
+            pass
+        elif rt.dev_scalars:
             check((lib.cham_score_softmax_bwd_b16_dev if b16 else lib.cham_score_softmax_bwd_dev)(
                 ptr(pl.S3), 32, ptr(p('Ws4')), ptr(pl.probs), ptr(pl.mask), BT, N, float(self.softmax_temperature), ptr(rt.scalars),
                 ptr(pl.ds), ptr(pl.dS3), self.novelty_reg_factor, ptr(neg_ids), ptr(self._dev_state['pop_norm']), ptr(pl.logits),
@@ -1280,13 +1306,15 @@
             rt.gemm_b16(pl.dS2, 64, 0, sh['Ws2'], 64, 1, pl.dS1, 128, 0, Rc, 128, 64, dref=pl.S1, ldr=128, dact=ACT_LEAKY)
             Z2c, dZ2c = pl.Z2c[:Rc], pl.dZ2c[:Rc]
         else:
-            rt.gemm(pl.dS3, p('Ws3'), pl.dS2, Rc, 64, 32, 32, 32, 64, transB=1, dref=pl.S2, ldr=64, dact=ACT_LEAKY)
-            rt.gemm(pl.dS2, p('Ws2'), pl.dS1, Rc, 128, 64, 64, 64, 128, transB=1, dref=pl.S1, ldr=128, dact=ACT_LEAKY)
+            if not tail:
+                rt.gemm(pl.dS3, p('Ws3'), pl.dS2, Rc, 64, 32, 32, 32, 64, transB=1, dref=pl.S2, ldr=64, dact=ACT_LEAKY)
+            if tail != "2":
+                rt.gemm(pl.dS2, p('Ws2'), pl.dS1, Rc, 128, 64, 64, 64, 128, transB=1, dref=pl.S1, ldr=128, dact=ACT_LEAKY)
             if not (use_p3 and rt.dm_fused and 32 <= NC <= 256):
                 pl.ensure_rows('dZ2')
             Z2c, dZ2c = pl.Z2[BT:Rall], pl.dZ2[BT:Rall]
         h2 = use_p3 and rt.h2
-        if h2:
+        if h2 and tail != "2":
             check(lib.cham_h2_scale_rownorm2(ptr(pl.dS1), Rc, pl.dS1.shape[1], pl.dS1.shape[1], rt.sc_ws1n.data_ptr() + 8, ptr(pl.sc_dz2),
                                              ptr(pl.sc_ds1), s), "cham_h2_scale_rownorm2")
         e_dS1 = mark()
diff --git a/include/chameleon_nar.h b/include/chameleon_nar.h
--- a/include/chameleon_nar.h
+++ b/include/chameleon_nar.h
@@ -197,6 +197,16 @@
                            float tau, float sum_mask, float* ds, float* dS3, float novelty_reg_factor, const int64_t* neg_ids,
                            const float* pop_norm, const float* logits, const float* nov_aux, void* stream);
 
+int cham_scorer_tail(const float* S1, const float* Ws2, const float* bs2, const float* Ws3, const float* bs3, const float* w4, const float* b4,
+                     int BT, int N, float tau, const uint8_t* mask, float* S2, float* S3, float* logits, float* probs, float* nll,
+                     float novelty_reg_factor, const int64_t* neg_ids, const float* pop_norm, float* nov_aux, int train, float sum_mask,
+                     float* ds, float* dS3, float* dS2, float* dS1, const float* factor, void* rec, void* rec_plain, void* stream);
+int cham_scorer_tail_dev(const float* S1, const float* Ws2, const float* bs2, const float* Ws3, const float* bs3, const float* w4, const float* b4,
+                         int BT, int N, float tau, const uint8_t* mask, float* S2, float* S3, float* logits, float* probs, float* nll,
+                         float novelty_reg_factor, const int64_t* neg_ids, const float* pop_norm, float* nov_aux, int train, const void* scalars,
+                         float* ds, float* dS3, float* dS2, float* dS1, const float* factor, void* rec, void* rec_plain, void* stream);
+int cham_scorer_tail_rows(void);
+
 int cham_rank_items(const float* probs, const int64_t* label_next, const int64_t* neg_ids, const uint8_t* mask, int BT, int N,
                     int64_t* pred_ids, float* pred_probs, int32_t* label_rank, void* stream);
 
```

After: 35010, median of 6. About the same (+0.2%).
